# tarepan/DDSP-SVC-official

Hardware: AMD Instinct MI355X
Metric: audio samples/sec @44.1kHz CombSub synth (higher is better)
Workload: dtype f32 storage and accumulation; products of the GEMM / FIR contractions split-bf16x3 (hi*hi+hi*lo+lo*hi), of the attention split-bf16 from three pieces (6 products) for the feature projections and two (3 products) for the context sums; everything else f32; `value_fp32_mfma` is the leg with every produ; 1 GPU; CombSub 44.1 kHz, batch=64x2 s per GPU (Fr=172, T=88064), units/f0/volume/spk_id -> audio, seeded random weights, in-kernel noise

## Files before the change

### ddsp-svc-official_amd/csrc/fir_synth.hip

```cpp
#include "gemm_f32.h"
#include "tables.h"

#include <stdlib.h>

namespace {

__global__ void __launch_bounds__(256) fir_act_kernel(int mode, const float* __restrict__ ctrl, int64_t ld, int M,
                                                      int ldo, int64_t rows, float* __restrict__ out, int split) {
    const int lane = threadIdx.x & 63;
    const int64_t row = (int64_t)blockIdx.x * 4 + (threadIdx.x >> 6);
    if (row >= rows) return;
    const float* src = ctrl + row * ld;
    if (mode != DDSP_FIR_ALLPASS) {
        float* dst = out + row * ldo;
        const float scale = (mode == DDSP_FIR_STATIC) ? (1.0f / 128.0f) : 1.0f;
        if (split) {
            for (int f0 = 0; f0 < M; f0 += 64) {
                const int f = f0 + lane;
                const float v = f < M ? expf(src[f]) * scale : 0.f;
                const uint32_t w = ddsp_split1_group8(v, lane);
                if (f < M) ((uint32_t*)dst)[f] = w;
            }
            return;
        }
        for (int f = lane; f < M; f += 64) dst[f] = expf(src[f]) * scale;
        return;
    }
    float* dst = out + row * ldo;
    const float pi_f = 3.14159274101257324f;
    double carry = 0.0;
    for (int f0 = 0; f0 < M; f0 += 64) {
        const int f = f0 + lane;
        const float gd = (f < M) ? __fmul_rn(pi_f, tanhf(src[f])) : 0.f;
        double incl = (double)gd;
#pragma unroll
        for (int o = 1; o < 64; o <<= 1) {
            double nb = __shfl_up(incl, o, 64);
            if (lane >= o) incl += nb;
        }
        const float phi = (float)(carry + incl);
        carry += __shfl(incl, 63, 64);
        float s = 0.f, c = 0.f;
        if (f < M) sincosf(phi, &s, &c);
        if (split) {
            const uint32_t wc = ddsp_split1_group8(c, lane), ws = ddsp_split1_group8(s, lane);
            if (f < M) {
                ((uint32_t*)dst)[f] = wc;
                ((uint32_t*)dst)[M + f] = ws;
            }
        } else if (f < M) {
            dst[f] = c;
            dst[M + f] = s;
        }
    }
}

struct EpiDynWindow {
    float* ir;
    int n;
    const float* f0;
    float sr15;
    int fast;
    __device__ __forceinline__ float col(int) const { return 0.f; }
    __device__ __forceinline__ float window_fast(float inv_hw, int k) const {
        float w = (float)(k - n / 2) * inv_hw;
        if (w > 1.0f) w = 0.0f;
        return fmaf(0.5f, __builtin_amdgcn_cosf(0.5f * w), 0.5f);
    }
    __device__ __forceinline__ float window(float hw, int k) const {
        float w = __fdiv_rn((float)(k - n / 2), hw);
        if (w > 1.0f) w = 0.0f;
        return __fdiv_rn(__fadd_rn(1.0f, cosf(__fmul_rn(3.14159274101257324f, w))), 2.0f);
    }
    __device__ __forceinline__ void operator()(int, int m, int k, float v, float) const {
        float* row = ir + (int64_t)m * n;
        if (fast) {
            const float inv_hw = __fdiv_rn(__fadd_rn(f0[m], 1e-3f), sr15);
            row[k] = v * window_fast(inv_hw, k);
            if (k > 0 && k < n / 2) row[n - k] = v * window_fast(inv_hw, n - k);
            return;
        }
        const float hw = __fdiv_rn(sr15, __fadd_rn(f0[m], 1e-3f));
        row[k] = __fmul_rn(v, window(hw, k));
        if (k > 0 && k < n / 2) row[n - k] = __fmul_rn(v, window(hw, n - k));
    }
};

struct EpiMirrorStore {
    float* ir;
    int n;
    __device__ __forceinline__ float col(int) const { return 0.f; }
    __device__ __forceinline__ void operator()(int, int m, int k, float v, float) const {
        float* row = ir + (int64_t)m * n;
        row[k] = v;
        if (k > 0 && k < n / 2) row[n - k] = v;
    }
};


__global__ void __launch_bounds__(256) fir_act_exp8_kernel(float scale, const float* __restrict__ ctrl, int64_t ld, int M, int ldo,
                                                           int64_t rows, float* __restrict__ out, int split) {
    const int per_row = M / 8;
    const int64_t i = (int64_t)blockIdx.x * 256 + threadIdx.x;
    if (i >= rows * per_row) return;
    const int64_t row = i / per_row;
    const int gq = (int)(i % per_row);
    const float* src = ctrl + row * ld + 8 * gq;
    const f32x4 a = *(const f32x4*)src, b = *(const f32x4*)(src + 4);
    float v[8];
#pragma unroll
    for (int e = 0; e < 4; ++e) {
        v[e] = expf(a[e]) * scale;
        v[4 + e] = expf(b[e]) * scale;
    }
    float* dst = out + row * ldo + 8 * gq;
    if (split) {
        ddsp_u32x4 hi, lo;
        ddsp_split8(v, hi, lo);
        *(ddsp_u32x4*)dst = hi;
        *(ddsp_u32x4*)(dst + 4) = lo;
    } else {
        *(f32x4*)dst = f32x4{v[0], v[1], v[2], v[3]};
        *(f32x4*)(dst + 4) = f32x4{v[4], v[5], v[6], v[7]};
    }
}

template <int CTRL, int ROW_MASK>
__device__ __forceinline__ double act_dpp_d(double v) {
    const uint64_t u = __builtin_bit_cast(uint64_t, v);
    const int lo = __builtin_amdgcn_update_dpp(0, (int)(uint32_t)u, CTRL, ROW_MASK, 0xf, false);
    const int hi = __builtin_amdgcn_update_dpp(0, (int)(uint32_t)(u >> 32), CTRL, ROW_MASK, 0xf, false);
    return __builtin_bit_cast(double, ((uint64_t)(uint32_t)hi << 32) | (uint32_t)lo);
}
__global__ void __launch_bounds__(256) fir_act_allpass4_kernel(const float* __restrict__ ctrl, int64_t ld, int M, int ldo, int64_t rows,
                                                               float* __restrict__ out, int split) {
    const int lane = threadIdx.x & 63;
    const int64_t row = (int64_t)blockIdx.x * 4 + (threadIdx.x >> 6);
    if (row >= rows) return;
    const float* src = ctrl + row * ld;
    float* dst = out + row * ldo;
    const float pi_f = 3.14159274101257324f;
    double carry = 0.0;
    for (int f0 = 0; f0 < M; f0 += 256) {
        const int f = f0 + 4 * lane;
        const bool in = f < M;
        f32x4 x = {0.f, 0.f, 0.f, 0.f};
        if (in) x = *(const f32x4*)(src + f);
        double run = 0.0, loc[4];
#pragma unroll
        for (int e = 0; e < 4; ++e) {
            const float gd = in ? __fmul_rn(pi_f, tanhf(x[e])) : 0.f;
            run += (double)gd;
            loc[e] = run;
        }
        double incl = run;
        incl += act_dpp_d<0x111, 0xf>(incl);
        incl += act_dpp_d<0x112, 0xf>(incl);
        incl += act_dpp_d<0x114, 0xf>(incl);
        incl += act_dpp_d<0x118, 0xf>(incl);
        incl += act_dpp_d<0x142, 0xa>(incl);
        incl += act_dpp_d<0x143, 0xc>(incl);
        const double base = carry + (incl - run);
        f32x4 c, sn;
#pragma unroll
        for (int e = 0; e < 4; ++e) {
            const float phi = (float)(base + loc[e]);
            float s_ = 0.f, c_ = 0.f;
            if (in) sincosf(phi, &s_, &c_);
            c[e] = c_;
            sn[e] = s_;
        }
        {
            const uint64_t u = __builtin_bit_cast(uint64_t, incl);
            const uint32_t lo = __builtin_amdgcn_readlane((int)(uint32_t)u, 63), hi = __builtin_amdgcn_readlane((int)(uint32_t)(u >> 32), 63);
            carry += __builtin_bit_cast(double, ((uint64_t)hi << 32) | lo);
        }
        if (split) {
            const ddsp_u32x4 pc = ddsp_split4_pair(c, (lane & 1) != 0, 1), ps = ddsp_split4_pair(sn, (lane & 1) != 0, 1);
            if (in) {
                *(ddsp_u32x4*)(dst + f) = pc;
                *(ddsp_u32x4*)(dst + M + f) = ps;
            }
        } else if (in) {
            *(f32x4*)(dst + f) = c;
            *(f32x4*)(dst + M + f) = sn;
        }
    }
}

__global__ void __launch_bounds__(256) repack_rows_kernel(const float* __restrict__ src, int n, int64_t rows, int ld,
                                                          float* __restrict__ dst) {
    typedef float f32x2r __attribute__((ext_vector_type(2)));
    const int half = ld / 2;
    const int64_t total = rows * half;
    for (int64_t i = (int64_t)blockIdx.x * blockDim.x + threadIdx.x; i < total; i += (int64_t)gridDim.x * blockDim.x) {
        const int64_t m = i / half;
        const int k = 2 * (int)(i % half);
        f32x2r v = {0.f, 0.f};
        if (k < n) v = *(const f32x2r*)(src + m * n + k);
        *(f32x2r*)(dst + m * ld + k) = v;
    }
}

__global__ void __launch_bounds__(256) dyn_window_scale_kernel(float* __restrict__ d_ir, const float* __restrict__ f0,
                                                               int n, int64_t rows, float sr15) {
    const int64_t total = rows * n;
    for (int64_t i = (int64_t)blockIdx.x * blockDim.x + threadIdx.x; i < total; i += (int64_t)gridDim.x * blockDim.x) {
        const int64_t m = i / n;
        const int k = (int)(i % n);
        const float hw = __fdiv_rn(sr15, __fadd_rn(f0[m], 1e-3f));
        float w = __fdiv_rn((float)(k - n / 2), hw);
        if (w > 1.0f) w = 0.0f;
        d_ir[i] *= __fdiv_rn(__fadd_rn(1.0f, cosf(__fmul_rn(3.14159274101257324f, w))), 2.0f);
    }
}

__global__ void __launch_bounds__(256) fir_act_bwd_kernel(int mode, const float* __restrict__ ctrl, int64_t ld, int M,
                                                          const float* __restrict__ d_act, int lda, int64_t rows,
                                                          float* __restrict__ d_ctrl, int64_t ldo) {
    const int lane = threadIdx.x & 63;
    const int64_t row = (int64_t)blockIdx.x * 4 + (threadIdx.x >> 6);
    if (row >= rows) return;
    const float* src = ctrl + row * ld;
    const float* g = d_act + row * lda;
    float* dst = d_ctrl + row * ldo;
    if (mode != DDSP_FIR_ALLPASS) {
        const float scale = (mode == DDSP_FIR_STATIC) ? (1.0f / 128.0f) : 1.0f;
        for (int f = lane; f < M; f += 64) dst[f] = g[f] * (expf(src[f]) * scale);
        return;
    }
    const float pi_f = 3.14159274101257324f;
    float th[16], dphi[16];
    double carry = 0.0;
    const int nchunk = (M + 63) / 64;
#pragma unroll
    for (int c = 0; c < 16; ++c) {
        th[c] = 0.f;
        dphi[c] = 0.f;
        if (c < nchunk) {
            const int f = c * 64 + lane;
            const float t = (f < M) ? tanhf(src[f]) : 0.f;
            th[c] = t;
            double incl = (double)((f < M) ? __fmul_rn(pi_f, t) : 0.f);
#pragma unroll
            for (int o = 1; o < 64; o <<= 1) {
                double nb = __shfl_up(incl, o, 64);
                if (lane >= o) incl += nb;
            }
            const float phi = (float)(carry + incl);
            carry += __shfl(incl, 63, 64);
            if (f < M) {
                double sn, cs;
                sincos((double)phi, &sn, &cs);
                dphi[c] = (float)(-sn * (double)g[f] + cs * (double)g[M + f]);
            }
        }
    }
    float tail = 0.f;
#pragma unroll
    for (int c = 15; c >= 0; --c) {
        if (c < nchunk) {
            float incl = dphi[c];
#pragma unroll
            for (int o = 1; o < 64; o <<= 1) {
                float nb = __shfl_down(incl, o, 64);
                if (lane + o < 64) incl += nb;
            }
            const float G = incl + tail;
            tail += __shfl(incl, 0, 64);
            const int f = c * 64 + lane;
            if (f < M) dst[f] = G * pi_f * (1.0f - th[c] * th[c]);
        }
    }
}

}


extern "C" int ddsp_fir_from_ctrl(ddsp_ctx* ctx, void* stream, int mode, const float* ctrl, int64_t ctrl_ld,
                                  int n_mag, const float* f0_frames, int64_t rows, int sr, float* ir) {
    DDSP_REQUIRE(ctx, ctx && ctrl && ir, "ddsp_fir_from_ctrl: null argument");
    DDSP_REQUIRE(ctx, mode >= 0 && mode <= 2, "ddsp_fir_from_ctrl: unknown mode");
    DDSP_REQUIRE(ctx, n_mag >= 3 && n_mag <= 1024 && ctrl_ld >= n_mag && rows >= 0 && rows < (1 << 30),
                 "ddsp_fir_from_ctrl: bad shape");
    DDSP_REQUIRE(ctx, mode != DDSP_FIR_DYNAMIC || f0_frames, "ddsp_fir_from_ctrl: DYNAMIC needs f0_frames");
    if (rows == 0) return DDSP_OK;
    hipStream_t st = (hipStream_t)stream;
    DDSP_ENTER_DEVICE(ctx);
    const int M = n_mag, n = 2 * (n_mag - 1);
    const int K = (mode == DDSP_FIR_ALLPASS) ? 2 * M : M;
    const int lda = ddsp_pad4(K);
    int rc = ddsp_scratch_reserve_bytes(ctx, (size_t)rows * lda * sizeof(float) + 4096);
    if (rc) return rc;
    ddsp_scratch_reset(ctx);
    float* act = nullptr;
    rc = ddsp_scratch_get(ctx, (size_t)rows * lda * sizeof(float), (void**)&act);
    if (rc) return rc;
    float* tab = nullptr;
    const int kind = mode == DDSP_FIR_ALLPASS ? TAB_IRDFT_CPLX : (mode == DDSP_FIR_STATIC ? TAB_IRDFT_RE_HANN : TAB_IRDFT_RE);
    const bool tap_major = K % 32 == 0;
    rc = ddsp_get_table(ctx, st, kind, M, tap_major ? 1 : 0, &tab);
    if (rc) return rc;
    float* tab_split = nullptr;
    if (tap_major && ctx->math != DDSP_MATH_FP32 && (rc = ddsp_get_table(ctx, st, kind, M, 2, &tab_split))) return rc;

    const bool presplit = tap_major && tab_split && rows >= 8192 && M % 8 == 0 && ctx->math != 4;
    ddsp_prof_begin(ctx, st, PF_FIR_ACT);
    const bool wide = M % 8 == 0 && ctrl_ld % 4 == 0 && lda % 8 == 0 && ((uintptr_t)ctrl % 16) == 0;
    if (wide && mode != DDSP_FIR_ALLPASS)
        hipLaunchKernelGGL(fir_act_exp8_kernel, dim3((unsigned)ceil_div64(rows * (M / 8), 256)), dim3(256), 0, st,
                           mode == DDSP_FIR_STATIC ? 1.0f / 128.0f : 1.0f, ctrl, ctrl_ld, M, lda, rows, act, presplit ? 1 : 0);
    else if (wide)
        hipLaunchKernelGGL(fir_act_allpass4_kernel, dim3((unsigned)ceil_div64(rows, 4)), dim3(256), 0, st, ctrl, ctrl_ld, M, lda, rows,
                           act, presplit ? 1 : 0);
    else
        hipLaunchKernelGGL(fir_act_kernel, dim3((unsigned)ceil_div64(rows, 4)), dim3(256), 0, st, mode, ctrl, ctrl_ld, M,
                           lda, rows, act, presplit ? 1 : 0);
    ddsp_prof_end(ctx, st, 0.0, 4.0 * rows * (M + K));
    DDSP_LAUNCH_CHECK(ctx);
    ddsp_prof_begin(ctx, st, PF_FIR_DFT_GEMM);

    auto run = [&](gemm::Args g, const auto& epi) {
        g.math = tap_major ? (ctx->math == 4 ? DDSP_MATH_SPLIT_BF16 : ctx->math) : 0;
        g.B_split = tab_split;
        if (presplit) {
            g.A_split = 1;
            g.B = tab_split;
        }
        if (tap_major)
            gemm::launch<true, true, gemm::A_PLAIN>(st, g, 1, epi);
        else
            gemm::launch<true, false, gemm::A_PLAIN>(st, g, 1, epi);
    };
    const int64_t ldb = tap_major ? K : ddsp_pad4(n);
    if (mode == DDSP_FIR_ALLPASS) {
        gemm::Args g = gemm::make(act, lda, tab, ldb, (int)rows, n, K);
        run(g, gemm::EpiStore{ir, n, nullptr, 1, 0, 0});
    } else {
        gemm::Args g = gemm::make(act, lda, tab, ldb, (int)rows, n / 2 + 1, K);
        if (mode == DDSP_FIR_DYNAMIC)
            run(g, EpiDynWindow{ir, n, f0_frames, 1.5f * (float)sr, (tap_major && ctx->math != DDSP_MATH_FP32) ? 1 : 0});
        else
            run(g, EpiMirrorStore{ir, n});
    }
    ddsp_prof_end(ctx, st, 2.0 * rows * (double)n * K, 4.0 * rows * (K + n));
    DDSP_LAUNCH_CHECK(ctx);
    return DDSP_OK;
}

extern "C" int ddsp_fir_from_ctrl_bwd(ddsp_ctx* ctx, void* stream, int mode, const float* ctrl, int64_t ctrl_ld,
                                      int n_mag, const float* f0_frames, int64_t rows, int sr, float* d_ir,
                                      float* d_ctrl, int64_t d_ctrl_ld) {
    DDSP_REQUIRE(ctx, ctx && ctrl && d_ir && d_ctrl, "ddsp_fir_from_ctrl_bwd: null argument");
    DDSP_REQUIRE(ctx, mode >= 0 && mode <= 2, "ddsp_fir_from_ctrl_bwd: unknown mode");
    DDSP_REQUIRE(ctx, n_mag >= 3 && n_mag <= 1024 && ctrl_ld >= n_mag && d_ctrl_ld >= n_mag && rows >= 0 && rows < (1 << 30),
                 "ddsp_fir_from_ctrl_bwd: bad shape");
    DDSP_REQUIRE(ctx, mode != DDSP_FIR_DYNAMIC || f0_frames, "ddsp_fir_from_ctrl_bwd: DYNAMIC needs f0_frames");
    if (rows == 0) return DDSP_OK;
    hipStream_t st = (hipStream_t)stream;
    DDSP_ENTER_DEVICE(ctx);
    const int M = n_mag, n = 2 * (n_mag - 1);
    const int K = (mode == DDSP_FIR_ALLPASS) ? 2 * M : M;
    const int lda = ddsp_pad4(K);
    const int ldp = ddsp_pad4(n);
    const bool repack = ctx->math != DDSP_MATH_FP32 && ldp % 32 == 0 && rows >= 1024;
    int rc = ddsp_scratch_reserve_bytes(ctx, (size_t)rows * (lda + (repack ? ldp : 0)) * sizeof(float) + 8192);
    if (rc) return rc;
    ddsp_scratch_reset(ctx);
    float* d_act = nullptr;
    if ((rc = ddsp_scratch_get(ctx, (size_t)rows * lda * sizeof(float), (void**)&d_act))) return rc;
    float* d_pad = nullptr;
    if (repack && (rc = ddsp_scratch_get(ctx, (size_t)rows * ldp * sizeof(float), (void**)&d_pad))) return rc;
    float* tab = nullptr;
    const int kind = mode == DDSP_FIR_ALLPASS ? TAB_IRDFT_CPLX : (mode == DDSP_FIR_STATIC ? TAB_IRDFT_RE_HANN : TAB_IRDFT_RE);
    if ((rc = ddsp_get_table(ctx, st, kind, M, 0, &tab))) return rc;
    ddsp_prof_begin(ctx, st, PF_FIR_SYNTH_BWD);
    if (mode == DDSP_FIR_DYNAMIC) {
        int64_t blocks = ceil_div64(rows * n, 256);
        if (blocks > 8192) blocks = 8192;
        hipLaunchKernelGGL(dyn_window_scale_kernel, dim3((unsigned)blocks), dim3(256), 0, st, d_ir, f0_frames, n, rows,
                           1.5f * (float)sr);
    }
    gemm::EpiStore e{d_act, lda, nullptr, 1, 0, 0};
    if (repack) {
        int64_t blocks = ceil_div64(rows * (ldp / 2), 256);
        if (blocks > 8192) blocks = 8192;
        hipLaunchKernelGGL(repack_rows_kernel, dim3((unsigned)blocks), dim3(256), 0, st, d_ir, n, rows, ldp, d_pad);
        gemm::Args g = gemm::make(d_pad, ldp, tab, ldp, (int)rows, K, ldp);
        g.math = DDSP_MATH_SPLIT_BF16;
        gemm::launch<true, true, gemm::A_PLAIN>(st, g, 1, e);
    } else {
        gemm::Args g = gemm::make(d_ir, n, tab, ddsp_pad4(n), (int)rows, K, n);
        gemm::launch<true, true, gemm::A_PLAIN>(st, g, 1, e);
    }
    hipLaunchKernelGGL(fir_act_bwd_kernel, dim3((unsigned)ceil_div64(rows, 4)), dim3(256), 0, st, mode, ctrl, ctrl_ld, M,
                       d_act, lda, rows, d_ctrl, d_ctrl_ld);
    ddsp_prof_end(ctx, st, 2.0 * rows * (double)n * K, 4.0 * rows * (2.0 * K + n));
    DDSP_LAUNCH_CHECK(ctx);
    return DDSP_OK;
}
```

### ddsp-svc-official_amd/csrc/gemm_f32.h

```cpp
#pragma once
#include "common.h"

#include <stdlib.h>
#include <type_traits>

namespace gemm {

enum { A_PLAIN = 0, A_CONV3 = 1, A_FRAMES = 2, A_CONVK = 3 };

struct Args {
    const float* A;
    const float* B;
    int M, N, K;
    int64_t lda, ldb;
    int zdiv;
    int64_t sA_hi, sA_lo, sB_hi, sB_lo;
    int Fr, Cin;
    int tap_shift;
    int ktaps, dil;
    float in_slope;
    const float* zeros;
    int sub_from, parent_tn;
    int math;
    const float* B_split;
    int A_split;
    int xcd;
    int xcd_cut;
    int kz;
};

constexpr int BK = 32;
typedef float f32x4_u __attribute__((ext_vector_type(4), aligned(4)));

template <class E, class = void>
struct epi_wants_pair : std::false_type {};
template <class E>
struct epi_wants_pair<E, std::void_t<decltype(E::kPair)>> : std::true_type {};
template <class E, class = void>
struct epi_has_store4 : std::false_type {};
template <class E>
struct epi_has_store4<E, std::void_t<decltype(E::kStore4)>> : std::true_type {};

template <class E, class = void>
struct epi_is_gated : std::false_type {};
template <class E>
struct epi_is_gated<E, std::void_t<decltype(E::kGatedPair)>> : std::true_type {};

template <class E, class = void>
struct epi_is_rowpair : std::false_type {};
template <class E>
struct epi_is_rowpair<E, std::void_t<decltype(E::kRowPair)>> : std::true_type {};

__device__ __forceinline__ void quad_transpose(float (&x)[4], int q) {
    const bool odd = q & 1, hi = q & 2;
    auto swap1 = [](float v) { return __builtin_bit_cast(float, __builtin_amdgcn_mov_dpp(__builtin_bit_cast(int, v), 0xB1, 0xF, 0xF, true)); };
    auto swap2 = [](float v) { return __builtin_bit_cast(float, __builtin_amdgcn_mov_dpp(__builtin_bit_cast(int, v), 0x4E, 0xF, 0xF, true)); };
    const float r0 = swap1(odd ? x[0] : x[1]);
    const float r1 = swap1(odd ? x[2] : x[3]);
    const float a_lo = odd ? r0 : x[0], a_hi = odd ? x[1] : r0;
    const float b_lo = odd ? r1 : x[2], b_hi = odd ? x[3] : r1;
    const float s_lo = swap2(hi ? a_lo : b_lo);
    const float s_hi = swap2(hi ? a_hi : b_hi);
    x[0] = hi ? s_lo : a_lo;
    x[1] = hi ? s_hi : a_hi;
    x[2] = hi ? b_lo : s_lo;
    x[3] = hi ? b_hi : s_hi;
}

template <int BM, int BN, bool A_KC, bool B_KC, int A_MODE, class Epi, int NW = 4>
__global__ void __launch_bounds__(64 * NW) kernel(Args g, Epi epi) {
    constexpr int WGM = NW / 2, WGN = 2, NT = 64 * NW;
    constexpr int TM = BM / (32 * WGM), TN = BN / (32 * WGN);
    static_assert(TM >= 1 && TN >= 1, "tile too small for the wave grid");
    constexpr int LDM = BM + 1, LDN = BN + 1;
    __shared__ float lds[2 * BK * (LDM + LDN)];
    float* const As0 = lds;
    float* const Bs0 = lds + 2 * BK * LDM;

    const int tid = threadIdx.x;
    const int lane = tid & 63;
    const int wave = tid >> 6;
    const int wm = (wave >> 1) * (BM / WGM);
    const int wn = (wave & 1) * (BN / WGN);
    const int m0 = blockIdx.y * BM;
    const int n0 = blockIdx.x * BN;
    const int z = blockIdx.z;
    const float* __restrict__ A = g.A + (A_MODE == A_FRAMES ? 0 : (int64_t)(z / g.zdiv) * g.sA_hi + (int64_t)(z % g.zdiv) * g.sA_lo);
    const float* __restrict__ B = g.B + (int64_t)(z / g.zdiv) * g.sB_hi + (int64_t)(z % g.zdiv) * g.sB_lo;

    constexpr int NA = BM * BK / (4 * NT), NB = BN * BK / (4 * NT);
    static_assert(NA >= 1 && NB >= 1, "tile too small for the thread count");
    f32x4 ra[NA], rb[NB];

    auto arow = [&](int m) -> const float* {
        if (A_MODE == A_FRAMES) return A + (int64_t)(m / g.Fr) * g.sA_hi + (int64_t)(m % g.Fr) * g.lda;
        return A + (int64_t)m * g.lda;
    };
    auto load_tiles = [&](int k0) {
        const bool k_full = (k0 + BK <= g.K);
        const bool a_full = k_full && (m0 + BM <= g.M);
        const bool b_full = k_full && (n0 + BN <= g.N);
#pragma unroll
        for (int i = 0; i < NA; ++i) {
            const int q = tid + i * NT;
            f32x4 v = {0.f, 0.f, 0.f, 0.f};
            if (A_KC) {
                const int r = q / (BK / 4), kq = q % (BK / 4);
                const int m = m0 + r, k = k0 + kq * 4;
                if (A_MODE == A_CONV3) {
                    if (m < g.M && k < g.K) {
                        const int tap = k / g.Cin, c = k - tap * g.Cin;
                        const int off = tap - 1 + g.tap_shift;
                        const int f = m % g.Fr + off;
                        if (f >= 0 && f < g.Fr) v = *(const f32x4_u*)(A + (int64_t)(m + off) * g.lda + c);
                    }
                } else if (A_MODE == A_CONVK) {
                    if (m < g.M && k < g.K) {
                        const int tap = k / g.Cin, c = k - tap * g.Cin;
                        const int off = (tap - (g.ktaps - 1) / 2) * g.dil;
                        const int f = m % g.Fr + off;
                        if (f >= 0 && f < g.Fr) {
                            v = *(const f32x4_u*)(A + (int64_t)(m + off) * g.lda + c);
#pragma unroll
                            for (int j = 0; j < 4; ++j) v[j] = v[j] > 0.f ? v[j] : v[j] * g.in_slope;
                        }
                    }
                } else if (a_full) {
                    v = *(const f32x4_u*)(arow(m) + k);
                } else if (m < g.M) {
                    const float* p = arow(m) + k;
                    if (k + 3 < g.K) {
                        v = *(const f32x4_u*)p;
                    } else {
                        if (k < g.K) v[0] = p[0];
                        if (k + 1 < g.K) v[1] = p[1];
                        if (k + 2 < g.K) v[2] = p[2];
                    }
                }
            } else {
                const int kr = q / (BM / 4), mq = q % (BM / 4);
                const int k = k0 + kr, m = m0 + mq * 4;
                if (a_full) {
                    v = *(const f32x4_u*)(A + (int64_t)k * g.lda + m);
                } else if (k < g.K) {
                    const float* p = A + (int64_t)k * g.lda + m;
                    if (m + 3 < g.M) {
                        v = *(const f32x4_u*)p;
                    } else {
                        if (m < g.M) v[0] = p[0];
                        if (m + 1 < g.M) v[1] = p[1];
                        if (m + 2 < g.M) v[2] = p[2];
                    }
                }
            }
            ra[i] = v;
        }
#pragma unroll
        for (int i = 0; i < NB; ++i) {
            const int q = tid + i * NT;
            f32x4 v = {0.f, 0.f, 0.f, 0.f};
            if (B_KC) {
                const int r = q / (BK / 4), kq = q % (BK / 4);
                const int n = n0 + r, k = k0 + kq * 4;
                if (b_full) {
                    v = *(const f32x4_u*)(B + (int64_t)n * g.ldb + k);
                } else if (n < g.N) {
                    const float* p = B + (int64_t)n * g.ldb + k;
                    if (k + 3 < g.K) {
                        v = *(const f32x4_u*)p;
                    } else {
                        if (k < g.K) v[0] = p[0];
                        if (k + 1 < g.K) v[1] = p[1];
                        if (k + 2 < g.K) v[2] = p[2];
                    }
                }
            } else {
                const int kr = q / (BN / 4), nq = q % (BN / 4);
                const int k = k0 + kr, n = n0 + nq * 4;
                if (b_full) {
                    v = *(const f32x4_u*)(B + (int64_t)k * g.ldb + n);
                } else if (k < g.K) {
                    const float* p = B + (int64_t)k * g.ldb + n;
                    if (n + 3 < g.N) {
                        v = *(const f32x4_u*)p;
                    } else {
                        if (n < g.N) v[0] = p[0];
                        if (n + 1 < g.N) v[1] = p[1];
                        if (n + 2 < g.N) v[2] = p[2];
                    }
                }
            }
            rb[i] = v;
        }
    };

    auto store_tiles = [&](int buf) {
        float* as = As0 + buf * (BK * LDM);
        float* bs = Bs0 + buf * (BK * LDN);
#pragma unroll
        for (int i = 0; i < NA; ++i) {
            const int q = tid + i * NT;
            if (A_KC) {
                const int r = q / (BK / 4), kq = q % (BK / 4);
#pragma unroll
                for (int j = 0; j < 4; ++j) as[(kq * 4 + j) * LDM + r] = ra[i][j];
            } else {
                const int kr = q / (BM / 4), mq = q % (BM / 4);
#pragma unroll
                for (int j = 0; j < 4; ++j) as[kr * LDM + mq * 4 + j] = ra[i][j];
            }
        }
#pragma unroll
        for (int i = 0; i < NB; ++i) {
            const int q = tid + i * NT;
            if (B_KC) {
                const int r = q / (BK / 4), kq = q % (BK / 4);
#pragma unroll
                for (int j = 0; j < 4; ++j) bs[(kq * 4 + j) * LDN + r] = rb[i][j];
            } else {
                const int kr = q / (BN / 4), nq = q % (BN / 4);
#pragma unroll
                for (int j = 0; j < 4; ++j) bs[kr * LDN + nq * 4 + j] = rb[i][j];
            }
        }
    };

    f32x16 acc[TM][TN];
#pragma unroll
    for (int i = 0; i < TM; ++i)
#pragma unroll
        for (int j = 0; j < TN; ++j)
#pragma unroll
            for (int r = 0; r < 16; ++r) acc[i][j][r] = 0.f;

    const int nk = (g.K + BK - 1) / BK;
    load_tiles(0);
    store_tiles(0);
    __syncthreads();
    const int lr = lane & 31, lh = lane >> 5;
    for (int kt = 0; kt < nk; ++kt) {
        const int buf = kt & 1;
        if (kt + 1 < nk) load_tiles((kt + 1) * BK);
        const float* as = As0 + buf * (BK * LDM) + wm + lr + lh * LDM;
        const float* bs = Bs0 + buf * (BK * LDN) + wn + lr + lh * LDN;
        float a[TM], b[TN];
#pragma unroll
        for (int i = 0; i < TM; ++i) a[i] = as[32 * i];
#pragma unroll
        for (int j = 0; j < TN; ++j) b[j] = bs[32 * j];
#pragma unroll
        for (int kk = 0; kk < BK; kk += 2) {
            float an[TM], bn[TN];
            if (kk + 2 < BK) {
#pragma unroll
                for (int i = 0; i < TM; ++i) an[i] = as[(kk + 2) * LDM + 32 * i];
#pragma unroll
                for (int j = 0; j < TN; ++j) bn[j] = bs[(kk + 2) * LDN + 32 * j];
            }
#pragma unroll
            for (int i = 0; i < TM; ++i)
#pragma unroll
                for (int j = 0; j < TN; ++j)
                    acc[i][j] = __builtin_amdgcn_mfma_f32_32x32x2f32(a[i], b[j], acc[i][j], 0, 0, 0);
            if (kk + 2 < BK) {
#pragma unroll
                for (int i = 0; i < TM; ++i) a[i] = an[i];
#pragma unroll
                for (int j = 0; j < TN; ++j) b[j] = bn[j];
            }
        }
        if (kt + 1 < nk) store_tiles(buf ^ 1);
        __syncthreads();
    }

#pragma unroll
    for (int i = 0; i < TM; ++i)
#pragma unroll
        for (int j = 0; j < TN; ++j) {
            const int n = n0 + wn + 32 * j + lr;
            const bool n_ok = n < g.N;
            const float cb = n_ok ? epi.col(n) : 0.f;
#pragma unroll
            for (int r = 0; r < 16; ++r) {
                const int m = m0 + wm + 32 * i + (r & 3) + 8 * (r >> 2) + 4 * lh;
                if constexpr (epi_is_rowpair<Epi>::value) {
                    if ((r & 1) == 0 && n_ok && m < g.M) epi.pair(z, m, n, acc[i][j][r], acc[i][j][r + 1], cb);
                } else if constexpr (epi_wants_pair<Epi>::value) {
                    const float other = __shfl_xor(acc[i][j][r], 1, 64);
                    if (n_ok && m < g.M) epi(z, m, n, acc[i][j][r], other);
                } else {
                    if (n_ok && m < g.M) epi(z, m, n, acc[i][j][r], cb);
                }
            }
        }
}


template <int BM, int BN, class Epi, int NS = 3, int NW = 8, int A_MODE = A_PLAIN, int MATH = 0>
__global__ void __launch_bounds__(64 * NW, (NW == 4 ? 3 : BM * BN <= 128 * 128 ? 4 : 2)) kernel_dma(Args g, Epi epi, int tiles_m, int tiles_n, int total_tiles) {
    constexpr int WGM = NW / 2, WGN = 2;
    constexpr int TM = BM / (32 * WGM), TN = BN / (32 * WGN);
    constexpr int ROWS = BM + BN;
    constexpr int STAGE = ROWS * 32;
    constexpr int PIECES = ROWS / 8;
    constexpr int PPW = PIECES / NW;
    static_assert(PIECES % NW == 0, "stage must split evenly over the waves");
    __shared__ __attribute__((aligned(1024))) float lds[NS * STAGE];

    const int tid = threadIdx.x, lane = tid & 63, wave = __builtin_amdgcn_readfirstlane(tid >> 6);
    const int wm = (wave >> 1) * (BM / WGM), wn = (wave & 1) * (BN / WGN);
    const int lr = lane & 31, lh = lane >> 5;
    const int nk = g.K / 32;

    const bool xcd_order = g.xcd && (gridDim.x & 7) == 0 && g.sub_from == 0 && total_tiles == tiles_m * tiles_n - g.xcd_cut;
    const int xq0 = (int)blockIdx.x >> 3, xgs = (int)gridDim.x >> 3, xx = (int)blockIdx.x & 7;
    const int xown = (tiles_m / 8) * tiles_n, xleft = (tiles_m % 8) * tiles_n - g.xcd_cut;
    int my_tiles = (total_tiles - (int)blockIdx.x + (int)gridDim.x - 1) / (int)gridDim.x;
    if (xcd_order) {
        const int qx = xown + (xleft > xx ? (xleft - xx + 7) / 8 : 0);
        my_tiles = xq0 < qx ? (qx - xq0 + xgs - 1) / xgs : 0;
    }
    auto tile_of = [&](int i) -> int {
        if (!xcd_order) return (int)blockIdx.x + i * (int)gridDim.x;
        const int q = xq0 + i * xgs;
        if (q < xown) return (xx + 8 * (q / tiles_n)) * tiles_n + q % tiles_n;
        const int u = (q - xown) * 8 + xx;
        return ((tiles_m / 8) * 8 + u / tiles_n) * tiles_n + u % tiles_n;
    };
    const int steps = my_tiles * nk;

    constexpr int PA = (BM / 8) / NW;
    static_assert((BM / 8) % NW == 0, "A rows must split evenly over the waves");
    const float* src_m1[PA];
    const float* src_p1[PA];
    int conv_f[PA];
    int kbase_cur = 0;
    auto tile_src = [&](int tile, const float* (&src)[PPW]) {
        const int per_z = tiles_m * tiles_n;
        int z = tile / per_z, rem = tile - z * per_z;
        int m0 = (rem / tiles_n) * BM, n0 = (rem % tiles_n) * BN;
        if (g.sub_from > 0) {
            const int big = g.sub_from + (tile >> 2), q = tile & 3;
            z = 0;
            m0 = (2 * (big / g.parent_tn) + (q >> 1)) * BM;
            n0 = (2 * (big % g.parent_tn) + (q & 1)) * BN;
        }
        const float* A = g.A + (int64_t)(z / g.zdiv) * g.sA_hi + (int64_t)(z % g.zdiv) * g.sA_lo;
        const float* B = g.B + (int64_t)(z / g.zdiv) * g.sB_hi + (int64_t)(z % g.zdiv) * g.sB_lo;
        kbase_cur = z * g.kz;
#pragma unroll
        for (int i = 0; i < PPW; ++i) {
            const int piece = wave + NW * i;
            const int row = piece * 8 + (lane >> 3);
            const int slot = (lane & 7) ^ ((row >> 1) & 7);
            if (row < BM) {
                int m = m0 + row;
                m = m < g.M ? m : g.M - 1;
                src[i] = A + (int64_t)m * g.lda + slot * 4;
                if constexpr (A_MODE == A_CONVK) {
                    if (i < PA) conv_f[i < PA ? i : 0] = m % g.Fr;
                }
                if constexpr (A_MODE == A_CONV3) {
                    if (i < PA) {
                        const int f = m % g.Fr;
                        const int s = g.tap_shift;
                        const float* base = src[i];
                        const float* zp = g.zeros + slot * 4;
                        src_m1[i < PA ? i : 0] = (f - 1 + s >= 0 && f - 1 + s < g.Fr) ? base + (int64_t)(s - 1) * g.lda : zp;
                        src_p1[i < PA ? i : 0] = (f + 1 + s >= 0 && f + 1 + s < g.Fr) ? base + (int64_t)(s + 1) * g.lda : zp;
                        src[i] = (f + s >= 0 && f + s < g.Fr) ? base + (int64_t)s * g.lda : zp;
                    }
                }
            } else {
                int n = n0 + row - BM;
                n = n < g.N ? n : g.N - 1;
                src[i] = B + (int64_t)n * g.ldb + slot * 4;
            }
        }
    };
    auto issue = [&](const float* const (&src)[PPW], int kt, int stage) {
        int tap = 1, koff = kt * 32 + kbase_cur;
        if constexpr (A_MODE == A_CONV3 || A_MODE == A_CONVK) {
            tap = koff / g.Cin;
            koff -= tap * g.Cin;
        }
        const int conv_off = A_MODE == A_CONVK ? (tap - (g.ktaps - 1) / 2) * g.dil : 0;
#pragma unroll
        for (int i = 0; i < PPW; ++i) {
            const int piece = wave + NW * i;
            const float* p = src[i] + kt * 32 + kbase_cur;
            if constexpr (A_MODE == A_CONV3) {
                if (i < PA) p = (tap == 0 ? src_m1[i < PA ? i : 0] : tap == 1 ? src[i] : src_p1[i < PA ? i : 0]) + koff;
            }
            if constexpr (A_MODE == A_CONVK) {
                if (i < PA) {
                    const int f = conv_f[i < PA ? i : 0] + conv_off;
                    p = (f >= 0 && f < g.Fr) ? src[i] + (int64_t)conv_off * g.lda + koff : g.zeros + (lane & 7) * 4;
                }
            }
            __builtin_amdgcn_global_load_lds((const __attribute__((address_space(1))) void*)p,
                                             (__attribute__((address_space(3))) void*)(lds + stage * STAGE + piece * 256),
                                             16, 0, 0);
        }
    };

    const float* src_cur[PPW];
    int issued = 0;
    int issue_tile = 0, issue_kt = 0;
    if (steps > 0) tile_src(tile_of(0), src_cur);
    auto issue_next = [&]() {
        if (issued >= steps) return;
        issue(src_cur, issue_kt, issued % NS);
        ++issued;
        if (++issue_kt == nk) {
            issue_kt = 0;
            ++issue_tile;
            if (issue_tile < my_tiles) tile_src(tile_of(issue_tile), src_cur);
        }
    };
#pragma unroll
    for (int i = 0; i < NS - 1; ++i) issue_next();

    f32x16 acc[TM][TN];
#pragma unroll
    for (int i = 0; i < TM; ++i)
#pragma unroll
        for (int j = 0; j < TN; ++j)
#pragma unroll
            for (int r = 0; r < 16; ++r) acc[i][j][r] = 0.f;

    int kt = 0, tile_i = 0;
    for (int step = 0; step < steps; ++step) {
        static_assert((NS - 2) * PPW <= 63, "vmcnt is a 6-bit counter");
        if (NS > 2 && step + NS - 2 < steps)
            asm volatile("s_waitcnt vmcnt(%0)" ::"n"((NS - 2) * PPW) : "memory");
        else
            asm volatile("s_waitcnt vmcnt(0)" ::: "memory");
        __builtin_amdgcn_s_barrier();
        issue_next();
        const float* st = lds + (step % NS) * STAGE;
        f32x4 av[TM][4], bv[TN][4];
#pragma unroll
        for (int i = 0; i < TM; ++i) {
            const int row = wm + 32 * i + lr;
            const float* rp = st + row * 32;
#pragma unroll
            for (int c = 0; c < 4; ++c) av[i][c] = *(const f32x4*)(rp + 4 * ((4 * lh + c) ^ ((row >> 1) & 7)));
        }
#pragma unroll
        for (int j = 0; j < TN; ++j) {
            const int row = BM + wn + 32 * j + lr;
            const float* rp = st + row * 32;
#pragma unroll
            for (int c = 0; c < 4; ++c) bv[j][c] = *(const f32x4*)(rp + 4 * ((4 * lh + c) ^ ((row >> 1) & 7)));
        }
        if constexpr (MATH != 0) {
            typedef __bf16 bf16x8 __attribute__((ext_vector_type(8)));
            typedef float f32x2p __attribute__((ext_vector_type(2)));
            typedef __bf16 bf16x2p __attribute__((ext_vector_type(2)));
            typedef uint32_t u32x4p __attribute__((ext_vector_type(4)));
            auto split = [](const f32x4& x0, const f32x4& x1, bf16x8 (&p)[3]) {
                constexpr int NQ = 2;
                u32x4p w[3];
#pragma unroll
                for (int d = 0; d < 4; ++d) {
                    f32x2p r = d < 2 ? (f32x2p){x0[2 * d], x0[2 * d + 1]} : (f32x2p){x1[2 * d - 4], x1[2 * d - 3]};
#pragma unroll
                    for (int q = 0; q < NQ; ++q) {
                        const uint32_t h = __builtin_bit_cast(uint32_t, __builtin_convertvector(r, bf16x2p));
                        w[q][d] = h;
                        if (q + 1 < NQ)
                            r = r - (f32x2p){__builtin_bit_cast(float, h << 16), __builtin_bit_cast(float, h & 0xffff0000u)};
                    }
                }
#pragma unroll
                for (int q = 0; q < NQ; ++q) p[q] = __builtin_bit_cast(bf16x8, w[q]);
            };
#pragma unroll
            for (int half = 0; half < 2; ++half) {
                bf16x8 ap[TM][3], bp[TN][3];
#pragma unroll
                for (int i = 0; i < TM; ++i) {
                    if constexpr (MATH == 8) {
                        ap[i][0] = __builtin_bit_cast(bf16x8, av[i][2 * half]);
                        ap[i][1] = __builtin_bit_cast(bf16x8, av[i][2 * half + 1]);
                    } else {
                        split(av[i][2 * half], av[i][2 * half + 1], ap[i]);
                    }
                }
#pragma unroll
                for (int j = 0; j < TN; ++j) {
                    if constexpr (MATH == 7 || MATH == 8) {
                        bp[j][0] = __builtin_bit_cast(bf16x8, bv[j][2 * half]);
                        bp[j][1] = __builtin_bit_cast(bf16x8, bv[j][2 * half + 1]);
                    } else {
                        split(bv[j][2 * half], bv[j][2 * half + 1], bp[j]);
                    }
                }
#pragma unroll
                for (int i = 0; i < TM; ++i)
#pragma unroll
                    for (int j = 0; j < TN; ++j) {
                        auto mm = [&](int x, int y) {
                            acc[i][j] = __builtin_amdgcn_mfma_f32_32x32x16_bf16(ap[i][x], bp[j][y], acc[i][j], 0, 0, 0);
                        };
                        mm(1, 0);
                        mm(0, 1);
                        mm(0, 0);
                    }
            }
        } else {
#pragma unroll
            for (int s = 0; s < 16; ++s)
#pragma unroll
                for (int i = 0; i < TM; ++i)
#pragma unroll
                    for (int j = 0; j < TN; ++j)
                        acc[i][j] = __builtin_amdgcn_mfma_f32_32x32x2f32(av[i][s >> 2][s & 3], bv[j][s >> 2][s & 3],
                                                                         acc[i][j], 0, 0, 0);
        }
        if (++kt == nk) {
            const int tile = tile_of(tile_i);
            const int per_z = tiles_m * tiles_n;
            int z = tile / per_z, rem = tile - z * per_z;
            int m0 = (rem / tiles_n) * BM, n0 = (rem % tiles_n) * BN;
            if (g.sub_from > 0) {
                const int big = g.sub_from + (tile >> 2), q = tile & 3;
                z = 0;
                m0 = (2 * (big / g.parent_tn) + (q >> 1)) * BM;
                n0 = (2 * (big % g.parent_tn) + (q & 1)) * BN;
            }
            bool vec = false;
            if constexpr (epi_has_store4<Epi>::value) vec = epi.vec_ok() && n0 + BN <= g.N;
            if constexpr (epi_is_gated<Epi>::value) {
                static_assert(TN == 2, "gated-pair epilogue needs the wave's two column blocks");
                const int q = lane & 3;
                const int na = n0 + wn + lr;
                const float ba = epi.col(na), bg = epi.col(na + 32);
                const int oc = ((n0 + wn) >> 1) + (lr & ~3);
#pragma unroll
                for (int i = 0; i < TM; ++i)
#pragma unroll
                    for (int rg = 0; rg < 4; ++rg) {
                        float x[4];
#pragma unroll
                        for (int r = 0; r < 4; ++r) {
                            const float a = acc[i][0][4 * rg + r] + ba, gt = acc[i][1][4 * rg + r] + bg;
                            if constexpr (MATH != 0)
                                x[r] = a * __builtin_amdgcn_rcpf(1.0f + __builtin_amdgcn_exp2f(-1.44269504088896341f * gt));
                            else
                                x[r] = a * (1.0f / (1.0f + expf(-gt)));
                            acc[i][0][4 * rg + r] = 0.f;
                            acc[i][1][4 * rg + r] = 0.f;
                        }
                        quad_transpose(x, q);
                        const int m = m0 + wm + 32 * i + q + 8 * rg + 4 * lh;
                        if (m < g.M) epi.store4(z, m, oc, f32x4{x[0], x[1], x[2], x[3]});
                    }
            } else if (vec) {
                if constexpr (epi_has_store4<Epi>::value) {
                    const int q = lane & 3;
#pragma unroll
                    for (int i = 0; i < TM; ++i)
#pragma unroll
                        for (int j = 0; j < TN; ++j) {
                            const int n = n0 + wn + 32 * j + (lr & ~3);
#pragma unroll
                            for (int rg = 0; rg < 4; ++rg) {
                                float x[4] = {acc[i][j][4 * rg], acc[i][j][4 * rg + 1], acc[i][j][4 * rg + 2], acc[i][j][4 * rg + 3]};
                                quad_transpose(x, q);
                                const int m = m0 + wm + 32 * i + q + 8 * rg + 4 * lh;
                                if (m < g.M) epi.store4(z, m, n, f32x4{x[0], x[1], x[2], x[3]});
#pragma unroll
                                for (int r = 0; r < 4; ++r) acc[i][j][4 * rg + r] = 0.f;
                            }
                        }
                }
            } else
#pragma unroll
            for (int i = 0; i < TM; ++i)
#pragma unroll
                for (int j = 0; j < TN; ++j) {
                    const int n = n0 + wn + 32 * j + lr;
                    const bool n_ok = n < g.N;
                    const float cb = n_ok ? epi.col(n) : 0.f;
#pragma unroll
                    for (int r = 0; r < 16; ++r) {
                        const int m = m0 + wm + 32 * i + (r & 3) + 8 * (r >> 2) + 4 * lh;
                        if constexpr (epi_is_rowpair<Epi>::value) {
                            if ((r & 1) == 0 && n_ok && m < g.M) epi.pair(z, m, n, acc[i][j][r], acc[i][j][r + 1], cb);
                        } else if constexpr (epi_wants_pair<Epi>::value) {
                            const float other = __shfl_xor(acc[i][j][r], 1, 64);
                            if (n_ok && m < g.M) epi(z, m, n, acc[i][j][r], other);
                        } else {
                            if (n_ok && m < g.M) epi(z, m, n, acc[i][j][r], cb);
                        }
                        acc[i][j][r] = 0.f;
                    }
                }
            kt = 0;
            ++tile_i;
        }
    }
}

inline bool dma_ok(const Args& g) {
    return g.K % 32 == 0 && g.lda % 4 == 0 && g.ldb % 4 == 0 && ((uintptr_t)g.A % 16) == 0 && ((uintptr_t)g.B % 16) == 0 &&
           g.sA_hi % 4 == 0 && g.sA_lo % 4 == 0 && g.sB_hi % 4 == 0 && g.sB_lo % 4 == 0;
}

template <int BM, int BN, class Epi, int NS = 3, int NW = 8, int A_MODE = A_PLAIN, int MATH = 0>
inline void launch_dma(hipStream_t st, const Args& g, int batch, const Epi& epi, int total_override = -1) {
    const int tiles_m = (g.M + BM - 1) / BM, tiles_n = (g.N + BN - 1) / BN;
    const int total = total_override >= 0 ? total_override : tiles_m * tiles_n * batch;
    if (total == 0) return;
    constexpr int lds_bytes = NS * (BM + BN) * 128;
    constexpr int by_waves = 16 / NW;
    constexpr int by_lds = 160 * 1024 / lds_bytes;
    constexpr int per_cu = by_lds < by_waves ? by_lds : by_waves;
    int grid = 256 * per_cu;
    if (grid > total) grid = total;
    hipLaunchKernelGGL((kernel_dma<BM, BN, Epi, NS, NW, A_MODE, MATH>), dim3(grid), dim3(64 * NW), 0, st, g, epi, tiles_m, tiles_n, total);
}

inline int xcd_default(int math) { return math == 3 ? 1 : 0; }

template <int BM, int BN, class Epi, int NS = 3, int NW = 8, int A_MODE = A_PLAIN>
inline void dma_go(hipStream_t st, const Args& g0, int batch, const Epi& epi, int total_override = -1) {
    Args g = g0;
    if (g.xcd < 0) g.xcd = (batch == 1 && total_override < 0) ? xcd_default(g.math) : 0;
    if (g.math == 3 && g.B_split && g.A_split) {
        Args h = g;
        h.B = g.B_split;
        launch_dma<BM, BN, Epi, NS, NW, A_MODE, 8>(st, h, batch, epi, total_override);
    } else if (g.math == 3 && g.B_split) {
        Args h = g;
        h.B = g.B_split;
        launch_dma<BM, BN, Epi, NS, NW, A_MODE, 7>(st, h, batch, epi, total_override);
    } else if (g.math == 3)
        launch_dma<BM, BN, Epi, NS, NW, A_MODE, 3>(st, g, batch, epi, total_override);
    else
        launch_dma<BM, BN, Epi, NS, NW, A_MODE, 0>(st, g, batch, epi, total_override);
}

template <int BM, int BN, bool A_KC, bool B_KC, int A_MODE, class Epi, int NW = 4>
inline void launch_tile(hipStream_t st, const Args& g, int batch, const Epi& epi) {
    dim3 grid((g.N + BN - 1) / BN, (g.M + BM - 1) / BM, batch);
    hipLaunchKernelGGL((kernel<BM, BN, A_KC, B_KC, A_MODE, Epi, NW>), grid, dim3(64 * NW), 0, st, g, epi);
}

constexpr int64_t T128_MIN = 512;

constexpr int SMALL_NS = 4;


template <bool A_KC, bool B_KC, int A_MODE, class Epi>
inline void launch(hipStream_t st, const Args& g, int batch, const Epi& epi) {
    auto blocks = [&](int bm, int bn) {
        return (int64_t)((g.M + bm - 1) / bm) * ((g.N + bn - 1) / bn) * batch;
    };
    if constexpr (A_KC && B_KC && A_MODE == A_CONV3) {
        if (dma_ok(g) && g.zeros && g.Cin % 32 == 0 && g.Cin + 32 <= DDSP_ZERO_FLOATS && g.N <= 256) {
            if (blocks(64, 64) < 128 && blocks(64, 64) > 16)
                dma_go<32, 64, Epi, 4, 2, A_CONV3>(st, g, batch, epi);
            else
                dma_go<64, 64, Epi, 3, 4, A_CONV3>(st, g, batch, epi);
            return;
        }
    }
    if constexpr (A_KC && B_KC && A_MODE == A_PLAIN) {
        if (dma_ok(g) && blocks(64, 64) < 128 && blocks(64, 64) > 16 && g.K >= 256) {
            dma_go<32, 64, Epi, 4, 2>(st, g, batch, epi);
            return;
        }
        if (dma_ok(g) && blocks(64, 64) < 256 && g.K >= 256) {
            dma_go<64, 64, Epi, SMALL_NS, 4>(st, g, batch, epi);
            return;
        }
        if (dma_ok(g) && g.N <= 256 && blocks(64, 64) >= 256) {
            dma_go<64, 64, Epi, 3, 4>(st, g, batch, epi);
            return;
        }
        if (dma_ok(g) && blocks(128, 64) >= 256) {
            if (g.N <= 256)
                dma_go<64, 64, Epi, 3, 4>(st, g, batch, epi);
            else if (blocks(128, 128) >= T128_MIN) {
                const int total = (int)blocks(128, 128);
                const int rem = total % 512;
                bool split = false;
                if constexpr (!epi_is_gated<Epi>::value) {
                    const bool xcd_on = g.xcd > 0 || (g.xcd < 0 && xcd_default(g.math));
                    if (batch == 1 && rem > 0 && rem <= 64 && !xcd_on) {
                        split = true;
                        dma_go<128, 128, Epi, 2>(st, g, batch, epi, total - rem);
                        Args r = g;
                        r.xcd = 0;
                        r.sub_from = total - rem;
                        r.parent_tn = (g.N + 127) / 128;
                        dma_go<64, 64, Epi, 3, 4>(st, r, 1, epi, 4 * rem);
                    }
                }
                if (!split) dma_go<128, 128, Epi, 2>(st, g, batch, epi);
            }
            else
                dma_go<128, 64, Epi, 3>(st, g, batch, epi);
            return;
        }
        if (dma_ok(g) && blocks(64, 64) >= 256) {
            dma_go<64, 64, Epi, 3, 4>(st, g, batch, epi);
            return;
        }
    }
    if ((g.B_split && g.B_split == g.B) || g.A_split) {
        ddsp_launch_refusal() = "pre-split GEMM operands reached the register-staged path (size predicates disagree)";
        return;
    }
    if (blocks(128, 64) >= 512)
        launch_tile<128, 64, A_KC, B_KC, A_MODE, Epi, 8>(st, g, batch, epi);
    else
        launch_tile<64, 64, A_KC, B_KC, A_MODE, Epi, 4>(st, g, batch, epi);
}

inline Args make(const float* A, int64_t lda, const float* B, int64_t ldb, int M, int N, int K) {
    Args g;
    g.A = A;
    g.B = B;
    g.M = M;
    g.N = N;
    g.K = K;
    g.lda = lda;
    g.ldb = ldb;
    g.zdiv = 1;
    g.sA_hi = g.sA_lo = g.sB_hi = g.sB_lo = 0;
    g.Fr = 1;
    g.Cin = 4;
    g.tap_shift = 0;
    g.ktaps = 3;
    g.dil = 1;
    g.in_slope = 1.f;
    g.zeros = nullptr;
    g.sub_from = 0;
    g.parent_tn = 0;
    g.math = 0;
    g.B_split = nullptr;
    g.A_split = 0;
    g.xcd_cut = 0;
    g.xcd = -1;
    g.kz = 0;
    return g;
}

struct EpiStore {
    float* C;
    int64_t ldc;
    const float* bias;
    int zdiv;
    int64_t sC_hi, sC_lo;
    __device__ __forceinline__ float col(int n) const { return bias ? bias[n] : 0.f; }
    __device__ __forceinline__ void operator()(int z, int m, int n, float v, float cb) const {
        float* c = C + (int64_t)(z / zdiv) * sC_hi + (int64_t)(z % zdiv) * sC_lo;
        c[(int64_t)m * ldc + n] = v + cb;
    }
    static constexpr bool kStore4 = true;
    __device__ __forceinline__ bool vec_ok() const {
        return ((uintptr_t)C % 16) == 0 && ldc % 4 == 0 && sC_hi % 4 == 0 && sC_lo % 4 == 0;
    }
    __device__ __forceinline__ void store4(int z, int m, int n, f32x4 v) const {
        float* c = C + (int64_t)(z / zdiv) * sC_hi + (int64_t)(z % zdiv) * sC_lo;
        if (bias) v += *(const f32x4_u*)(bias + n);
        *(f32x4*)(c + (int64_t)m * ldc + n) = v;
    }
};

struct EpiResidual {
    float* C;
    const float* res;
    int64_t ldc;
    const float* bias;
    __device__ __forceinline__ float col(int n) const { return bias[n]; }
    __device__ __forceinline__ void operator()(int, int m, int n, float v, float cb) const {
        const int64_t o = (int64_t)m * ldc + n;
        C[o] = res[o] + (v + cb);
    }
    static constexpr bool kStore4 = true;
    __device__ __forceinline__ bool vec_ok() const { return (((uintptr_t)C | (uintptr_t)res) % 16) == 0 && ldc % 4 == 0; }
    __device__ __forceinline__ void store4(int, int m, int n, f32x4 v) const {
        const int64_t o = (int64_t)m * ldc + n;
        *(f32x4*)(C + o) = *(const f32x4*)(res + o) + (v + *(const f32x4_u*)(bias + n));
    }
};

}
```

### ddsp-svc-official_amd/csrc/tables.h

```cpp
#pragma once
#include "common.h"

enum {
    TAB_IRDFT_RE = 1,
    TAB_IRDFT_RE_HANN = 2,
    TAB_IRDFT_CPLX = 3,
    TAB_RDFT_FWD_W = 4,
    TAB_RDFT_INV_W = 5,
};

static inline int ddsp_pad4(int n) { return (n + 3) & ~3; }
```

### ddsp-svc-official_amd/csrc/tables.hip

```cpp
#include "tables.h"

namespace {

constexpr double kTwoPi = 6.283185307179586476925286766559;

__global__ void irdft_table_kernel(float* __restrict__ tab, int M, int n, int ld, int rows, int hann, int tap_major) {
    const int64_t total = tap_major ? (int64_t)n * rows : (int64_t)rows * ld;
    for (int64_t idx = (int64_t)blockIdx.x * blockDim.x + threadIdx.x; idx < total;
         idx += (int64_t)gridDim.x * blockDim.x) {
        const int row = tap_major ? (int)(idx % rows) : (int)(idx / ld);
        const int k = tap_major ? (int)(idx / rows) : (int)(idx % ld);
        if (k >= n) {
            tab[idx] = 0.f;
            continue;
        }
        const int f = row < M ? row : row - M;
        const double cf = (f == 0 || f == M - 1) ? 1.0 : 2.0;
        int64_t r = ((int64_t)f * (k - n / 2)) % n;
        if (r < 0) r += n;
        const double ang = kTwoPi * (double)r / (double)n;
        double v;
        if (row < M)
            v = cf / n * cos(ang);
        else
            v = (f == 0 || f == M - 1) ? 0.0 : -cf / n * sin(ang);
        if (hann) v *= 0.5 - 0.5 * cos(kTwoPi * (double)k / (double)n);
        tab[idx] = (float)v;
    }
}

__global__ void rdft_w_table_kernel(float* __restrict__ tab, int N, int ld, int inverse) {
    const int Mb = N / 2 + 1;
    const int64_t total = inverse ? (int64_t)N * 2 * Mb : (int64_t)N * ld;
    for (int64_t idx = (int64_t)blockIdx.x * blockDim.x + threadIdx.x; idx < total;
         idx += (int64_t)gridDim.x * blockDim.x) {
        int i, col;
        if (!inverse) {
            i = (int)(idx / ld);
            col = (int)(idx % ld);
            if (col >= 2 * Mb) {
                tab[idx] = 0.f;
                continue;
            }
        } else {
            col = (int)(idx / N);
            i = (int)(idx % N);
        }
        const int f = col < Mb ? col : col - Mb;
        const bool im = col >= Mb;
        const int64_t r = ((int64_t)f * i) % N;
        const double ang = kTwoPi * (double)r / (double)N;
        const double w = sqrt(0.5 - 0.5 * cos(kTwoPi * (double)i / (double)N));
        double v;
        if (!inverse) {
            v = im ? -sin(ang) : cos(ang);
        } else {
            const double cf = (f == 0 || f == N / 2) ? 1.0 : 2.0;
            v = im ? ((f == 0 || f == N / 2) ? 0.0 : -cf / N * sin(ang)) : cf / N * cos(ang);
        }
        tab[idx] = (float)(v * w);
    }
}

__global__ void presplit_kernel(const float* __restrict__ src, uint32_t* __restrict__ dst, int64_t groups) {
    typedef float f32x2v __attribute__((ext_vector_type(2)));
    typedef __bf16 bf16x2v __attribute__((ext_vector_type(2)));
    for (int64_t gidx = (int64_t)blockIdx.x * blockDim.x + threadIdx.x; gidx < groups; gidx += (int64_t)gridDim.x * blockDim.x) {
        const float* s = src + 8 * gidx;
        uint32_t hi[4], lo[4];
#pragma unroll
        for (int d = 0; d < 4; ++d) {
            const float a = s[2 * d], b = s[2 * d + 1];
            hi[d] = __builtin_bit_cast(uint32_t, __builtin_convertvector((f32x2v){a, b}, bf16x2v));
            const float ha = __builtin_bit_cast(float, hi[d] << 16), hb = __builtin_bit_cast(float, hi[d] & 0xffff0000u);
            lo[d] = __builtin_bit_cast(uint32_t, __builtin_convertvector((f32x2v){a - ha, b - hb}, bf16x2v));
        }
        uint32_t* o = dst + 8 * gidx;
#pragma unroll
        for (int d = 0; d < 4; ++d) {
            o[d] = hi[d];
            o[4 + d] = lo[d];
        }
    }
}

}

int ddsp_get_table(ddsp_ctx* ctx, hipStream_t st, int kind, int n0, int n1, float** out) {
    for (int i = 0; i < ctx->n_tables; ++i) {
        ddsp_table& t = ctx->tables[i];
        if (t.kind == kind && t.n0 == n0 && t.n1 == n1) {
            *out = t.dev;
            return DDSP_OK;
        }
    }
    if (ctx->n_tables >= 64) return ddsp_fail(ctx, DDSP_ERR_OOM, "table cache full", "");
    if (n1 == 2) {
        float* plain = nullptr;
        int rc = ddsp_get_table(ctx, st, kind, n0, 1, &plain);
        if (rc) return rc;
        if (ctx->n_tables >= 64) return ddsp_fail(ctx, DDSP_ERR_OOM, "table cache full", "");
        size_t bytes = 0;
        for (int i = 0; i < ctx->n_tables; ++i)
            if (ctx->tables[i].dev == plain) bytes = ctx->tables[i].bytes;
        if (bytes == 0 || bytes % 32 != 0) return ddsp_fail(ctx, DDSP_ERR_ARG, "table cannot be pre-split", "");
        float* dev = nullptr;
        hipError_t e = hipMalloc((void**)&dev, bytes);
        if (e != hipSuccess) return ddsp_fail(ctx, DDSP_ERR_OOM, "table hipMalloc", hipGetErrorString(e));
        const int64_t groups = (int64_t)(bytes / 32);
        hipLaunchKernelGGL(presplit_kernel, dim3((unsigned)((groups + 255) / 256 > 2048 ? 2048 : (groups + 255) / 256)), dim3(256), 0,
                           st, plain, (uint32_t*)dev, groups);
        DDSP_LAUNCH_CHECK(ctx);
        ddsp_table& t = ctx->tables[ctx->n_tables++];
        t.kind = kind;
        t.n0 = n0;
        t.n1 = n1;
        t.dev = dev;
        t.bytes = bytes;
        *out = dev;
        return DDSP_OK;
    }
    size_t elems = 0;
    switch (kind) {
        case TAB_IRDFT_RE:
        case TAB_IRDFT_RE_HANN:
            elems = n1 ? (size_t)n0 * 2 * (n0 - 1) : (size_t)n0 * ddsp_pad4(2 * (n0 - 1));
            break;
        case TAB_IRDFT_CPLX:
            elems = n1 ? (size_t)2 * n0 * 2 * (n0 - 1) : (size_t)2 * n0 * ddsp_pad4(2 * (n0 - 1));
            break;
        case TAB_RDFT_FWD_W:
            elems = (size_t)n0 * ddsp_pad4(2 * (n0 / 2 + 1));
            break;
        case TAB_RDFT_INV_W:
            elems = (size_t)n0 * 2 * (n0 / 2 + 1);
            break;
        default:
            return ddsp_fail(ctx, DDSP_ERR_ARG, "unknown table kind", "");
    }
    float* dev = nullptr;
    hipError_t e = hipMalloc((void**)&dev, elems * sizeof(float));
    if (e != hipSuccess) return ddsp_fail(ctx, DDSP_ERR_OOM, "table hipMalloc", hipGetErrorString(e));
    const unsigned blocks = (unsigned)((elems + 255) / 256 > 2048 ? 2048 : (elems + 255) / 256);
    if (kind == TAB_IRDFT_RE || kind == TAB_IRDFT_RE_HANN || kind == TAB_IRDFT_CPLX) {
        const int M = n0, n = 2 * (n0 - 1);
        const int rows = kind == TAB_IRDFT_CPLX ? 2 * M : M;
        hipLaunchKernelGGL(irdft_table_kernel, dim3(blocks), dim3(256), 0, st, dev, M, n, ddsp_pad4(n), rows,
                           kind == TAB_IRDFT_RE_HANN ? 1 : 0, n1 ? 1 : 0);
    } else {
        hipLaunchKernelGGL(rdft_w_table_kernel, dim3(blocks), dim3(256), 0, st, dev, n0,
                           ddsp_pad4(2 * (n0 / 2 + 1)), kind == TAB_RDFT_INV_W ? 1 : 0);
    }
    DDSP_LAUNCH_CHECK(ctx);
    ddsp_table& t = ctx->tables[ctx->n_tables++];
    t.kind = kind;
    t.n0 = n0;
    t.n1 = n1;
    t.dev = dev;
    t.bytes = elems * sizeof(float);
    *out = dev;
    return DDSP_OK;
}
```

### ddsp-svc-official_amd/ddsp/vocoder.py

```python
import os

import torch
import yaml

import hipddsp
from hipddsp import (COMB_SINC, COMB_SINC_GATED, COMB_NONE, EXC_AUDIO, EXC_GENERATE, EXC_UNIT_NOISE, FIR_ALLPASS,
                     FIR_DYNAMIC, FIR_STATIC, FIR_SPLIT_BF16)


from .hubert import RaggedCounts
from .unit2control import Unit2Control


class Volume_Extractor:

    def __init__(self, hop_size=512, device="cuda"):
        self.hop_size = hop_size
        self.device = device

    def extract(self, audio, n_samples=None):
        import numpy as np
        if n_samples is not None:
            if not isinstance(audio, torch.Tensor) or audio.dim() != 2:
                raise ValueError("Volume_Extractor.extract: a ragged batch is a (B, T) tensor")
            if not float(self.hop_size).is_integer():
                raise ValueError("Volume_Extractor.extract: a ragged batch needs an integral hop_size")
            vals = hipddsp.check_volume_n_samples(n_samples, audio.shape[0], audio.shape[1], int(self.hop_size))
            if not audio.is_cuda:
                raise RuntimeError("Volume_Extractor runs on a HIP device only (no CPU fallback)")
            return hipddsp.context_for(audio.device).volume_extract(audio, int(self.hop_size), vals)
        is_np = isinstance(audio, np.ndarray)
        x = torch.from_numpy(np.ascontiguousarray(audio, dtype=np.float32)).to(self.device) if is_np else audio
        if not x.is_cuda:
            raise RuntimeError("Volume_Extractor runs on a HIP device only (no CPU fallback)")
        flat = x.dim() == 1
        hop = int(self.hop_size) if float(self.hop_size).is_integer() else float(self.hop_size)
        vol = hipddsp.context_for(x.device).volume_extract(x.reshape(1, -1) if flat else x, hop)
        vol = vol[0] if flat else vol
        return vol.cpu().numpy() if is_np else vol


def _find_torchcrepe_checkpoint(model="full"):
    import importlib.util
    try:
        spec = importlib.util.find_spec("torchcrepe")
    except (ImportError, ValueError):
        spec = None
    for d in (list(spec.submodule_search_locations or []) if spec is not None else []):
        p = os.path.join(d, "assets", f"{model}.pth")
        if os.path.isfile(p):
            return p
    raise FileNotFoundError(
        f"F0_Extractor('crepe'): no CREPE checkpoint given and no installed torchcrepe with assets/{model}.pth was found; pass "
        "crepe_ckpt='/path/to/full.pth' (torchcrepe's state dict) or a ddsp.crepe.Crepe module")


class F0_Extractor:

    def __init__(self, f0_extractor, sample_rate=44100, hop_size=512, f0_min=65, f0_max=800, *, crepe_ckpt=None, device=None):
        if f0_extractor in ('parselmouth', 'dio', 'harvest'):
            raise NotImplementedError(
                f"f0 extractor '{f0_extractor}' has no device implementation (it is a CPU library): 'crepe' is the device "
                "extractor; keep the reference's F0_Extractor for the others")
        if f0_extractor != 'crepe':
            raise ValueError(f" [x] Unknown f0 extractor: {f0_extractor}")
        self.f0_extractor, self.sample_rate, self.hop_size, self.f0_min, self.f0_max = \
            f0_extractor, sample_rate, hop_size, f0_min, f0_max
        if device is None:
            if not torch.cuda.is_available():
                raise RuntimeError("F0_Extractor runs on a HIP device only (no CPU fallback)")
            device = "cuda"
        if torch.device(device).type != "cuda":
            raise RuntimeError("F0_Extractor runs on a HIP device only (no CPU fallback); got device=%r" % (device,))
        from .crepe import Crepe
        if isinstance(crepe_ckpt, Crepe):
            model = crepe_ckpt
        else:
            path = crepe_ckpt if crepe_ckpt is not None else _find_torchcrepe_checkpoint("full")
            sd = torch.load(path, map_location="cpu", weights_only=True)
            model = Crepe("tiny" if sd["conv1.weight"].shape[0] == 128 else "full")
            model.load_state_dict(sd)
        self.model = model.to(device).eval()
        self.device = device

    def extract(self, audio, uv_interp=False, device=None, silence_front=0, *, dither=True, seed=None, seed_dev=None,
                n_samples=None):
        import numpy as np
        from .crepe import HOP, SAMPLE_RATE
        if n_samples is not None:
            return self._extract_ragged(audio, uv_interp, silence_front, dither, seed, seed_dev, n_samples)
        is_np = isinstance(audio, np.ndarray)
        x = torch.from_numpy(np.ascontiguousarray(audio, dtype=np.float32)).to(self.device) if is_np else audio
        if not x.is_cuda:
            raise RuntimeError("F0_Extractor runs on a HIP device only (no CPU fallback)")
        flat = x.dim() == 1
        if x.dim() not in (1, 2):
            raise ValueError("F0_Extractor.extract: audio must be (T,) or (B, T)")
        x = x.reshape(1, -1) if flat else x
        sr, hop = self.sample_rate, self.hop_size
        n_frames = int(x.shape[-1] // hop) + 1
        start_frame = int(silence_front * sr / hop)
        real_silence_front = start_frame * hop / sr
        x = x[:, int(np.round(real_silence_front * sr)):].contiguous().float()
        ctx = hipddsp.context_for(x.device)
        x16 = x if int(sr) == SAMPLE_RATE else ctx.resample(x, int(sr), SAMPLE_RATE, lowpass_filter_width=128)
        fr = hipddsp.crepe_frames(x16.shape[-1], HOP)
        if fr < 3:
            raise ValueError(f"F0_Extractor('crepe'): {x16.shape[-1]} samples at 16 kHz give {fr} CREPE frames; the reference's "
                             "reflect-padded filters need at least 3 (audio of at least 160 samples at 16 kHz)")
        probs = self.model.activations(x16, HOP)
        if seed_dev is not None:
            f0, pd = ctx.crepe_decode(probs, self.f0_min, self.f0_max, segment=512, dither=dither, seed_dev=seed_dev)
        else:
            if dither and seed is None:
                seed = _seed_from_torch()
            f0, pd = ctx.crepe_decode(probs, self.f0_min, self.f0_max, segment=512, dither_seed=int(seed or 0), dither=dither)
        out = ctx.f0_postfilter(f0, pd, sr, hop, n_frames, start_frame, 0.05, uv_interp, self.f0_min)
        out = out[0] if flat else out
        return out.cpu().numpy() if is_np else out


    def _extract_ragged(self, audio, uv_interp, silence_front, dither, seed, seed_dev, n_samples):
        from .crepe import HOP, SAMPLE_RATE
        if silence_front != 0:
            raise ValueError("F0_Extractor.extract: silence_front is not available with n_samples (a ragged batch)")
        if seed_dev is not None:
            raise ValueError("F0_Extractor.extract: seed_dev is not available with n_samples (a ragged batch)")
        if not isinstance(audio, torch.Tensor) or audio.dim() != 2:
            raise ValueError("F0_Extractor.extract: a ragged batch is a (B, T) tensor")
        B, T = audio.shape
        sr, hop = self.sample_rate, self.hop_size
        vals = hipddsp.check_n_samples(n_samples, B, T)
        resampled = int(sr) != SAMPLE_RATE
        lib = hipddsp.load_library()
        n16 = [int(lib.ddsp_resample_length(v, int(sr), SAMPLE_RATE)) for v in vals] if resampled else vals
        T16 = int(lib.ddsp_resample_length(T, int(sr), SAMPLE_RATE)) if resampled else T
        n16 = hipddsp.check_crepe_n_samples(n16, B, T16, HOP)
        if not audio.is_cuda:
            raise RuntimeError("F0_Extractor runs on a HIP device only (no CPU fallback)")
        ctx = hipddsp.context_for(audio.device)
        n_crepe = [hipddsp.crepe_frames(v, HOP) for v in n16]
        n_out = [int(v // hop) + 1 for v in vals]
        table = hipddsp.crepe_ragged_table(n16, HOP)
        dev = ctx.ragged_counts(vals + table + n_crepe + n_out)
        n_dev, table_dev, nc_dev, no_dev = dev[:B], dev[B:3 * B + 1], dev[3 * B + 1:4 * B + 1], dev[4 * B + 1:]
        x = audio.contiguous().float()
        x16 = ctx.resample_ragged(x, n_dev, int(sr), SAMPLE_RATE, lowpass_filter_width=128) if resampled else x
        probs = self.model.activations(x16, HOP, n16, table_dev)
        if dither and seed is None:
            seed = _seed_from_torch()
        f0, pd = ctx.crepe_decode(probs, self.f0_min, self.f0_max, segment=512, dither_seed=int(seed or 0), dither=dither,
                                  n_frames=n_crepe, counts_dev=nc_dev)
        return ctx.f0_postfilter(f0, pd, sr, hop, max(n_out), 0, 0.05, uv_interp, self.f0_min, n_crepe=n_crepe, n_out=n_out,
                                 counts_dev=(nc_dev, no_dev))


def align_units(units, n_samples, sample_rate, hop_size, encoder_sample_rate=16000, encoder_hop_size=320):
    n_frames = int(int(n_samples) // hop_size) + 1
    ratio = (hop_size / sample_rate) / (encoder_hop_size / encoder_sample_rate)
    return hipddsp.context_for(units.device).align_units(units, n_frames, ratio)


class Audio2HubertSoft(torch.nn.Module):

    def __init__(self, path, h_sample_rate=16000, h_hop_size=320, device=None):
        super().__init__()
        from torch.nn.modules.utils import consume_prefix_in_state_dict_if_present
        from .hubert import HubertSoft
        print(' [Encoder Model] HuBERT Soft')
        self.hubert = HubertSoft()
        print(' [Loading] ' + path)
        checkpoint = torch.load(path, map_location="cpu")
        consume_prefix_in_state_dict_if_present(checkpoint, "module.")
        self.hubert.load_state_dict(checkpoint)
        self.hubert.eval()
        if device is not None:
            self.hubert.to(device)

    def forward(self, audio, n_samples=None):
        return self.hubert.units(audio.unsqueeze(1), n_samples)


class Units_Encoder:

    def __init__(self, encoder, encoder_ckpt, encoder_sample_rate=16000, encoder_hop_size=320, device=None):
        if encoder in ('hubertbase', 'hubertbase768', 'contentvec', 'contentvec768', 'xunit', 'yunit'):
            raise NotImplementedError(
                f"units encoder '{encoder}' has no device implementation: 'hubertsoft' is the device encoder; callers that "
                "keep the reference's encoders can align their units on the device with ddsp.vocoder.align_units")
        if encoder != 'hubertsoft':
            raise ValueError(f" [x] Unknown units encoder: {encoder}")
        if device is None:
            if not torch.cuda.is_available():
                raise RuntimeError("Units_Encoder runs on a HIP device only (no CPU fallback)")
            device = "cuda"
        if torch.device(device).type != "cuda":
            raise RuntimeError("Units_Encoder runs on a HIP device only (no CPU fallback); got device=%r" % (device,))
        self.device = device
        self.model = Audio2HubertSoft(encoder_ckpt, device=device)
        self.model = self.model.eval()
        self.encoder_sample_rate = encoder_sample_rate
        self.encoder_hop_size = encoder_hop_size

    def encode(self, audio, sample_rate, hop_size, n_samples=None):
        if n_samples is not None:
            return self._encode_ragged(audio, sample_rate, hop_size, n_samples)
        if not audio.is_cuda:
            raise RuntimeError("Units_Encoder runs on a HIP device only (no CPU fallback)")
        ctx = hipddsp.context_for(audio.device)
        audio_res = audio if sample_rate == self.encoder_sample_rate else \
            ctx.resample(audio, int(sample_rate), int(self.encoder_sample_rate), lowpass_filter_width=128)
        units = self.model(audio_res)
        return align_units(units, audio.size(-1), sample_rate, hop_size, self.encoder_sample_rate, self.encoder_hop_size)

    def _encode_ragged(self, audio, sample_rate, hop_size, n_samples):
        if audio.dim() != 2:
            raise ValueError("Units_Encoder.encode: a ragged batch is (B, T) audio")
        B, T = audio.shape
        vals = hipddsp.check_n_samples(n_samples, B, T)
        resampled = sample_rate != self.encoder_sample_rate
        lib = hipddsp.load_library()
        n16 = [int(lib.ddsp_resample_length(v, int(sample_rate), int(self.encoder_sample_rate))) for v in vals] \
            if resampled else vals
        T16 = int(lib.ddsp_resample_length(T, int(sample_rate), int(self.encoder_sample_rate))) if resampled else T
        n16 = hipddsp.check_hubert_n_samples(n16, B, T16)
        if not audio.is_cuda:
            raise RuntimeError("Units_Encoder runs on a HIP device only (no CPU fallback)")
        ctx = hipddsp.context_for(audio.device)
        n_units = [hipddsp.hubert_frames(v) for v in n16]
        n_out = [int(v // hop_size) + 1 for v in vals]
        dev = ctx.ragged_counts(vals + n16 + n_units + n_out).reshape(4, B)
        audio_res = ctx.resample_ragged(audio, dev[0], int(sample_rate), int(self.encoder_sample_rate),
                                        lowpass_filter_width=128) if resampled else audio
        units = self.model(audio_res, RaggedCounts(n16, T16, dev[1]))
        ratio = (hop_size / sample_rate) / (self.encoder_hop_size / self.encoder_sample_rate)
        return ctx.align_units_ragged(units, max(n_out), ratio, dev[2], dev[3])


class DotDict(dict):

    def __getattr__(self, key):
        val = self.get(key)
        return DotDict(val) if type(val) is dict else val

    __setattr__ = dict.__setitem__
    __delattr__ = dict.__delitem__


def load_model(model_path, device="cpu"):
    with open(os.path.join(os.path.split(model_path)[0], "config.yaml"), "r") as fh:
        args = DotDict(yaml.safe_load(fh))
    kind = args.model.type
    if kind == "Sins":
        model = Sins(sampling_rate=args.data.sampling_rate, block_size=args.data.block_size,
                     n_harmonics=args.model.n_harmonics, n_mag_allpass=args.model.n_mag_allpass,
                     n_mag_noise=args.model.n_mag_noise, n_unit=args.data.encoder_out_channels,
                     n_spk=args.model.n_spk, c=args.model.c)
    elif kind == "CombSub":
        model = CombSub(sampling_rate=args.data.sampling_rate, block_size=args.data.block_size,
                        n_mag_allpass=args.model.n_mag_allpass, n_mag_harmonic=args.model.n_mag_harmonic,
                        n_mag_noise=args.model.n_mag_noise, n_unit=args.data.encoder_out_channels,
                        n_spk=args.model.n_spk, c=args.model.c)
    elif kind == "CombSubFast":
        model = CombSubFast(sampling_rate=args.data.sampling_rate, block_size=args.data.block_size,
                            n_unit=args.data.encoder_out_channels, n_spk=args.model.n_spk, c=args.model.c)
    else:
        raise ValueError(f" [x] Unknown Model: {kind}")
    print(" [Loading] " + model_path)
    ckpt = torch.load(model_path, map_location=torch.device(device), weights_only=True)
    model.to(device)
    model.load_state_dict(ckpt["model"])
    model.eval()
    return model, args


def _seed_from_torch():
    return int(torch.randint(0, 2 ** 62, (1,), dtype=torch.int64).item())


class _SynthBase(torch.nn.Module):
    def __init__(self, sampling_rate, block_size):
        super().__init__()
        self.register_buffer("sampling_rate", torch.tensor(sampling_rate))
        self.register_buffer("block_size", torch.tensor(block_size))
        self._sr = int(sampling_rate)
        self._hop = int(block_size)

    def _front(self, f0_frames, initial_phase, infer, comb_mode, **want):
        if not f0_frames.is_cuda:
            raise RuntimeError("the synthesiser runs on a HIP device only (no CPU fallback): move the model and its "
                               "inputs to 'cuda'")
        ctx = hipddsp.context_for(f0_frames.device)
        return ctx, ctx.phase_scan(f0_frames, self._hop, self._sr, initial_phase, bool(infer), comb_mode, **want)

    def _ragged_front(self, units, f0_frames, volume, n_frames, initial_phase, infer, comb_mode, **want):
        B, Fr = units.shape[0], units.shape[1]
        vals = hipddsp.check_n_frames(n_frames, B, Fr)
        if self._training_graph():
            raise NotImplementedError("n_frames= (ragged batches) is inference only: there is no ragged backward pass; call the "
                                      "model under torch.no_grad() (training crops every clip to one length)")
        if not f0_frames.is_cuda:
            raise RuntimeError("the synthesiser runs on a HIP device only (no CPU fallback): move the model and its "
                               "inputs to 'cuda'")
        if self._hop % 4:
            raise ValueError("n_frames= needs a block_size that is a multiple of 4")
        ctx = hipddsp.context_for(f0_frames.device)
        n_dev = ctx.ragged_counts(vals)
        units = ctx.ragged_frames(units, n_dev, hold=False)
        f0 = ctx.ragged_frames(f0_frames.reshape(B, Fr), n_dev, hold=True).reshape(B, Fr, 1)
        volume = ctx.ragged_frames(volume.reshape(B, Fr), n_dev, hold=False)
        ps = ctx.phase_scan(f0, self._hop, self._sr, initial_phase, bool(infer), comb_mode, **want)
        return ctx, n_dev, units, f0, volume, ps

    def _ragged_noise(self, ctx, n_dev, B, Fr, noise, noise_seed):
        seed = 0 if noise is not None else (_seed_from_torch() if noise_seed is None else int(noise_seed))
        return ctx.ragged_noise(noise, seed, n_dev, B, Fr, self._hop), EXC_UNIT_NOISE, 0

    def _empty_result(self, f0_frames, sample_rate_phase=False, shared=False):
        Fr = f0_frames.shape[1]
        T = Fr * self._hop
        z = lambda *shape: torch.zeros(*shape, device=f0_frames.device)
        sig = z(0, T)
        ph = z(0, T, 1) if sample_rate_phase else z(0, Fr, 1)
        return sig, ph, ((sig, sig) if shared else (z(0, T), z(0, T)))

    def _training_graph(self):
        return torch.is_grad_enabled() and any(p.requires_grad for p in self.unit2ctrl.parameters())

    @staticmethod
    def _noise_args(noise, noise_seed):
        if noise is not None:
            return noise.contiguous().float(), EXC_UNIT_NOISE, 0
        return None, EXC_GENERATE, (_seed_from_torch() if noise_seed is None else int(noise_seed))


class _SynthTrainFn(torch.autograd.Function):

    @staticmethod
    def forward(fctx, model, units, f0_frames, volume, spk_id, spk_mix_dict, initial_phase, infer, noise, noise_seed,
                *params):
        ctx, ps = model._front(f0_frames, initial_phase, infer, model._comb_mode, **model._front_wants)
        keep_math = ctx.math
        ctx.set_math(hipddsp.MATH_FP32)
        try:
            ctrl, kept = model.unit2ctrl.forward_flat_keep(units, f0_frames, ps["phase_frames"], volume, spk_id,
                                                           spk_mix_dict, ctx=ctx)
            nargs = model._noise_args(noise, noise_seed)
            outs, saved = model._train_forward(ctx, ctrl, ps, f0_frames, nargs)
        finally:
            ctx.set_math(keep_math)
        fctx.model, fctx.dsp = model, ctx
        fctx.set_materialize_grads(False)
        fctx.args = (units, f0_frames, volume, spk_id, spk_mix_dict, nargs, ps["phase_frames"])
        fctx.saved = (ctrl, saved, kept)
        phase_out = ps["phase"] if model._front_wants.get("want_phase") else ps["phase_frames"]
        fctx.mark_non_differentiable(phase_out)
        return (phase_out,) + tuple(outs)

    @staticmethod
    def backward(fctx, d_phase, *d_outs):
        model, ctx = fctx.model, fctx.dsp
        units, f0_frames, volume, spk_id, spk_mix_dict, nargs, phase_frames = fctx.args
        if fctx.saved is None:
            raise RuntimeError("this synthesiser forward was already back-propagated (its kept activations are released)")
        ctrl, saved, kept = fctx.saved
        B, Fr = ctrl.shape[0], ctrl.shape[1]
        d_ctrl = model._train_backward(ctx, ctrl, saved, f0_frames, nargs, d_outs)
        grads = model.unit2ctrl.backward_flat(units, f0_frames, phase_frames, volume, spk_id, spk_mix_dict,
                                              d_ctrl.reshape(B, Fr, -1), ctx=ctx, kept=kept)
        fctx.saved = None
        return (None,) * 10 + tuple(grads.get(p) for p in model.unit2ctrl.parameters())


def _sum_grads(ref, *gs):
    acc = None
    for g in gs:
        if g is not None:
            acc = g.contiguous() if acc is None else acc + g
    return torch.zeros_like(ref) if acc is None else acc


class CombSub(_SynthBase):

    def __init__(self, sampling_rate, block_size, n_mag_allpass, n_mag_harmonic, n_mag_noise, n_unit=256, n_spk=1,
                 c=False):
        super().__init__(sampling_rate, block_size)
        print(" [DDSP Model] Combtooth Subtractive Synthesiser (Old Version)")
        self.n_mags = (int(n_mag_allpass), int(n_mag_harmonic), int(n_mag_noise))
        self.unit2ctrl = Unit2Control(n_unit, n_spk, {"group_delay": n_mag_allpass,
                                                      "harmonic_magnitude": n_mag_harmonic,
                                                      "noise_magnitude": n_mag_noise}, c)

    _comb_mode = COMB_SINC
    _front_wants = {}

    def _train_forward(self, ctx, ctrl, ps, f0_frames, nargs):
        B, Fr = ctrl.shape[0], ctrl.shape[1]
        rows, sr, hop = B * Fr, self._sr, self._hop
        na, nh, nn_ = self.n_mags
        c2 = ctrl.reshape(rows, -1)
        ir_ap = ctx.fir_from_ctrl(FIR_ALLPASS, c2, 0, na, rows, sr)
        h1, _ = ctx.ltv_fir(ps["comb"], ir_ap, B, Fr, hop, math=ctx.fir_math)
        ir_h = ctx.fir_from_ctrl(FIR_DYNAMIC, c2, na, nh, rows, sr, f0_frames)
        harmonic, _ = ctx.ltv_fir(h1, ir_h, B, Fr, hop, math=ctx.fir_math)
        ir_n = ctx.fir_from_ctrl(FIR_STATIC, c2, na + nh, nn_, rows, sr)
        nz, exc, seed = nargs
        noise_out, signal = ctx.ltv_fir(nz, ir_n, B, Fr, hop, excitation=exc, noise_seed=seed, add_in=harmonic,
                                        math=ctx.fir_math)
        return (signal, harmonic, noise_out), (ps["comb"], h1, ir_ap, ir_h, ir_n)

    def _train_backward(self, ctx, ctrl, saved, f0_frames, nargs, d_outs):
        comb, h1, ir_ap, ir_h, ir_n = saved
        d_signal, d_harm, d_noise = d_outs
        B, Fr = ctrl.shape[0], ctrl.shape[1]
        rows, sr, hop = B * Fr, self._sr, self._hop
        na, nh, nn_ = self.n_mags
        nz, exc, seed = nargs
        d_h = _sum_grads(comb, d_signal, d_harm)
        d_n = _sum_grads(comb, d_signal, d_noise)
        c2 = ctrl.reshape(rows, -1)
        d_ctrl = torch.empty_like(c2)
        _, d_ir = ctx.ltv_fir_bwd(nz, ir_n, d_n, B, Fr, hop, excitation=exc, noise_seed=seed, want_d_audio=False)
        ctx.fir_from_ctrl_bwd(FIR_STATIC, c2, na + nh, nn_, rows, sr, d_ir, d_ctrl)
        d_h1, d_ir = ctx.ltv_fir_bwd(h1, ir_h, d_h, B, Fr, hop)
        ctx.fir_from_ctrl_bwd(FIR_DYNAMIC, c2, na, nh, rows, sr, d_ir, d_ctrl, f0_frames)
        _, d_ir = ctx.ltv_fir_bwd(comb, ir_ap, d_h1, B, Fr, hop, want_d_audio=False)
        ctx.fir_from_ctrl_bwd(FIR_ALLPASS, c2, 0, na, rows, sr, d_ir, d_ctrl)
        return d_ctrl

    def synth_from_ctrl(self, ctx, ctrl, f0_frames, comb, noise=None, noise_seed=None, n_dev=None):
        B, Fr = ctrl.shape[0], ctrl.shape[1]
        rows, sr, hop = B * Fr, self._sr, self._hop
        na, nh, nn_ = self.n_mags
        c2 = ctrl.reshape(rows, -1)
        crop = (lambda *xs: ctx.ragged_crop_(n_dev, Fr, hop, *xs)) if n_dev is not None else (lambda *xs: None)
        crop(comb)
        ir = ctx.fir_from_ctrl(FIR_ALLPASS, c2, 0, na, rows, sr)
        h, _ = ctx.ltv_fir(comb, ir, B, Fr, hop, math=ctx.fir_math)
        crop(h)
        ir = ctx.fir_from_ctrl(FIR_DYNAMIC, c2, na, nh, rows, sr, f0_frames)
        harmonic, _ = ctx.ltv_fir(h, ir, B, Fr, hop, math=ctx.fir_math)
        crop(harmonic)
        ir = ctx.fir_from_ctrl(FIR_STATIC, c2, na + nh, nn_, rows, sr)
        nz, exc, seed = self._noise_args(noise, noise_seed) if n_dev is None else \
            self._ragged_noise(ctx, n_dev, B, Fr, noise, noise_seed)
        noise_out, signal = ctx.ltv_fir(nz, ir, B, Fr, hop, excitation=exc, noise_seed=seed, add_in=harmonic,
                                        math=ctx.fir_math)
        crop(noise_out, signal)
        return signal, harmonic, noise_out

    def forward(self, units_frames, f0_frames, volume_frames, spk_id, spk_mix_dict=None, initial_phase=None,
                infer=True, noise=None, noise_seed=None, n_frames=None, **kwargs):
        if units_frames.shape[0] == 0:
            return self._empty_result(f0_frames)
        if n_frames is not None:
            ctx, n_dev, units, f0, vol, ps = self._ragged_front(units_frames, f0_frames, volume_frames, n_frames,
                                                                initial_phase, infer, COMB_SINC)
            ctrl = self.unit2ctrl.forward_ragged(ctx, units, f0, ps["phase_frames"], vol, spk_id, spk_mix_dict, n_dev)
            signal, harmonic, noise_out = self.synth_from_ctrl(ctx, ctrl, f0, ps["comb"], noise, noise_seed, n_dev)
            pf = ctx.ragged_frames(ps["phase_frames"], n_dev, hold=False, out=ps["phase_frames"])
            return signal, pf.unsqueeze(-1), (harmonic, noise_out)
        if self._training_graph():
            pf, signal, harmonic, noise_out = _SynthTrainFn.apply(
                self, units_frames, f0_frames, volume_frames, spk_id, spk_mix_dict, initial_phase, infer, noise,
                noise_seed, *self.unit2ctrl.parameters())
            return signal, pf.unsqueeze(-1), (harmonic, noise_out)
        ctx, ps = self._front(f0_frames, initial_phase, infer, COMB_SINC)
        ctrl = self.unit2ctrl.forward_flat(units_frames, f0_frames, ps["phase_frames"], volume_frames, spk_id,
                                           spk_mix_dict)
        signal, harmonic, noise_out = self.synth_from_ctrl(ctx, ctrl, f0_frames, ps["comb"], noise, noise_seed)
        return signal, ps["phase_frames"].unsqueeze(-1), (harmonic, noise_out)


class Sins(_SynthBase):

    def __init__(self, sampling_rate, block_size, n_harmonics, n_mag_allpass, n_mag_noise, n_unit=256, n_spk=1,
                 c=False):
        super().__init__(sampling_rate, block_size)
        print(" [DDSP Model] Sinusoids Additive Synthesiser")
        self.n_mags = (int(n_harmonics), int(n_mag_allpass), int(n_mag_noise))
        self.unit2ctrl = Unit2Control(n_unit, n_spk, {"amplitudes": n_harmonics, "group_delay": n_mag_allpass,
                                                      "noise_magnitude": n_mag_noise}, c)

    _comb_mode = COMB_NONE
    _front_wants = {"want_phase": True}

    def _train_forward(self, ctx, ctrl, ps, f0_frames, nargs):
        B, Fr = ctrl.shape[0], ctrl.shape[1]
        rows, sr, hop = B * Fr, self._sr, self._hop
        nhm, na, nn_ = self.n_mags
        c2 = ctrl.reshape(rows, -1)
        sinusoids = ctx.sins_bank(c2, 0, nhm, f0_frames, ps["phase"], B, Fr, hop, sr)
        ir_ap = ctx.fir_from_ctrl(FIR_ALLPASS, c2, nhm, na, rows, sr)
        harmonic, _ = ctx.ltv_fir(sinusoids, ir_ap, B, Fr, hop, math=ctx.fir_math)
        ir_n = ctx.fir_from_ctrl(FIR_STATIC, c2, nhm + na, nn_, rows, sr)
        nz, exc, seed = nargs
        noise_out, signal = ctx.ltv_fir(nz, ir_n, B, Fr, hop, excitation=exc, noise_seed=seed, add_in=harmonic,
                                        math=ctx.fir_math)
        return (signal, harmonic, noise_out), (ps["phase"], sinusoids, ir_ap, ir_n)

    def _train_backward(self, ctx, ctrl, saved, f0_frames, nargs, d_outs):
        phase, sinusoids, ir_ap, ir_n = saved
        d_signal, d_harm, d_noise = d_outs
        B, Fr = ctrl.shape[0], ctrl.shape[1]
        rows, sr, hop = B * Fr, self._sr, self._hop
        nhm, na, nn_ = self.n_mags
        nz, exc, seed = nargs
        d_h = _sum_grads(sinusoids, d_signal, d_harm)
        d_n = _sum_grads(sinusoids, d_signal, d_noise)
        c2 = ctrl.reshape(rows, -1)
        d_ctrl = torch.empty_like(c2)
        _, d_ir = ctx.ltv_fir_bwd(nz, ir_n, d_n, B, Fr, hop, excitation=exc, noise_seed=seed, want_d_audio=False)
        ctx.fir_from_ctrl_bwd(FIR_STATIC, c2, nhm + na, nn_, rows, sr, d_ir, d_ctrl)
        d_sin, d_ir = ctx.ltv_fir_bwd(sinusoids, ir_ap, d_h, B, Fr, hop)
        ctx.fir_from_ctrl_bwd(FIR_ALLPASS, c2, nhm, na, rows, sr, d_ir, d_ctrl)
        ctx.sins_bank_bwd(c2, 0, nhm, f0_frames, phase, d_sin, B, Fr, hop, sr, d_ctrl)
        return d_ctrl

    def synth_from_ctrl(self, ctx, ctrl, f0_frames, phase, noise=None, noise_seed=None, n_dev=None):
        B, Fr = ctrl.shape[0], ctrl.shape[1]
        rows, sr, hop = B * Fr, self._sr, self._hop
        nhm, na, nn_ = self.n_mags
        c2 = ctrl.reshape(rows, -1)
        crop = (lambda *xs: ctx.ragged_crop_(n_dev, Fr, hop, *xs)) if n_dev is not None else (lambda *xs: None)
        sinusoids = ctx.sins_bank(c2, 0, nhm, f0_frames, phase, B, Fr, hop, sr)
        crop(sinusoids)
        ir = ctx.fir_from_ctrl(FIR_ALLPASS, c2, nhm, na, rows, sr)
        harmonic, _ = ctx.ltv_fir(sinusoids, ir, B, Fr, hop, math=ctx.fir_math)
        crop(harmonic)
        ir = ctx.fir_from_ctrl(FIR_STATIC, c2, nhm + na, nn_, rows, sr)
        nz, exc, seed = self._noise_args(noise, noise_seed) if n_dev is None else \
            self._ragged_noise(ctx, n_dev, B, Fr, noise, noise_seed)
        noise_out, signal = ctx.ltv_fir(nz, ir, B, Fr, hop, excitation=exc, noise_seed=seed, add_in=harmonic,
                                        math=ctx.fir_math)
        crop(noise_out, signal)
        return signal, harmonic, noise_out

    def forward(self, units_frames, f0_frames, volume_frames, spk_id, spk_mix_dict=None, initial_phase=None,
                infer=True, max_upsample_dim=32, noise=None, noise_seed=None, n_frames=None):
        if units_frames.shape[0] == 0:
            return self._empty_result(f0_frames, sample_rate_phase=True)
        if n_frames is not None:
            ctx, n_dev, units, f0, vol, ps = self._ragged_front(units_frames, f0_frames, volume_frames, n_frames,
                                                                initial_phase, infer, COMB_NONE, want_phase=True)
            ctrl = self.unit2ctrl.forward_ragged(ctx, units, f0, ps["phase_frames"], vol, spk_id, spk_mix_dict, n_dev)
            signal, harmonic, noise_out = self.synth_from_ctrl(ctx, ctrl, f0, ps["phase"], noise, noise_seed, n_dev)
            ctx.ragged_crop_(n_dev, f0.shape[1], self._hop, ps["phase"])
            return signal, ps["phase"].unsqueeze(-1), (harmonic, noise_out)
        if self._training_graph():
            ph, signal, harmonic, noise_out = _SynthTrainFn.apply(
                self, units_frames, f0_frames, volume_frames, spk_id, spk_mix_dict, initial_phase, infer, noise,
                noise_seed, *self.unit2ctrl.parameters())
            return signal, ph.unsqueeze(-1), (harmonic, noise_out)
        ctx, ps = self._front(f0_frames, initial_phase, infer, COMB_NONE, want_phase=True)
        ctrl = self.unit2ctrl.forward_flat(units_frames, f0_frames, ps["phase_frames"], volume_frames, spk_id,
                                           spk_mix_dict)
        signal, harmonic, noise_out = self.synth_from_ctrl(ctx, ctrl, f0_frames, ps["phase"], noise, noise_seed)
        return signal, ps["phase"].unsqueeze(-1), (harmonic, noise_out)


class CombSubFast(_SynthBase):

    def __init__(self, sampling_rate, block_size, n_unit=256, n_spk=1, c=False):
        super().__init__(sampling_rate, block_size)
        print(" [DDSP Model] Combtooth Subtractive Synthesiser")
        self.register_buffer("window", torch.sqrt(torch.hann_window(2 * block_size)))
        nb = int(block_size) + 1
        self.unit2ctrl = Unit2Control(n_unit, n_spk, {"harmonic_magnitude": nb, "harmonic_phase": nb,
                                                      "noise_magnitude": nb}, c)

    _comb_mode = COMB_SINC_GATED
    _front_wants = {}

    def _train_forward(self, ctx, ctrl, ps, f0_frames, nargs):
        B, Fr = ctrl.shape[0], ctrl.shape[1]
        nz, exc, seed = nargs
        signal = ctx.spectral_ola(ctrl.reshape(B * Fr, -1), ps["comb"], nz, exc, seed, B, Fr, self._hop)
        return (signal,), (ps["comb"],)

    def _train_backward(self, ctx, ctrl, saved, f0_frames, nargs, d_outs):
        (comb,) = saved
        B, Fr = ctrl.shape[0], ctrl.shape[1]
        nz, exc, seed = nargs
        return ctx.spectral_ola_bwd(ctrl.reshape(B * Fr, -1), comb, nz, exc, seed, _sum_grads(comb, *d_outs), B, Fr,
                                    self._hop)

    def synth_from_ctrl(self, ctx, ctrl, comb, noise=None, noise_seed=None, n_dev=None):
        B, Fr = ctrl.shape[0], ctrl.shape[1]
        if n_dev is None:
            nz, exc, seed = self._noise_args(noise, noise_seed)
            return ctx.spectral_ola(ctrl.reshape(B * Fr, -1), comb, nz, exc, seed, B, Fr, self._hop)
        ctx.ragged_crop_(n_dev, Fr, self._hop, comb)
        nz, exc, seed = self._ragged_noise(ctx, n_dev, B, Fr, noise, noise_seed)
        signal = ctx.spectral_ola(ctrl.reshape(B * Fr, -1), comb, nz, exc, seed, B, Fr, self._hop)
        ctx.ragged_crop_(n_dev, Fr, self._hop, signal)
        return signal

    def forward(self, units_frames, f0_frames, volume_frames, spk_id, spk_mix_dict=None, initial_phase=None,
                infer=True, noise=None, noise_seed=None, n_frames=None, **kwargs):
        if units_frames.shape[0] == 0:
            return self._empty_result(f0_frames, shared=True)
        if n_frames is not None:
            ctx, n_dev, units, f0, vol, ps = self._ragged_front(units_frames, f0_frames, volume_frames, n_frames,
                                                                initial_phase, infer, COMB_SINC_GATED)
            ctrl = self.unit2ctrl.forward_ragged(ctx, units, f0, ps["phase_frames"], vol, spk_id, spk_mix_dict, n_dev)
            signal = self.synth_from_ctrl(ctx, ctrl, ps["comb"], noise, noise_seed, n_dev)
            pf = ctx.ragged_frames(ps["phase_frames"], n_dev, hold=False, out=ps["phase_frames"])
            return signal, pf.unsqueeze(-1), (signal, signal)
        if self._training_graph():
            pf, signal = _SynthTrainFn.apply(self, units_frames, f0_frames, volume_frames, spk_id, spk_mix_dict,
                                             initial_phase, infer, noise, noise_seed, *self.unit2ctrl.parameters())
            return signal, pf.unsqueeze(-1), (signal, signal)
        ctx, ps = self._front(f0_frames, initial_phase, infer, COMB_SINC_GATED)
        ctrl = self.unit2ctrl.forward_flat(units_frames, f0_frames, ps["phase_frames"], volume_frames, spk_id,
                                           spk_mix_dict)
        signal = self.synth_from_ctrl(ctx, ctrl, ps["comb"], noise, noise_seed)
        return signal, ps["phase_frames"].unsqueeze(-1), (signal, signal)
```

### ddsp-svc-official_amd/hipddsp/__init__.py

```python
import ctypes
import numbers
import os
import threading

import torch

_HERE = os.path.dirname(os.path.abspath(__file__))
LIB_PATH = os.path.join(_HERE, "libddsp_amd.so")

DDSP_OK, DDSP_ERR_ARG, DDSP_ERR_HIP, DDSP_ERR_OOM = 0, -1, -2, -3

COMB_NONE, COMB_SINC, COMB_SINC_GATED = 0, 1, 2
FIR_ALLPASS, FIR_DYNAMIC, FIR_STATIC = 0, 1, 2
EXC_AUDIO, EXC_UNIT_NOISE, EXC_GENERATE = 0, 1, 2
FIR_FP32, FIR_SPLIT_BF16 = 0, 3
ABI_VERSION = 7
MATH_FP32, MATH_SPLIT_BF16 = 0, 3
ATTENTION_CAUSAL = 200
ATTENTION_PAIR = 100

_c = ctypes
_vp, _i64, _u64, _int, _f32, _f64 = _c.c_void_p, _c.c_int64, _c.c_uint64, _c.c_int, _c.c_float, _c.c_double


class U2CWeights(_c.Structure):
    _fields_ = (
        [(n, _vp) for n in ("prenet_conv1_w", "prenet_conv1_b", "prenet_gn_w", "prenet_gn_b",
                            "prenet_conv2_w", "prenet_conv2_b",
                            "f0_w", "f0_b", "phase_w", "phase_b", "volume_w", "volume_b", "spk_table")]
        + [("n_spk", _int), ("n_unit", _int), ("n_out", _int), ("causal", _int)]
        + [(f"l{i}_{n}", _vp) for i in range(3) for n in (
            "norm_w", "norm_b", "q_w", "q_b", "k_w", "k_b", "v_w", "v_b", "proj", "out_w", "out_b",
            "cm_ln_w", "cm_ln_b", "cm_pw1_w", "cm_pw1_b", "cm_dw_w", "cm_dw_b", "cm_pw2_w", "cm_pw2_b")]
        + [(n, _vp) for n in ("final_ln_w", "final_ln_b", "head_g", "head_v", "head_b")]
        + [("version", _c.c_uint64)]
    )


HUBERT_LAYER_FIELDS = ("in_proj_w", "in_proj_b", "out_proj_w", "out_proj_b", "linear1_w", "linear1_b", "linear2_w",
                       "linear2_b", "norm1_w", "norm1_b", "norm2_w", "norm2_b")


class HubertWeights(_c.Structure):
    _fields_ = (
        [(n, _vp) for n in ("conv0_w", "norm0_w", "norm0_b")]
        + [(f"conv{i + 1}_w", _vp) for i in range(6)]
        + [(n, _vp) for n in ("fp_norm_w", "fp_norm_b", "fp_proj_w", "fp_proj_b", "pos_b", "pos_g", "pos_v", "norm_w", "norm_b")]
        + [(f"l{i}_{n}", _vp) for i in range(12) for n in HUBERT_LAYER_FIELDS]
        + [(n, _vp) for n in ("proj_w", "proj_b")]
        + [("version", _c.c_uint64)]
    )


class CrepeWeights(_c.Structure):
    _fields_ = (
        [(f"{n}{i + 1}_{s}", _vp) for n, s in (("conv", "w"), ("conv", "b"), ("bn", "w"), ("bn", "b"), ("bn", "mean"),
                                                 ("bn", "var")) for i in range(6)]
        + [("cls_w", _vp), ("cls_b", _vp)]
        + [("width", _int * 6)]
        + [("version", _c.c_uint64)]
    )


class WeightTable:

    def __init__(self, struct_cls, named_tensors, owner, copy=False, grad_uncached=False, **ints):
        self.struct_cls, self.named_tensors, self.owner = struct_cls, named_tensors, owner
        self.copy, self.grad_uncached, self.ints = copy, grad_uncached, ints
        self.invalidate()

    def invalidate(self):
        self._slots = self._ws = None
        self._nonce = int.from_bytes(os.urandom(6), "little") << 16

    def struct(self, module):
        if self._slots is None:
            by_id = {id(t): (d, k) for mod in module.modules() for d in (mod._parameters, mod._buffers)
                     for k, t in d.items() if t is not None}
            self._slots = [(name,) + by_id[id(t)] for name, t in self.named_tensors(module)]
        tensors = [d[k] for _, d, k in self._slots]
        uncached = self.grad_uncached and torch.is_grad_enabled()
        key = (uncached,) + tuple([(t.data_ptr(), t._version) for t in tensors])
        if self._ws is not None and self._ws[0] == key:
            return self._ws[1], self._ws[2]
        w = self.struct_cls(**self.ints)
        keep = []
        for (name, _, _), t in zip(self._slots, tensors):
            if not t.is_cuda:
                raise RuntimeError(f"{self.owner} parameters must live on a HIP device (no CPU fallback)")
            t = t.detach()
            if not t.is_contiguous() or t.dtype != torch.float32:
                if not self.copy:
                    raise ValueError(f"{self.owner} parameters must be contiguous fp32")
                t = t.contiguous().float()
            keep.append(t)
            setattr(w, name, t.data_ptr())
        w.version = 0 if uncached else (self._nonce + 1 + sum(int(t._version) for t in tensors)) & ((1 << 64) - 1)
        if all(a.data_ptr() == b.data_ptr() for a, b in zip(keep, tensors)):
            self._ws = (key, w, keep)
        return w, keep


class ProfEntry(_c.Structure):
    _fields_ = [("family", _int), ("name", _c.c_char * 36), ("launches", _i64), ("ms_total", _c.c_double),
                ("flops_total", _c.c_double), ("bytes_total", _c.c_double)]


CONV_X_SPLIT, CONV_ACT_SPLIT = 1, 2


def presplit(w):
    if w.dtype != torch.float32 or w.shape[-1] % 8:
        raise ValueError("presplit: fp32 with a multiple of 8 columns")
    g = w.contiguous().reshape(*w.shape[:-1], w.shape[-1] // 8, 8)
    hi = g.to(torch.bfloat16)
    lo = (g - hi.float()).to(torch.bfloat16)
    return torch.cat([hi, lo], dim=-1).contiguous().view(torch.float32).reshape(w.shape)


FAMILIES = ["phase_scan", "fir_act", "fir_dft_gemm", "ltv_fir", "u2c_prep", "u2c_gemm_conv3", "u2c_gemm_linear",
            "u2c_gemm_feat", "u2c_gemm_ctx", "u2c_gemm_attnout", "u2c_rowwise", "sins_bank", "spectral_ola", "rss_loss",
            "sola", "upsample", "other", "ltv_fir_bwd", "fir_synth_bwd", "u2c_bwd", "optim"]

SIGNATURES = {
    "ddsp_abi_version": (_int, []),
    "ddsp_ctx_create": (_int, [_c.POINTER(_vp), _int]),
    "ddsp_ctx_destroy": (_int, [_vp]),
    "ddsp_last_error": (_c.c_char_p, [_vp]),
    "ddsp_ctx_reserve": (_int, [_vp, _u64]),
    "ddsp_ctx_poll_error": (_int, [_vp]),
    "ddsp_ctx_set_math": (_int, [_vp, _int]),
    "ddsp_ctx_get_math": (_int, [_vp]),
    "ddsp_upsample": (_int, [_vp, _vp, _vp, _i64, _i64, _i64, _int, _vp]),
    "ddsp_phase_scan": (_int, [_vp, _vp, _vp, _vp, _i64, _i64, _int, _int, _int, _int, _vp, _vp, _vp, _vp, _vp]),
    "ddsp_fir_from_ctrl": (_int, [_vp, _vp, _int, _vp, _i64, _int, _vp, _i64, _int, _vp]),
    "ddsp_ltv_fir_bwd": (_int, [_vp, _vp, _vp, _int, _u64, _vp, _vp, _i64, _i64, _int, _int, _vp, _vp]),
    "ddsp_fir_from_ctrl_bwd": (_int, [_vp, _vp, _int, _vp, _i64, _int, _vp, _i64, _int, _vp, _vp, _i64]),
    "ddsp_sins_bank": (_int, [_vp, _vp, _vp, _i64, _int, _vp, _vp, _i64, _i64, _int, _int, _vp]),
    "ddsp_spectral_ola": (_int, [_vp, _vp, _vp, _i64, _vp, _vp, _int, _u64, _i64, _i64, _int, _vp]),
    "ddsp_sins_bank_bwd": (_int, [_vp, _vp, _vp, _i64, _int, _vp, _vp, _vp, _i64, _i64, _int, _int, _vp, _i64]),
    "ddsp_spectral_ola_bwd": (_int, [_vp, _vp, _vp, _i64, _vp, _vp, _int, _u64, _vp, _i64, _i64, _int, _vp, _i64]),
    "ddsp_rss_loss": (_int, [_vp, _vp, _vp, _vp, _i64, _i64, _c.POINTER(_int), _c.POINTER(_int), _int, _f32, _f32, _vp, _vp]),
    "ddsp_sola": (_int, [_vp, _vp, _vp, _i64, _int, _int, _int, _int, _vp, _vp, _vp]),
    "ddsp_volume_gate": (_int, [_vp, _vp, _vp, _vp, _f32, _i64, _i64, _int]),
    "ddsp_phase_vocoder": (_int, [_vp, _vp, _vp, _vp, _vp, _vp, _int, _vp]),
    "ddsp_volume_extract": (_int, [_vp, _vp, _vp, _i64, _i64, _int, _vp]),
    "ddsp_volume_extract_frac": (_int, [_vp, _vp, _vp, _i64, _i64, _f64, _vp]),
    "ddsp_align_units": (_int, [_vp, _vp, _vp, _i64, _i64, _i64, _i64, _f32, _vp]),
    "ddsp_gemm_res_ln": (_int, [_vp, _vp, _vp, _vp, _vp, _vp, _vp, _vp, _int, _int, _vp, _vp, _int]),
    "ddsp_conv1d_pair_supported": (_int, [_vp, _int, _int, _int]),
    "ddsp_conv1d_pair": (_int, [_vp, _vp, _vp, _vp, _vp, _vp, _vp, _i64, _int, _int, _int, _f32, _vp, _vp]),
    "ddsp_retime_f0": (_int, [_vp, _vp, _vp, _i64, _f64, _f64, _f32, _f64, _i64, _vp]),
    "ddsp_resample_length": (_i64, [_i64, _int, _int]),
    "ddsp_resample": (_int, [_vp, _vp, _vp, _i64, _i64, _int, _int, _int, _vp]),
    "ddsp_conv1d": (_int, [_vp, _vp, _vp, _vp, _vp, _i64, _int, _int, _int, _int, _f32, _vp, _vp, _vp, _f32, _vp, _int]),
    "ddsp_nsf_source": (_int, [_vp, _vp, _vp, _vp, _vp, _vp, _i64, _int, _int, _f32, _vp]),
    "ddsp_nsf_noise_conv": (_int, [_vp, _vp, _vp, _i64, _vp, _vp, _int, _int, _int, _int, _i64, _vp]),
    "ddsp_nsf_post": (_int, [_vp, _vp, _vp, _vp, _vp, _i64, _int, _int, _f32, _vp]),
    "ddsp_nsf_mean": (_int, [_vp, _vp, _vp, _vp, _vp, _int, _i64, _vp, _vp, _f32, _int]),
    "ddsp_log_mel": (_int, [_vp, _vp, _vp, _vp, _vp, _i64, _int, _int, _f32, _vp]),
    "ddsp_adamw_step": (_int, [_vp, _vp, _vp, _vp, _vp, _vp, _i64, _f32, _f32, _f32, _f32, _f32, _i64]),
    "ddsp_adamw_step_multi": (_int, [_vp, _vp, _int, _vp, _vp, _vp, _vp, _vp, _f32, _f32, _f32, _f32, _f32, _i64]),
    "ddsp_gemm_f32": (_int, [_vp, _vp, _vp, _i64, _int, _vp, _i64, _int, _vp, _vp, _i64, _int, _int, _int, _int, _int]),
    "ddsp_performer_attention": (_int, [_vp, _vp, _vp, _vp, _vp, _vp, _i64, _i64, _vp, _int]),
    "ddsp_hubert_frames": (_i64, [_i64]),
    "ddsp_hubert_soft_units": (_int, [_vp, _vp, _c.POINTER(HubertWeights), _vp, _i64, _i64, _vp]),
    "ddsp_hubert_encode": (_int, [_vp, _vp, _c.POINTER(HubertWeights), _vp, _i64, _i64, _int, _vp]),
    "ddsp_softmax_attention": (_int, [_vp, _vp, _vp, _vp, _vp, _i64, _i64, _int, _vp, _int]),
    "ddsp_hubert_soft_units_ragged": (_int, [_vp, _vp, _c.POINTER(HubertWeights), _vp, _i64, _i64, _vp, _vp]),
    "ddsp_hubert_encode_ragged": (_int, [_vp, _vp, _c.POINTER(HubertWeights), _vp, _i64, _i64, _vp, _int, _vp]),
    "ddsp_softmax_attention_ragged": (_int, [_vp, _vp, _vp, _vp, _vp, _i64, _i64, _int, _vp, _int, _vp]),
    "ddsp_resample_ragged": (_int, [_vp, _vp, _vp, _i64, _i64, _vp, _int, _int, _int, _vp]),
    "ddsp_align_units_ragged": (_int, [_vp, _vp, _vp, _i64, _i64, _i64, _i64, _f32, _vp, _vp, _vp]),
    "ddsp_conv1d_ragged": (_int, [_vp, _vp, _vp, _vp, _vp, _i64, _i64, _int, _int, _int, _int, _f32, _vp, _vp, _vp, _f32, _vp, _int,
                                  _vp, _int]),
    "ddsp_conv1d_pair_ragged": (_int, [_vp, _vp, _vp, _vp, _vp, _vp, _vp, _i64, _i64, _int, _int, _int, _f32, _vp, _vp, _vp, _int]),
    "ddsp_nsf_source_ragged": (_int, [_vp, _vp, _vp, _vp, _vp, _vp, _i64, _i64, _int, _int, _f32, _vp, _vp]),
    "ddsp_nsf_noise_conv_ragged": (_int, [_vp, _vp, _vp, _i64, _i64, _vp, _vp, _int, _int, _int, _int, _i64, _vp]),
    "ddsp_nsf_post_ragged": (_int, [_vp, _vp, _vp, _vp, _vp, _i64, _i64, _int, _int, _f32, _vp, _vp, _int]),
    "ddsp_stft_frames_ragged": (_int, [_vp, _vp, _vp, _i64, _i64, _vp, _int, _int, _i64, _vp]),
    "ddsp_retime_f0_ragged": (_int, [_vp, _vp, _vp, _i64, _i64, _vp, _f64, _f64, _f32, _f64, _i64, _vp, _vp]),
    "ddsp_volume_extract_ragged": (_int, [_vp, _vp, _vp, _i64, _i64, _vp, _int, _vp]),
    "ddsp_crepe_activations_ragged": (_int, [_vp, _vp, _c.POINTER(CrepeWeights), _vp, _i64, _i64, _vp, _vp, _i64, _int, _vp]),
    "ddsp_crepe_decode_ragged": (_int, [_vp, _vp, _vp, _i64, _i64, _vp, _f32, _f32, _i64, _u64, _int, _vp, _vp, _vp]),
    "ddsp_f0_postfilter_ragged": (_int, [_vp, _vp, _vp, _vp, _i64, _i64, _vp, _int, _f64, _i64, _vp, _f32, _int, _f32, _vp]),
    "ddsp_crepe_frames": (_i64, [_i64, _int]),
    "ddsp_crepe_activations": (_int, [_vp, _vp, _c.POINTER(CrepeWeights), _vp, _i64, _i64, _int, _vp]),
    "ddsp_crepe_decode": (_int, [_vp, _vp, _vp, _i64, _i64, _f32, _f32, _i64, _u64, _int, _vp, _vp, _vp]),
    "ddsp_crepe_decode_dseed": (_int, [_vp, _vp, _vp, _i64, _i64, _f32, _f32, _i64, _vp, _int, _vp, _vp, _vp]),
    "ddsp_stream_push": (_int, [_vp, _vp, _vp, _i64, _vp, _i64]),
    "ddsp_f0_postfilter": (_int, [_vp, _vp, _vp, _vp, _i64, _i64, _int, _f64, _i64, _i64, _f32, _int, _f32, _vp]),
    "ddsp_profile_begin": (_int, [_vp, _u64]),
    "ddsp_profile_mask": (_int, [_vp, _u64]),
    "ddsp_profile_end": (_int, [_vp, _c.POINTER(ProfEntry), _int, _c.POINTER(_int)]),
    "ddsp_unit2ctrl_fwd": (_int, [_vp, _vp, _c.POINTER(U2CWeights), _vp, _vp, _vp, _vp, _vp, _i64,
                                  _c.POINTER(_i64), _c.POINTER(_f32), _int, _i64, _i64, _vp]),
    "ddsp_unit2ctrl_bwd": (_int, [_vp, _vp, _c.POINTER(U2CWeights), _vp, _vp, _vp, _vp, _vp, _i64,
                                  _c.POINTER(_i64), _c.POINTER(_f32), _int, _i64, _i64, _vp, _c.POINTER(U2CWeights), _vp]),
    "ddsp_unit2ctrl_fwd_ragged": (_int, [_vp, _vp, _c.POINTER(U2CWeights), _vp, _vp, _vp, _vp, _vp, _i64,
                                         _c.POINTER(_i64), _c.POINTER(_f32), _int, _i64, _i64, _vp, _vp]),
    "ddsp_ragged_frames": (_int, [_vp, _vp, _vp, _vp, _i64, _i64, _i64, _int, _vp]),
    "ddsp_ragged_crop": (_int, [_vp, _vp, _vp, _vp, _vp, _vp, _i64, _i64, _int]),
    "ddsp_ragged_noise": (_int, [_vp, _vp, _vp, _u64, _vp, _i64, _i64, _int, _vp]),
    "ddsp_ltv_fir": (_int, [_vp, _vp, _vp, _int, _u64, _vp, _i64, _i64, _int, _int, _vp, _vp, _vp, _int]),
    "ddsp_unit2ctrl_keep_bytes": (_i64, [_c.POINTER(U2CWeights), _i64, _i64]),
    "ddsp_unit2ctrl_fwd_keep": (_int, [_vp, _vp, _c.POINTER(U2CWeights), _vp, _vp, _vp, _vp, _vp, _i64,
                                       _c.POINTER(_i64), _c.POINTER(_f32), _int, _i64, _i64, _vp, _i64, _vp]),
    "ddsp_unit2ctrl_bwd_kept": (_int, [_vp, _vp, _c.POINTER(U2CWeights), _vp, _vp, _vp, _vp, _vp, _i64,
                                       _c.POINTER(_i64), _c.POINTER(_f32), _int, _i64, _i64, _vp, _i64, _vp,
                                       _c.POINTER(U2CWeights)]),
}

_lib = None
_lib_lock = threading.Lock()


def load_library():
    global _lib
    with _lib_lock:
        if _lib is None:
            if not os.path.exists(LIB_PATH):
                raise RuntimeError(
                    f"{LIB_PATH} is missing: build it with `python ddsp-svc-official_amd/hipddsp/build.py` "
                    "(there is no CPU fallback for the synthesis path)")
            lib = ctypes.CDLL(LIB_PATH)
            for name, (res, args) in SIGNATURES.items():
                fn = getattr(lib, name)
                fn.restype = res
                fn.argtypes = args
            if lib.ddsp_abi_version() != ABI_VERSION:
                raise RuntimeError(f"{LIB_PATH} has ABI version {lib.ddsp_abi_version()}, this binding needs {ABI_VERSION}: "
                                   "rebuild it (`python ddsp-svc-official_amd/hipddsp/build.py`)")
            _lib = lib
    return _lib


def _check_counts(name, counts, B):
    if isinstance(counts, torch.Tensor):
        if counts.is_cuda:
            raise ValueError(f"{name} must be a CPU tensor or a sequence of ints (it is checked on the host)")
        if counts.dtype not in (torch.int8, torch.int16, torch.int32, torch.int64, torch.uint8) or counts.dim() != 1:
            raise ValueError(f"{name} must be an integer tensor of shape (B,), got {counts.dtype} {tuple(counts.shape)}")
        vals = counts.tolist()
    else:
        try:
            vals = list(counts)
        except TypeError:
            raise ValueError(f"{name} must be a sequence of B ints or a CPU integer tensor of shape (B,)") from None
        for v in vals:
            if isinstance(v, bool) or not isinstance(v, numbers.Integral):
                raise ValueError(f"{name} must hold ints, got {type(v).__name__} {v!r}")
        vals = [int(v) for v in vals]
    if len(vals) != int(B):
        raise ValueError(f"{name} must hold B={int(B)} counts, got {len(vals)}")
    return vals


def check_n_frames(n_frames, B, Fr):
    vals = _check_counts("n_frames", n_frames, B)
    for b, v in enumerate(vals):
        if not 1 <= v <= int(Fr):
            raise ValueError(f"n_frames[{b}] = {v} is outside 1..Fr={int(Fr)}")
    return vals


def check_n_samples(n_samples, B, T):
    vals = _check_counts("n_samples", n_samples, B)
    for b, v in enumerate(vals):
        if not 1 <= v <= int(T):
            raise ValueError(f"n_samples[{b}] = {v} is outside 1..T={int(T)}")
    return vals


def check_hubert_n_samples(n_samples, B, T):
    vals = check_n_samples(n_samples, B, T)
    for b, v in enumerate(vals):
        if hubert_frames(v) < 1:
            raise ValueError(f"n_samples[{b}] = {v} samples are too short for the conv stack")
    return vals


def check_crepe_n_samples(n_samples, B, T, hop=80):
    vals = check_n_samples(n_samples, B, T)
    for b, v in enumerate(vals):
        if crepe_frames(v, hop) < 3:
            raise ValueError(f"n_samples[{b}] = {v} samples at 16 kHz give {crepe_frames(v, hop)} CREPE frames; the "
                             "reflect-padded filters need at least 3")
    return vals


def check_volume_n_samples(n_samples, B, T, hop):
    vals = check_n_samples(n_samples, B, T)
    for b, v in enumerate(vals):
        if v <= (int(hop) + 1) // 2:
            raise ValueError(f"n_samples[{b}] = {v} samples are not longer than the reflect padding {(int(hop) + 1) // 2}")
    return vals


def _ptr(t):
    if t is None:
        return None
    if not t.is_cuda:
        raise RuntimeError("libddsp_amd needs device tensors (no CPU fallback)")
    if not t.is_contiguous():
        raise ValueError("libddsp_amd needs contiguous tensors")
    return t.data_ptr()


class Context:

    def __init__(self, device):
        self.lib = load_library()
        dev = torch.device(device)
        if dev.type != "cuda":
            raise RuntimeError("libddsp_amd runs on a HIP device only (no CPU fallback); got device=%r" % (device,))
        if not torch.cuda.is_available():
            raise RuntimeError("no HIP device visible: libddsp_amd cannot run (no CPU fallback)")
        self.device = torch.device("cuda", dev.index if dev.index is not None else torch.cuda.current_device())
        h = _vp()
        rc = self.lib.ddsp_ctx_create(ctypes.byref(h), self.device.index)
        if rc != DDSP_OK:
            raise RuntimeError(f"ddsp_ctx_create failed with {rc}")
        self.handle = h

    def __del__(self):
        try:
            if getattr(self, "handle", None):
                self.lib.ddsp_ctx_destroy(self.handle)
                self.handle = None
        except Exception:
            pass

    def _stream(self):
        s = torch.cuda.current_stream(self.device)
        last = getattr(self, "_last_stream", None)
        if last is not None and last != s and not torch.cuda.is_current_stream_capturing():
            s.wait_stream(last)
        self._last_stream = s
        return s.cuda_stream

    def _check(self, rc, what):
        if rc == DDSP_OK:
            return
        msg = self.lib.ddsp_last_error(self.handle)
        msg = msg.decode() if msg else ""
        if rc == DDSP_ERR_ARG:
            raise ValueError(f"{what}: {msg}")
        raise RuntimeError(f"{what} failed ({rc}): {msg}")

    def call(self, name, *args):
        if getattr(self, "_frozen", False):
            raise RuntimeError("this ddsp context belongs to a captured HIP graph (its scratch arena and tables are "
                               "referenced by the graph's kernels); use another context for eager calls")
        rc = getattr(self.lib, name)(self.handle, self._stream(), *args)
        self._check(rc, name)

    def freeze(self):
        self._frozen = True

    def poll_error(self):
        self._check(self.lib.ddsp_ctx_poll_error(self.handle), "ddsp_ctx_poll_error")

    @property
    def math(self):
        return self.lib.ddsp_ctx_get_math(self.handle)

    @property
    def fir_math(self):
        return FIR_FP32 if self.math == MATH_FP32 else FIR_SPLIT_BF16

    def set_math(self, math):
        self._check(self.lib.ddsp_ctx_set_math(self.handle, int(math)), "ddsp_ctx_set_math")

    def profile_begin(self, families=None):
        mask = 0
        for f in (families if families is not None else FAMILIES):
            mask |= 1 << FAMILIES.index(f)
        self._check(self.lib.ddsp_profile_begin(self.handle, mask), "ddsp_profile_begin")

    def profile_mask(self, families):
        mask = 0
        for f in families:
            mask |= 1 << FAMILIES.index(f)
        self._check(self.lib.ddsp_profile_mask(self.handle, mask), "ddsp_profile_mask")

    def profile_end(self):
        buf = (ProfEntry * 32)()
        n = _int(0)
        self._check(self.lib.ddsp_profile_end(self.handle, buf, 32, ctypes.byref(n)), "ddsp_profile_end")
        return {buf[i].name.decode(): {"launches": buf[i].launches, "ms_total": buf[i].ms_total,
                                       "flops_total": buf[i].flops_total, "bytes_total": buf[i].bytes_total}
                for i in range(n.value)}

    def upsample(self, x, hop):
        B, Fr, C = x.shape
        x = x.contiguous().float()
        out = torch.empty(B, Fr * hop, C, device=x.device, dtype=torch.float32)
        self.call("ddsp_upsample", _ptr(x), B, Fr, C, int(hop), _ptr(out))
        return out

    def phase_scan(self, f0_frames, hop, sr, initial_phase=None, precise=True, comb_mode=COMB_NONE,
                   want_rot=False, want_phase=False, want_f0=False):
        f0 = f0_frames.reshape(f0_frames.shape[0], -1).contiguous().float()
        B, Fr = f0.shape
        T = Fr * hop
        dev = f0.device
        mk = lambda: torch.empty(B, T, device=dev, dtype=torch.float32)
        rot = mk() if want_rot else None
        phase = mk() if want_phase else None
        comb = mk() if comb_mode != COMB_NONE else None
        f0_up = mk() if want_f0 else None
        pf = torch.empty(B, Fr, device=dev, dtype=torch.float32)
        ip = None if initial_phase is None else initial_phase.reshape(-1).contiguous().float()
        self.call("ddsp_phase_scan", _ptr(f0), _ptr(ip), B, Fr, int(hop), int(sr), 1 if precise else 0,
                  int(comb_mode), _ptr(rot), _ptr(phase), _ptr(comb), _ptr(f0_up), _ptr(pf))
        return {"rot": rot, "phase": phase, "comb": comb, "f0_up": f0_up, "phase_frames": pf}

    def unit2ctrl(self, weights, units, f0_frames, phase_frames, volume, spk_id, spk_mix_dict, n_out, n_frames=None):
        B, Fr, _ = units.shape
        dev = units.device
        units = units.contiguous().float()
        f0 = f0_frames.reshape(B, Fr).contiguous().float()
        ph = phase_frames.reshape(B, Fr).contiguous().float()
        vol = volume.reshape(B, Fr).contiguous().float()
        ctrl = torch.empty(B, Fr, n_out, device=dev, dtype=torch.float32)
        if spk_mix_dict is not None:
            n_mix = len(spk_mix_dict)
            ids = (_i64 * max(n_mix, 1))(*[int(k) for k in spk_mix_dict.keys()])
            ws = (_f32 * max(n_mix, 1))(*[float(v) for v in spk_mix_dict.values()])
            sid, n_sid = None, 0
        else:
            n_mix, ids, ws = 0, None, None
            sid = spk_id.reshape(-1).to(device=dev, dtype=torch.int64).contiguous()
            n_sid = sid.numel()
            if n_sid not in (1, B):
                raise ValueError(f"spk_id must hold 1 or B={B} ids, got {n_sid}")
        if n_frames is not None:
            self.call("ddsp_unit2ctrl_fwd_ragged", ctypes.byref(weights), _ptr(units), _ptr(f0), _ptr(ph), _ptr(vol), _ptr(sid),
                      n_sid, ids, ws, n_mix, B, Fr, _ptr(n_frames), _ptr(ctrl))
            return ctrl
        self.call("ddsp_unit2ctrl_fwd", ctypes.byref(weights), _ptr(units), _ptr(f0), _ptr(ph), _ptr(vol), _ptr(sid),
                  n_sid, ids, ws, n_mix, B, Fr, _ptr(ctrl))
        return ctrl

    def ragged_counts(self, counts):
        return torch.tensor(counts, dtype=torch.int32).to(self.device)

    @staticmethod
    def _counts_dev(t, B):
        if not (isinstance(t, torch.Tensor) and t.is_cuda and t.dtype == torch.int32 and t.numel() == B and t.is_contiguous()):
            raise ValueError("counts_dev must be a contiguous (B,) int32 device tensor (`ragged_counts`)")
        return t

    def ragged_frames(self, x, n_dev, hold, out=None):
        B, Fr = x.shape[0], x.shape[1]
        C = x.numel() // max(B * Fr, 1)
        if out is None:
            x = x.contiguous().float()
            out = torch.empty_like(x)
        elif x.dtype != torch.float32 or not x.is_contiguous() or out.data_ptr() != x.data_ptr():
            raise ValueError("ragged_frames: `out` is for the in-place call, out=x, on a contiguous fp32 tensor")
        self.call("ddsp_ragged_frames", _ptr(x), _ptr(n_dev), B, Fr, C, 1 if hold else 0, _ptr(out))
        return out

    def ragged_crop_(self, n_dev, Fr, hop, *signals):
        xs = [s for s in signals if s is not None]
        for s in xs:
            if s.dtype != torch.float32 or not s.is_contiguous() or s.dim() != 2 or s.shape[1] != int(Fr) * int(hop):
                raise ValueError("ragged_crop_: contiguous fp32 (B, Fr*hop) signals")
        for i in range(0, len(xs), 3):
            grp = xs[i:i + 3] + [None] * (3 - len(xs[i:i + 3]))
            self.call("ddsp_ragged_crop", _ptr(grp[0]), _ptr(grp[1]), _ptr(grp[2]), _ptr(n_dev), grp[0].shape[0], int(Fr), int(hop))

    def ragged_noise(self, noise, noise_seed, n_dev, B, Fr, hop):
        out = torch.empty(B, Fr * hop, device=self.device, dtype=torch.float32)
        if noise is not None:
            noise = noise.contiguous().float()
            if tuple(noise.shape) != (B, Fr * hop):
                raise ValueError(f"noise must be (B, Fr*hop) = {(B, Fr * hop)}, got {tuple(noise.shape)}")
        self.call("ddsp_ragged_noise", _ptr(noise), int(noise_seed) & ((1 << 64) - 1), _ptr(n_dev), B, Fr, int(hop), _ptr(out))
        return out

    def unit2ctrl_bwd(self, weights, grads, units, f0_frames, phase_frames, volume, spk_id, spk_mix_dict, n_out,
                      d_ctrl, want_ctrl=False):
        B, Fr, _ = units.shape
        dev = units.device
        units = units.contiguous().float()
        f0 = f0_frames.reshape(B, Fr).contiguous().float()
        ph = phase_frames.reshape(B, Fr).contiguous().float()
        vol = volume.reshape(B, Fr).contiguous().float()
        d_ctrl = d_ctrl.contiguous().float()
        ctrl = torch.empty(B, Fr, n_out, device=dev, dtype=torch.float32) if want_ctrl else None
        if spk_mix_dict is not None:
            n_mix = len(spk_mix_dict)
            ids = (_i64 * max(n_mix, 1))(*[int(k) for k in spk_mix_dict.keys()])
            ws = (_f32 * max(n_mix, 1))(*[float(v) for v in spk_mix_dict.values()])
            sid, n_sid = None, 0
        else:
            n_mix, ids, ws = 0, None, None
            sid = spk_id.reshape(-1).to(device=dev, dtype=torch.int64).contiguous()
            n_sid = sid.numel()
        self.call("ddsp_unit2ctrl_bwd", ctypes.byref(weights), _ptr(units), _ptr(f0), _ptr(ph), _ptr(vol), _ptr(sid),
                  n_sid, ids, ws, n_mix, B, Fr, _ptr(d_ctrl), ctypes.byref(grads), _ptr(ctrl))
        return ctrl

    def _u2c_inputs(self, units, f0_frames, phase_frames, volume, spk_id, spk_mix_dict):
        B, Fr, _ = units.shape
        dev = units.device
        units = units.contiguous().float()
        f0 = f0_frames.reshape(B, Fr).contiguous().float()
        ph = phase_frames.reshape(B, Fr).contiguous().float()
        vol = volume.reshape(B, Fr).contiguous().float()
        if spk_mix_dict is not None:
            n_mix = len(spk_mix_dict)
            ids = (_i64 * max(n_mix, 1))(*[int(k) for k in spk_mix_dict.keys()])
            ws = (_f32 * max(n_mix, 1))(*[float(v) for v in spk_mix_dict.values()])
            sid, n_sid = None, 0
        else:
            n_mix, ids, ws = 0, None, None
            sid = spk_id.reshape(-1).to(device=dev, dtype=torch.int64).contiguous()
            n_sid = sid.numel()
            if n_sid not in (1, B):
                raise ValueError(f"spk_id must hold 1 or B={B} ids, got {n_sid}")
        return (units, f0, ph, vol, sid), (_ptr(units), _ptr(f0), _ptr(ph), _ptr(vol), _ptr(sid), n_sid, ids, ws, n_mix, B, Fr)

    def unit2ctrl_keep(self, weights, units, f0_frames, phase_frames, volume, spk_id, spk_mix_dict, n_out):
        B, Fr, _ = units.shape
        nbytes = int(self.lib.ddsp_unit2ctrl_keep_bytes(ctypes.byref(weights), B, Fr))
        if nbytes < 0:
            raise ValueError("ddsp_unit2ctrl_keep_bytes: bad shape")
        keep = torch.empty(nbytes, device=units.device, dtype=torch.uint8)
        ctrl = torch.empty(B, Fr, n_out, device=units.device, dtype=torch.float32)
        hold, args = self._u2c_inputs(units, f0_frames, phase_frames, volume, spk_id, spk_mix_dict)
        self.call("ddsp_unit2ctrl_fwd_keep", ctypes.byref(weights), *args, _ptr(keep), nbytes, _ptr(ctrl))
        return ctrl, keep

    def unit2ctrl_bwd_kept(self, weights, grads, units, f0_frames, phase_frames, volume, spk_id, spk_mix_dict, keep, d_ctrl):
        d_ctrl = d_ctrl.contiguous().float()
        hold, args = self._u2c_inputs(units, f0_frames, phase_frames, volume, spk_id, spk_mix_dict)
        self.call("ddsp_unit2ctrl_bwd_kept", ctypes.byref(weights), *args, _ptr(keep), keep.numel(), _ptr(d_ctrl),
                  ctypes.byref(grads))

    def fir_from_ctrl(self, mode, ctrl2d, col0, n_mag, rows, sr, f0_frames=None):
        ld = ctrl2d.shape[-1]
        n = 2 * (n_mag - 1)
        ir = torch.empty(rows, n, device=ctrl2d.device, dtype=torch.float32)
        base = _ptr(ctrl2d) + 4 * col0
        f0 = None if f0_frames is None else f0_frames.reshape(-1).contiguous().float()
        self.call("ddsp_fir_from_ctrl", int(mode), base, ld, int(n_mag), _ptr(f0), rows, int(sr), _ptr(ir))
        return ir

    def ltv_fir(self, audio, ir, B, Fr, hop, excitation=EXC_AUDIO, noise_seed=0, add_in=None, want_out=True,
                math=FIR_FP32):
        n = ir.shape[-1]
        mk = lambda: torch.empty(B, Fr * hop, device=ir.device, dtype=torch.float32)
        out = mk() if want_out else None
        out_sum = mk() if add_in is not None else None
        self.call("ddsp_ltv_fir", _ptr(audio), int(excitation), int(noise_seed), _ptr(ir), B, Fr, int(hop), int(n),
                  _ptr(add_in), _ptr(out), _ptr(out_sum), int(math))
        return out, out_sum


    def ltv_fir_bwd(self, audio, ir, d_out, B, Fr, hop, excitation=EXC_AUDIO, noise_seed=0, want_d_audio=True,
                    want_d_ir=True):
        n = ir.shape[-1]
        d_out = d_out.contiguous().float()
        d_audio = torch.empty(B, Fr * hop, device=ir.device, dtype=torch.float32) if want_d_audio else None
        d_ir = torch.empty(B * Fr, n, device=ir.device, dtype=torch.float32) if want_d_ir else None
        self.call("ddsp_ltv_fir_bwd", _ptr(audio), int(excitation), int(noise_seed), _ptr(ir), _ptr(d_out), B, Fr,
                  int(hop), int(n), _ptr(d_audio), _ptr(d_ir))
        return d_audio, d_ir

    def fir_from_ctrl_bwd(self, mode, ctrl2d, col0, n_mag, rows, sr, d_ir, d_ctrl2d, f0_frames=None):
        f0 = None if f0_frames is None else f0_frames.reshape(-1).contiguous().float()
        self.call("ddsp_fir_from_ctrl_bwd", int(mode), _ptr(ctrl2d) + 4 * col0, ctrl2d.shape[-1], int(n_mag), _ptr(f0),
                  rows, int(sr), _ptr(d_ir), _ptr(d_ctrl2d) + 4 * col0, d_ctrl2d.shape[-1])

    def volume_extract(self, audio, hop, n_samples=None):
        audio = audio.contiguous().float()
        B, T = audio.shape
        if n_samples is not None:
            if not float(hop).is_integer():
                raise ValueError("volume_extract: a ragged batch needs an integral hop")
            vals = check_volume_n_samples(n_samples, B, T, int(hop))
            out = torch.empty(B, T // int(hop) + 1, device=audio.device, dtype=torch.float32)
            if B:
                n_dev = self.ragged_counts(vals)
                self.call("ddsp_volume_extract_ragged", _ptr(audio), B, T, _ptr(n_dev), int(hop), _ptr(out))
            return out
        if float(hop).is_integer():
            out = torch.empty(B, T // int(hop) + 1, device=audio.device, dtype=torch.float32)
            if B == 0:
                return out
            self.call("ddsp_volume_extract", _ptr(audio), B, T, int(hop), _ptr(out))
            return out
        hop = float(hop)
        out = torch.empty(B, int(T // hop) + 1, device=audio.device, dtype=torch.float32)
        self.call("ddsp_volume_extract_frac", _ptr(audio), B, T, hop, _ptr(out))
        return out

    def align_units(self, units, n_frames, ratio):
        units = units.contiguous().float()
        B, Lu, C = units.shape
        out = torch.empty(B, int(n_frames), C, device=units.device, dtype=torch.float32)
        if B == 0 or int(n_frames) == 0:
            return out
        self.call("ddsp_align_units", _ptr(units), B, Lu, C, int(n_frames), float(ratio), _ptr(out))
        return out

    def align_units_ragged(self, units, n_frames, ratio, n_units_dev, n_out_dev):
        units = units.contiguous().float()
        B, Lu, C = units.shape
        out = torch.empty(B, int(n_frames), C, device=units.device, dtype=torch.float32)
        if B == 0 or int(n_frames) == 0:
            return out
        self.call("ddsp_align_units_ragged", _ptr(units), B, Lu, C, int(n_frames), float(ratio), _ptr(n_units_dev),
                  _ptr(n_out_dev), _ptr(out))
        return out

    def retime_f0_ragged(self, f0, n_src_dev, step_num, div, scale, step_dst, n_dst, n_dst_dev):
        f0 = f0.contiguous().float()
        B, n_src = f0.shape
        out = torch.empty(B, int(n_dst), device=f0.device, dtype=torch.float32)
        self.call("ddsp_retime_f0_ragged", _ptr(f0), B, n_src, _ptr(n_src_dev), float(step_num), float(div), float(scale),
                  float(step_dst), int(n_dst), _ptr(n_dst_dev), _ptr(out))
        return out

    def retime_f0(self, f0, step_num, div, scale, step_dst, n_dst):
        f0 = f0.reshape(-1).contiguous().float()
        out = torch.empty(int(n_dst), device=f0.device, dtype=torch.float32)
        self.call("ddsp_retime_f0", _ptr(f0), f0.numel(), float(step_num), float(div), float(scale), float(step_dst), int(n_dst),
                  _ptr(out))
        return out

    def resample(self, audio, orig_freq, new_freq, lowpass_filter_width=6):
        flat = audio.dim() == 1
        x = (audio.reshape(1, -1) if flat else audio).contiguous().float()
        B, T = x.shape
        T_out = self.lib.ddsp_resample_length(T, int(orig_freq), int(new_freq))
        if T_out < 0:
            raise ValueError("resample: bad rates")
        out = torch.empty(B, T_out, device=x.device, dtype=torch.float32)
        if B and T:
            self.call("ddsp_resample", _ptr(x), B, T, int(orig_freq), int(new_freq), int(lowpass_filter_width), _ptr(out))
        return out[0] if flat else out

    def resample_ragged(self, audio, n_dev, orig_freq, new_freq, lowpass_filter_width=6):
        x = audio.contiguous().float()
        B, T = x.shape
        T_out = self.lib.ddsp_resample_length(T, int(orig_freq), int(new_freq))
        if T_out < 0:
            raise ValueError("resample: bad rates")
        out = torch.empty(B, T_out, device=x.device, dtype=torch.float32)
        if B and T:
            self.call("ddsp_resample_ragged", _ptr(x), B, T, _ptr(n_dev), int(orig_freq), int(new_freq),
                      int(lowpass_filter_width), _ptr(out))
        return out

    def conv1d(self, x, w_packed, bias, ktaps, dil, in_slope, residual=None, want_out=True, act_slope=None, w_split=None,
               x_split=False, act_split=False, rows=None):
        T, Cin = x.shape
        Cout = w_packed.shape[0]
        if w_packed.shape[1] != ktaps * Cin:
            raise ValueError("conv1d: packed weight does not match (ktaps, Cin)")
        out = torch.empty(T, Cout, device=x.device, dtype=torch.float32) if want_out else None
        act = torch.empty(T, Cout, device=x.device, dtype=torch.float32) if act_slope is not None else None
        if out is None and act is None:
            raise ValueError("conv1d: nothing to return")
        flags = (CONV_X_SPLIT if x_split else 0) | (CONV_ACT_SPLIT if act_split else 0)
        if rows is not None:
            B, n_dev, scale = rows
            if T % int(B):
                raise ValueError("conv1d: x must hold B rows of equal padded length")
            self.call("ddsp_conv1d_ragged", _ptr(x), _ptr(w_packed), _ptr(bias), int(B), T // int(B), Cin, Cout, int(ktaps), int(dil),
                      float(in_slope), _ptr(residual), _ptr(out), _ptr(act), float(act_slope if act_slope is not None else 1.0),
                      _ptr(w_split), flags, _ptr(n_dev), int(scale))
            return out if act_slope is None else (out, act)
        self.call("ddsp_conv1d", _ptr(x), _ptr(w_packed), _ptr(bias), T, Cin, Cout, int(ktaps), int(dil), float(in_slope),
                  _ptr(residual), _ptr(out), _ptr(act), float(act_slope if act_slope is not None else 1.0), _ptr(w_split), flags)
        return out if act_slope is None else (out, act)

    def gemm_res_ln(self, A_split, W_split, bias, res, gamma, beta, y_split=True, a_fp32=False):
        M, K = A_split.shape
        X = torch.empty(M, 256, device=A_split.device, dtype=torch.float32)
        Y = torch.empty(M, 256, device=A_split.device, dtype=torch.float32)
        self.call("ddsp_gemm_res_ln", _ptr(A_split), _ptr(W_split), _ptr(bias), _ptr(res), _ptr(gamma), _ptr(beta), int(M), int(K),
                  _ptr(X), _ptr(Y), (1 if y_split else 0) | (2 if a_fp32 else 0))
        return X, Y

    def conv1d_pair_supported(self, C, ktaps, dil):
        return bool(self.lib.ddsp_conv1d_pair_supported(self.handle, int(C), int(ktaps), int(dil)))

    def conv1d_pair(self, x, w1, b1, w2, b2, ktaps, dil, slope, want_out=True, want_act=False, rows=None):
        T, C = x.shape
        out = torch.empty(T, C, device=x.device, dtype=torch.float32) if want_out else None
        act = torch.empty(T, C, device=x.device, dtype=torch.float32) if want_act else None
        if rows is not None:
            B, n_dev, scale = rows
            if T % int(B):
                raise ValueError("conv1d_pair: x must hold B rows of equal padded length")
            self.call("ddsp_conv1d_pair_ragged", _ptr(x), _ptr(w1), _ptr(b1), _ptr(w2), _ptr(b2), int(B), T // int(B), C, int(ktaps),
                      int(dil), float(slope), _ptr(out), _ptr(act), _ptr(n_dev), int(scale))
            return out, act
        self.call("ddsp_conv1d_pair", _ptr(x), _ptr(w1), _ptr(b1), _ptr(w2), _ptr(b2), T, C, int(ktaps), int(dil), float(slope),
                  _ptr(out), _ptr(act))
        return out, act

    def nsf_source(self, f0, rand_ini, lin_w, lin_b, upp, sr, sine_amp=0.1):
        L = f0.numel()
        out = torch.empty(L * int(upp), device=f0.device, dtype=torch.float32)
        self.call("ddsp_nsf_source", _ptr(f0), _ptr(rand_ini.contiguous().float()), _ptr(lin_w), _ptr(lin_b), L, int(upp),
                  int(sr), float(sine_amp), _ptr(out))
        return out

    def nsf_source_ragged(self, f0, rand_ini, lin_w, lin_b, upp, sr, sine_amp=0.1, n_dev=None):
        B, L = f0.shape
        if tuple(rand_ini.shape) != (B, 9):
            raise ValueError(f"nsf_source_ragged: rand_ini must be (B, 9) = ({B}, 9), got {tuple(rand_ini.shape)}")
        out = torch.empty(B, L * int(upp), device=f0.device, dtype=torch.float32)
        self.call("ddsp_nsf_source_ragged", _ptr(f0), _ptr(rand_ini.contiguous().float()), _ptr(lin_w), _ptr(lin_b), B, L, int(upp),
                  int(sr), float(sine_amp), _ptr(n_dev), _ptr(out))
        return out

    def nsf_noise_conv_ragged(self, src, w, b, K, stride, pad, T_out):
        B, T_src = src.shape
        C = w.shape[0]
        out = torch.empty(B * int(T_out), C, device=src.device, dtype=torch.float32)
        self.call("ddsp_nsf_noise_conv_ragged", _ptr(src), B, T_src, _ptr(w), _ptr(b), C, int(K), int(stride), int(pad), int(T_out),
                  _ptr(out))
        return out

    def nsf_post_ragged(self, x, w, b, K, slope, rows):
        B, n_dev, scale = rows
        T, C = x.shape[0] // int(B), x.shape[1]
        out = torch.empty(int(B), T, device=x.device, dtype=torch.float32)
        self.call("ddsp_nsf_post_ragged", _ptr(x), _ptr(w), _ptr(b), int(B), T, C, int(K), float(slope), _ptr(out), _ptr(n_dev),
                  int(scale))
        return out

    def stft_frames_ragged(self, audio, n_dev, n_fft, hop, L):
        audio = audio.contiguous().float()
        B, T = audio.shape
        out = torch.empty(B, int(L), int(n_fft), device=audio.device, dtype=torch.float32)
        self.call("ddsp_stft_frames_ragged", _ptr(audio), B, T, _ptr(n_dev), int(n_fft), int(hop), int(L), _ptr(out))
        return out

    def nsf_noise_conv(self, src, w, b, K, stride, pad, T_out):
        C = w.shape[0]
        out = torch.empty(int(T_out), C, device=src.device, dtype=torch.float32)
        self.call("ddsp_nsf_noise_conv", _ptr(src), src.numel(), _ptr(w), _ptr(b), C, int(K), int(stride), int(pad),
                  int(T_out), _ptr(out))
        return out

    def nsf_post(self, x, w, b, K, slope):
        T, C = x.shape
        out = torch.empty(T, device=x.device, dtype=torch.float32)
        self.call("ddsp_nsf_post", _ptr(x), _ptr(w), _ptr(b), T, C, int(K), float(slope), _ptr(out))
        return out

    def nsf_mean(self, terms, want_out=True, act_slope=None, act_split=False):
        a = terms[0]
        out = torch.empty_like(a) if want_out else None
        act = torch.empty_like(a) if act_slope is not None else None
        b = terms[1] if len(terms) > 1 else None
        c = terms[2] if len(terms) > 2 else None
        self.call("ddsp_nsf_mean", _ptr(a), _ptr(b), _ptr(c), len(terms), a.numel(), _ptr(out), _ptr(act),
                  float(act_slope if act_slope is not None else 1.0), CONV_ACT_SPLIT if act_split else 0)
        return out if act_slope is None else (out, act)

    def log_mel(self, frames, dft_table, mel_basis, clip):
        n_frames, n_fft = frames.shape
        n_mels = mel_basis.shape[0]
        out = torch.empty(n_frames, n_mels, device=frames.device, dtype=torch.float32)
        self.call("ddsp_log_mel", _ptr(frames), _ptr(dft_table), _ptr(mel_basis), n_frames, n_fft, n_mels, float(clip), _ptr(out))
        return out

    def adamw_step(self, param, grad, exp_avg, exp_avg_sq, lr, beta1, beta2, eps, weight_decay, step):
        self.call("ddsp_adamw_step", _ptr(param), _ptr(grad), _ptr(exp_avg), _ptr(exp_avg_sq), param.numel(), float(lr),
                  float(beta1), float(beta2), float(eps), float(weight_decay), int(step))

    def adamw_step_multi(self, params, grads, exp_avgs, exp_avg_sqs, lr, beta1, beta2, eps, weight_decay, step):
        n = len(params)
        if not (len(grads) == len(exp_avgs) == len(exp_avg_sqs) == n):
            raise ValueError("adamw_step_multi: lists of different length")
        for t in (*params, *grads, *exp_avgs, *exp_avg_sqs):
            if t.dtype != torch.float32:
                raise ValueError("adamw_step_multi: fp32 tensors only")
        for p, g, m, v in zip(params, grads, exp_avgs, exp_avg_sqs):
            if not (g.numel() == m.numel() == v.numel() == p.numel()):
                raise ValueError("adamw_step_multi: a tensor and its state differ in size")
        arr = lambda ts: (_vp * n)(*[_ptr(t) for t in ts])
        numel = (_i64 * n)(*[p.numel() for p in params])
        self.call("ddsp_adamw_step_multi", n, arr(params), arr(grads), arr(exp_avgs), arr(exp_avg_sqs), numel, float(lr),
                  float(beta1), float(beta2), float(eps), float(weight_decay), int(step))

    def gemm(self, A, B, bias=None, a_k_contig=True, b_k_contig=True, tile=0, variant=0, out=None):
        M, K = (A.shape if a_k_contig else A.shape[::-1])
        N = B.shape[0] if b_k_contig else B.shape[1]
        C = torch.empty(M, N, device=A.device, dtype=torch.float32) if out is None else out
        if C.shape != (M, N) or C.dtype != torch.float32 or not C.is_contiguous():
            raise ValueError("gemm: `out` must be a contiguous fp32 (M, N) matrix")
        for t in (A, B):
            if not t.is_cuda or t.stride(1) != 1 or t.dtype != torch.float32:
                raise ValueError("gemm operands must be fp32 device matrices with unit inner stride")
        self.call("ddsp_gemm_f32", A.data_ptr(), A.stride(0), int(a_k_contig), B.data_ptr(), B.stride(0), int(b_k_contig),
                  _ptr(bias), _ptr(C), N, M, N, K, int(tile), int(variant))
        return C

    def performer_attention(self, q, k, v, proj, B, Fr, math=MATH_SPLIT_BF16):
        out = torch.empty(B * Fr, 512, device=q.device, dtype=torch.float32)
        self.call("ddsp_performer_attention", _ptr(q), _ptr(k), _ptr(v), _ptr(proj), int(B), int(Fr), _ptr(out), int(math))
        return out

    def softmax_attention(self, q, k, v, B, L, heads, math=MATH_SPLIT_BF16):
        out = torch.empty(B * L, heads * 64, device=q.device, dtype=torch.float32)
        self.call("ddsp_softmax_attention", _ptr(q), _ptr(k), _ptr(v), int(B), int(L), int(heads), _ptr(out), int(math))
        return out

    def softmax_attention_ragged(self, q, k, v, B, L, heads, n_keys_dev, math=MATH_SPLIT_BF16, out=None):
        if out is None:
            out = torch.empty(B * L, heads * 64, device=q.device, dtype=torch.float32)
        elif out.dtype != torch.float32 or tuple(out.shape) != (B * L, heads * 64):
            raise ValueError("softmax_attention_ragged: `out` must be fp32 (B*L, heads*64)")
        self.call("ddsp_softmax_attention_ragged", _ptr(q), _ptr(k), _ptr(v), int(B), int(L), int(heads), _ptr(out), int(math),
                  _ptr(n_keys_dev))
        return out

    def hubert_units(self, weights, wav, n_dev=None):
        B, T = wav.shape
        Fr = hubert_frames(T)
        if Fr <= 0:
            raise ValueError(f"hubert: {T} samples are too short for the conv stack")
        wav = wav.contiguous().float()
        out = torch.empty(B, Fr, 256, device=wav.device, dtype=torch.float32)
        if B and n_dev is not None:
            self.call("ddsp_hubert_soft_units_ragged", ctypes.byref(weights), _ptr(wav), int(B), int(T), _ptr(n_dev), _ptr(out))
        elif B:
            self.call("ddsp_hubert_soft_units", ctypes.byref(weights), _ptr(wav), int(B), int(T), _ptr(out))
        return out

    def hubert_encode(self, weights, wav, layer, n_dev=None):
        B, T = wav.shape
        Fr = hubert_frames(T)
        if Fr <= 0:
            raise ValueError(f"hubert: {T} samples are too short for the conv stack")
        wav = wav.contiguous().float()
        out = torch.empty(B, Fr, 512 if layer == -1 else 768, device=wav.device, dtype=torch.float32)
        if B and n_dev is not None:
            self.call("ddsp_hubert_encode_ragged", ctypes.byref(weights), _ptr(wav), int(B), int(T), _ptr(n_dev), int(layer),
                      _ptr(out))
        elif B:
            self.call("ddsp_hubert_encode", ctypes.byref(weights), _ptr(wav), int(B), int(T), int(layer), _ptr(out))
        return out

    def crepe_activations(self, weights, audio16, hop=80, n_samples=None, counts_dev=None):
        B, T = audio16.shape
        Fr = crepe_frames(T, hop)
        x = audio16.contiguous().float()
        if n_samples is not None:
            vals = check_crepe_n_samples(n_samples, B, T, hop)
            table = crepe_ragged_table(vals, hop)
            if counts_dev is None:
                counts_dev = self.ragged_counts(table)
            elif counts_dev.dtype != torch.int32 or counts_dev.numel() != 2 * B + 1 or not counts_dev.is_contiguous():
                raise ValueError("crepe_activations: counts_dev must be the (2B + 1,) int32 upload of crepe_ragged_table")
            out = torch.empty(B, Fr, 360, device=x.device, dtype=torch.float32)
            if B:
                self.call("ddsp_crepe_activations_ragged", ctypes.byref(weights), _ptr(x), int(B), int(T), _ptr(counts_dev),
                          _ptr(counts_dev) + 4 * B, int(table[-1]), int(hop), _ptr(out))
            return out
        out = torch.empty(B, Fr, 360, device=x.device, dtype=torch.float32)
        if B:
            self.call("ddsp_crepe_activations", ctypes.byref(weights), _ptr(x), int(B), int(T), int(hop), _ptr(out))
        return out

    def crepe_decode(self, probs, fmin, fmax, segment=512, dither_seed=0, dither=False, want_bins=False, seed_dev=None,
                     n_frames=None, counts_dev=None):
        p = probs.contiguous().float()
        B, Fr, _ = p.shape
        if n_frames is not None:
            if seed_dev is not None:
                raise ValueError("crepe_decode: seed_dev is not available with n_frames (a ragged batch)")
            vals = check_n_frames(n_frames, B, Fr)
            n_dev = self._counts_dev(counts_dev, B) if counts_dev is not None else self.ragged_counts(vals)
            f0 = torch.empty(B, Fr, device=p.device, dtype=torch.float32)
            pd = torch.empty_like(f0)
            bins = torch.empty(B, Fr, device=p.device, dtype=torch.int32) if want_bins else None
            if B and Fr:
                self.call("ddsp_crepe_decode_ragged", _ptr(p), int(B), int(Fr), _ptr(n_dev), float(fmin), float(fmax),
                          int(segment), int(dither_seed) & ((1 << 64) - 1), 1 if dither else 0, _ptr(f0), _ptr(pd), _ptr(bins))
            return (f0, pd, bins) if want_bins else (f0, pd)
        f0 = torch.empty(B, Fr, device=p.device, dtype=torch.float32)
        pd = torch.empty_like(f0)
        bins = torch.empty(B, Fr, device=p.device, dtype=torch.int32) if want_bins else None
        if seed_dev is not None and (seed_dev.dtype != torch.int64 or seed_dev.numel() != 1 or seed_dev.device != p.device):
            raise ValueError("crepe_decode: seed_dev must be a (1,) int64 tensor on the device of probs")
        if B and Fr and seed_dev is not None:
            self.call("ddsp_crepe_decode_dseed", _ptr(p), int(B), int(Fr), float(fmin), float(fmax), int(segment),
                      _ptr(seed_dev), 1 if dither else 0, _ptr(f0), _ptr(pd), _ptr(bins))
        elif B and Fr:
            self.call("ddsp_crepe_decode", _ptr(p), int(B), int(Fr), float(fmin), float(fmax), int(segment),
                      int(dither_seed) & ((1 << 64) - 1), 1 if dither else 0, _ptr(f0), _ptr(pd), _ptr(bins))
        return (f0, pd, bins) if want_bins else (f0, pd)

    def f0_postfilter(self, f0, pd, sr, hop, n_frames, start_frame=0, threshold=0.05, uv_interp=False, f0_min=65.0,
                      n_crepe=None, n_out=None, counts_dev=None):
        f0 = f0.contiguous().float()
        pd = pd.contiguous().float()
        B, Fr = f0.shape
        if pd.shape != f0.shape:
            raise ValueError("f0_postfilter: f0 and pd must have the same shape")
        if (n_crepe is None) != (n_out is None):
            raise ValueError("f0_postfilter: a ragged batch needs both n_crepe and n_out")
        if n_crepe is not None:
            if int(start_frame) != 0:
                raise ValueError("f0_postfilter: start_frame must be 0 with n_crepe / n_out (a ragged batch)")
            vals = []
            for name, c, lo, hi in (("n_crepe", n_crepe, 3, Fr), ("n_out", n_out, 1, int(n_frames))):
                vals.append(_check_counts(name, c, B))
                for b, v in enumerate(vals[-1]):
                    if not lo <= v <= hi:
                        raise ValueError(f"{name}[{b}] = {v} is outside {lo}..{hi}")
            if counts_dev is not None:
                nc, no = (self._counts_dev(c, B) for c in counts_dev)
            else:
                nc, no = self.ragged_counts(vals[0] + vals[1]).reshape(2, B)
            out = torch.empty(B, int(n_frames), device=f0.device, dtype=torch.float32)
            if B:
                self.call("ddsp_f0_postfilter_ragged", _ptr(f0), _ptr(pd), int(B), int(Fr), _ptr(nc), int(sr), float(hop),
                          int(n_frames), _ptr(no), float(threshold), 1 if uv_interp else 0, float(f0_min), _ptr(out))
            return out
        out = torch.empty(B, int(n_frames), device=f0.device, dtype=torch.float32)
        if B:
            self.call("ddsp_f0_postfilter", _ptr(f0), _ptr(pd), int(B), int(Fr), int(sr), float(hop), int(n_frames),
                      int(start_frame), float(threshold), 1 if uv_interp else 0, float(f0_min), _ptr(out))
        return out

    def sins_bank(self, ctrl2d, col0, n_harmonics, f0_frames, phase, B, Fr, hop, sr):
        out = torch.empty(B, Fr * hop, device=ctrl2d.device, dtype=torch.float32)
        f0 = f0_frames.reshape(-1).contiguous().float()
        self.call("ddsp_sins_bank", _ptr(ctrl2d) + 4 * col0, ctrl2d.shape[-1], int(n_harmonics), _ptr(f0), _ptr(phase),
                  B, Fr, int(hop), int(sr), _ptr(out))
        return out

    def spectral_ola(self, ctrl2d, comb, noise, excitation, noise_seed, B, Fr, hop):
        out = torch.empty(B, Fr * hop, device=ctrl2d.device, dtype=torch.float32)
        self.call("ddsp_spectral_ola", _ptr(ctrl2d), ctrl2d.shape[-1], _ptr(comb), _ptr(noise), int(excitation),
                  int(noise_seed), B, Fr, int(hop), _ptr(out))
        return out

    def sins_bank_bwd(self, ctrl2d, col0, n_harmonics, f0_frames, phase, d_out, B, Fr, hop, sr, d_ctrl2d):
        f0 = f0_frames.reshape(-1).contiguous().float()
        self.call("ddsp_sins_bank_bwd", _ptr(ctrl2d) + 4 * col0, ctrl2d.shape[-1], int(n_harmonics), _ptr(f0),
                  _ptr(phase), _ptr(d_out.contiguous()), B, Fr, int(hop), int(sr), _ptr(d_ctrl2d) + 4 * col0,
                  d_ctrl2d.shape[-1])

    def spectral_ola_bwd(self, ctrl2d, comb, noise, excitation, noise_seed, d_out, B, Fr, hop):
        d_ctrl = torch.empty_like(ctrl2d)
        self.call("ddsp_spectral_ola_bwd", _ptr(ctrl2d), ctrl2d.shape[-1], _ptr(comb), _ptr(noise), int(excitation),
                  int(noise_seed), _ptr(d_out.contiguous()), B, Fr, int(hop), _ptr(d_ctrl), d_ctrl.shape[-1])
        return d_ctrl

    def rss_loss(self, x_pred, x_true, n_ffts, alpha=1.0, eps=1e-7, want_grad=False, hops=None):
        xp = x_pred.detach().contiguous().float()
        xt = x_true.detach().contiguous().float()
        B, T = xp.shape
        if xt.shape != xp.shape:
            raise ValueError(f"x_pred {tuple(xp.shape)} and x_true {tuple(xt.shape)} must have the same shape")
        if T % 4:
            raise ValueError("signal length must be a multiple of 4")
        arr = (_int * len(n_ffts))(*[int(n) for n in n_ffts])
        if hops is not None and len(hops) != len(n_ffts):
            raise ValueError("one hop per scale")
        harr = (_int * len(n_ffts))(*[int(h) for h in hops]) if hops is not None else None
        loss = torch.empty(1, device=xp.device, dtype=torch.float32)
        grad = torch.empty_like(xp) if want_grad else None
        self.call("ddsp_rss_loss", _ptr(xp), _ptr(xt), B, T, arr, harr, len(n_ffts), float(alpha), float(eps), _ptr(loss),
                  _ptr(grad))
        return loss, grad

    def sola(self, audio, sola_buffer, block, xfade, search, delay):
        audio = audio.contiguous().float()
        emitted = torch.empty(block, device=audio.device, dtype=torch.float32)
        shift = torch.empty(1, device=audio.device, dtype=torch.int32)
        self.call("ddsp_sola", _ptr(audio), audio.numel(), int(block), int(xfade), int(search), int(delay),
                  _ptr(sola_buffer), _ptr(emitted), _ptr(shift))
        return emitted, shift

    def stream_push_(self, window, block_in):
        if window.dtype != torch.float32 or block_in.dtype != torch.float32 or window.dim() != 1 or block_in.dim() != 1:
            raise ValueError("stream_push_: window and block_in must be 1-D fp32 tensors")
        self.call("ddsp_stream_push", _ptr(window), window.numel(), _ptr(block_in), block_in.numel())
        return window

    def phase_vocoder(self, a, b, fade_out, fade_in):
        a, b = a.contiguous().float(), b.contiguous().float()
        fo, fi = fade_out.contiguous().float(), fade_in.contiguous().float()
        n = a.numel()
        if not (b.numel() == fo.numel() == fi.numel() == n):
            raise ValueError("phase_vocoder: a, b and the fade windows must have the same length")
        out = torch.empty(n, device=a.device, dtype=torch.float32)
        self.call("ddsp_phase_vocoder", _ptr(a), _ptr(b), _ptr(fo), _ptr(fi), n, _ptr(out))
        return out

    def volume_gate_(self, signal, volume, threshold_db, hop):
        B, T = signal.shape
        vol = volume.reshape(B, -1).contiguous().float()
        self.call("ddsp_volume_gate", _ptr(signal), _ptr(vol), float(10 ** (float(threshold_db) / 20)), B,
                  vol.shape[1], int(hop))
        return signal


_contexts = {}
_ctx_lock = threading.Lock()


_override = threading.local()


def next_dither_seed(seed):
    return (int(seed) * 6364136223846793005 + 1442695040888963407) & ((1 << 64) - 1)


def hubert_frames(T):
    return int(load_library().ddsp_hubert_frames(int(T)))


def crepe_frames(T16, hop=80):
    n = int(load_library().ddsp_crepe_frames(int(T16), int(hop)))
    if n < 0:
        raise ValueError(f"crepe_frames: bad length {T16} or hop {hop}")
    return n


def crepe_ragged_table(n16, hop=80):
    prefix = [0]
    for v in n16:
        prefix.append(prefix[-1] + crepe_frames(v, hop))
    return list(n16) + prefix


class use_context:

    def __init__(self, ctx):
        self.ctx = ctx

    def __enter__(self):
        self.prev = getattr(_override, "ctx", None)
        _override.ctx = self.ctx
        return self.ctx

    def __exit__(self, *exc):
        _override.ctx = self.prev
        return False


def context_for(device):
    dev = torch.device(device)
    idx = dev.index if dev.index is not None else (torch.cuda.current_device() if torch.cuda.is_available() else 0)
    forced = getattr(_override, "ctx", None)
    if forced is not None and dev.type == "cuda" and forced.device.index == idx:
        return forced
    key = (dev.type, idx, threading.get_ident())
    with _ctx_lock:
        ctx = _contexts.get(key)
        if ctx is None:
            ctx = Context(torch.device(dev.type, idx) if dev.type == "cuda" else dev)
            _contexts[key] = ctx
    return ctx
```

### include/ddsp_amd.h

```cpp
#ifndef DDSP_AMD_H
#define DDSP_AMD_H

#include <stdint.h>

#ifdef __cplusplus
extern "C" {
#endif

#define DDSP_OK 0
#define DDSP_ERR_ARG (-1)
#define DDSP_ERR_HIP (-2)
#define DDSP_ERR_OOM (-3)

typedef struct ddsp_ctx ddsp_ctx;

int ddsp_ctx_create(ddsp_ctx** out, int device);
int ddsp_ctx_destroy(ddsp_ctx* ctx);
const char* ddsp_last_error(const ddsp_ctx* ctx);
int ddsp_ctx_reserve(ddsp_ctx* ctx, uint64_t bytes);
int ddsp_abi_version(void);
int ddsp_ctx_poll_error(ddsp_ctx* ctx);
#define DDSP_MATH_FP32 0
#define DDSP_MATH_SPLIT_BF16 3
int ddsp_ctx_set_math(ddsp_ctx* ctx, int math);
int ddsp_ctx_get_math(const ddsp_ctx* ctx);

int ddsp_upsample(ddsp_ctx* ctx, void* stream, const float* x, int64_t B, int64_t Fr, int64_t C, int hop,
                  float* out);

#define DDSP_COMB_NONE 0
#define DDSP_COMB_SINC 1
#define DDSP_COMB_SINC_GATED 2
int ddsp_phase_scan(ddsp_ctx* ctx, void* stream, const float* f0_frames, const float* initial_phase, int64_t B,
                    int64_t Fr, int hop, int sr, int precise, int comb_mode, float* rot, float* phase, float* comb,
                    float* f0_up, float* phase_frames);

#define DDSP_FIR_ALLPASS 0
#define DDSP_FIR_DYNAMIC 1
#define DDSP_FIR_STATIC 2
int ddsp_fir_from_ctrl(ddsp_ctx* ctx, void* stream, int mode, const float* ctrl, int64_t ctrl_ld, int n_mag,
                       const float* f0_frames, int64_t rows, int sr, float* ir);

#define DDSP_FIR_FP32 0
#define DDSP_FIR_SPLIT_BF16 3
#define DDSP_EXC_AUDIO 0
#define DDSP_EXC_UNIT_NOISE 1
#define DDSP_EXC_GENERATE 2
int ddsp_ltv_fir(ddsp_ctx* ctx, void* stream, const float* audio, int excitation, uint64_t noise_seed,
                 const float* ir, int64_t B, int64_t Fr, int hop, int n, const float* add_in, float* out,
                 float* out_sum, int math);


typedef struct ddsp_u2c_layer {
    const float *norm_w, *norm_b, *q_w, *q_b, *k_w, *k_b, *v_w, *v_b, *proj, *out_w, *out_b;
    const float *cm_ln_w, *cm_ln_b, *cm_pw1_w, *cm_pw1_b, *cm_dw_w, *cm_dw_b, *cm_pw2_w, *cm_pw2_b;
} ddsp_u2c_layer;

typedef struct ddsp_u2c_weights {
    const float *prenet_conv1_w, *prenet_conv1_b, *prenet_gn_w, *prenet_gn_b, *prenet_conv2_w, *prenet_conv2_b;
    const float *f0_w, *f0_b, *phase_w, *phase_b, *volume_w, *volume_b, *spk_table;
    int n_spk, n_unit, n_out;
    int causal;
    ddsp_u2c_layer layer[3];
    const float *final_ln_w, *final_ln_b, *head_g, *head_v, *head_b;
    uint64_t version;
} ddsp_u2c_weights;

int ddsp_unit2ctrl_fwd(ddsp_ctx* ctx, void* stream, const ddsp_u2c_weights* weights_host, const float* units,
                       const float* f0_frames, const float* phase_frames, const float* volume,
                       const int64_t* spk_id, int64_t n_spk_id, const int64_t* mix_ids_host,
                       const float* mix_w_host, int n_mix, int64_t B, int64_t Fr, float* ctrl);

int ddsp_unit2ctrl_fwd_ragged(ddsp_ctx* ctx, void* stream, const ddsp_u2c_weights* weights_host, const float* units,
                              const float* f0_frames, const float* phase_frames, const float* volume,
                              const int64_t* spk_id, int64_t n_spk_id, const int64_t* mix_ids_host,
                              const float* mix_w_host, int n_mix, int64_t B, int64_t Fr, const int32_t* n_frames,
                              float* ctrl);
int ddsp_ragged_frames(ddsp_ctx* ctx, void* stream, const float* src, const int32_t* n_frames, int64_t B, int64_t Fr,
                       int64_t C, int hold, float* dst);
int ddsp_ragged_crop(ddsp_ctx* ctx, void* stream, float* x0, float* x1, float* x2, const int32_t* n_frames, int64_t B,
                     int64_t Fr, int hop);
int ddsp_ragged_noise(ddsp_ctx* ctx, void* stream, const float* noise, uint64_t noise_seed, const int32_t* n_frames,
                      int64_t B, int64_t Fr, int hop, float* out);

int ddsp_unit2ctrl_bwd(ddsp_ctx* ctx, void* stream, const ddsp_u2c_weights* weights_host, const float* units,
                       const float* f0_frames, const float* phase_frames, const float* volume,
                       const int64_t* spk_id, int64_t n_spk_id, const int64_t* mix_ids_host,
                       const float* mix_w_host, int n_mix, int64_t B, int64_t Fr, const float* d_ctrl,
                       const ddsp_u2c_weights* grads_host, float* ctrl_out);

int64_t ddsp_unit2ctrl_keep_bytes(const ddsp_u2c_weights* w, int64_t B, int64_t Fr);
int ddsp_unit2ctrl_fwd_keep(ddsp_ctx* ctx, void* stream, const ddsp_u2c_weights* w, const float* units,
                            const float* f0_frames, const float* phase_frames, const float* volume,
                            const int64_t* spk_id, int64_t n_spk_id, const int64_t* mix_ids_host,
                            const float* mix_w_host, int n_mix, int64_t B, int64_t Fr, void* keep, int64_t keep_bytes,
                            float* ctrl);
int ddsp_unit2ctrl_bwd_kept(ddsp_ctx* ctx, void* stream, const ddsp_u2c_weights* w, const float* units,
                            const float* f0_frames, const float* phase_frames, const float* volume,
                            const int64_t* spk_id, int64_t n_spk_id, const int64_t* mix_ids_host,
                            const float* mix_w_host, int n_mix, int64_t B, int64_t Fr, void* keep, int64_t keep_bytes,
                            const float* d_ctrl, const ddsp_u2c_weights* grads_host);

int ddsp_ltv_fir_bwd(ddsp_ctx* ctx, void* stream, const float* audio, int excitation, uint64_t noise_seed,
                     const float* ir, const float* d_out, int64_t B, int64_t Fr, int hop, int n, float* d_audio,
                     float* d_ir);
int ddsp_fir_from_ctrl_bwd(ddsp_ctx* ctx, void* stream, int mode, const float* ctrl, int64_t ctrl_ld, int n_mag,
                           const float* f0_frames, int64_t rows, int sr, float* d_ir, float* d_ctrl,
                           int64_t d_ctrl_ld);

int ddsp_sins_bank(ddsp_ctx* ctx, void* stream, const float* ctrl, int64_t ctrl_ld, int n_harmonics,
                   const float* f0_frames, const float* phase, int64_t B, int64_t Fr, int hop, int sr, float* out);

int ddsp_spectral_ola(ddsp_ctx* ctx, void* stream, const float* ctrl, int64_t ctrl_ld, const float* comb,
                      const float* noise, int excitation, uint64_t noise_seed, int64_t B, int64_t Fr, int hop,
                      float* out);

int ddsp_sins_bank_bwd(ddsp_ctx* ctx, void* stream, const float* ctrl, int64_t ctrl_ld, int n_harmonics,
                       const float* f0_frames, const float* phase, const float* d_out, int64_t B, int64_t Fr, int hop,
                       int sr, float* d_ctrl, int64_t d_ctrl_ld);
int ddsp_spectral_ola_bwd(ddsp_ctx* ctx, void* stream, const float* ctrl, int64_t ctrl_ld, const float* comb,
                          const float* noise, int excitation, uint64_t noise_seed, const float* d_out, int64_t B,
                          int64_t Fr, int hop, float* d_ctrl, int64_t d_ctrl_ld);

int ddsp_rss_loss(ddsp_ctx* ctx, void* stream, const float* x_pred, const float* x_true, int64_t B, int64_t T,
                  const int* n_ffts_host, const int* hops_host, int n_scale, float alpha, float eps, float* loss,
                  float* grad_pred);

int ddsp_sola(ddsp_ctx* ctx, void* stream, const float* audio, int64_t n_audio, int block, int xfade, int search,
              int delay, float* sola_buffer, float* emitted, int* shift);

int ddsp_stream_push(ddsp_ctx* ctx, void* stream, float* window, int64_t n_in, const float* block_in, int64_t block);

int ddsp_phase_vocoder(ddsp_ctx* ctx, void* stream, const float* a, const float* b, const float* fade_out,
                       const float* fade_in, int n, float* out);

int ddsp_volume_gate(ddsp_ctx* ctx, void* stream, float* signal, const float* volume, float threshold, int64_t B,
                     int64_t Fr, int hop);

int ddsp_volume_extract(ddsp_ctx* ctx, void* stream, const float* audio, int64_t B, int64_t T, int hop,
                        float* volume);
int ddsp_volume_extract_ragged(ddsp_ctx* ctx, void* stream, const float* audio, int64_t B, int64_t T,
                               const int32_t* n_samples, int hop, float* volume);
int ddsp_volume_extract_frac(ddsp_ctx* ctx, void* stream, const float* audio, int64_t B, int64_t T, double hop_size,
                             float* volume);
int ddsp_align_units(ddsp_ctx* ctx, void* stream, const float* units, int64_t B, int64_t Lu, int64_t C,
                     int64_t n_frames, float ratio, float* out);
int ddsp_align_units_ragged(ddsp_ctx* ctx, void* stream, const float* units, int64_t B, int64_t Lu, int64_t C,
                            int64_t n_frames, float ratio, const int32_t* n_units, const int32_t* n_out, float* out);

int ddsp_retime_f0(ddsp_ctx* ctx, void* stream, const float* f0, int64_t n_src, double step_num, double div, float scale,
                   double step_dst, int64_t n_dst, float* out);
int ddsp_retime_f0_ragged(ddsp_ctx* ctx, void* stream, const float* f0, int64_t B, int64_t n_src, const int32_t* n_src_rows,
                          double step_num, double div, float scale, double step_dst, int64_t n_dst, const int32_t* n_dst_rows,
                          float* out);

int64_t ddsp_resample_length(int64_t T, int orig_freq, int new_freq);
int ddsp_resample(ddsp_ctx* ctx, void* stream, const float* x, int64_t B, int64_t T, int orig_freq, int new_freq,
                  int lowpass_filter_width, float* out);
int ddsp_resample_ragged(ddsp_ctx* ctx, void* stream, const float* x, int64_t B, int64_t T, const int32_t* n_samples,
                         int orig_freq, int new_freq, int lowpass_filter_width, float* out);

#define DDSP_CONV_X_SPLIT 1
#define DDSP_CONV_ACT_SPLIT 2
int ddsp_conv1d(ddsp_ctx* ctx, void* stream, const float* x, const float* w_packed, const float* bias, int64_t T, int Cin,
                int Cout, int ktaps, int dil, float in_slope, const float* residual, float* out, float* out_act,
                float act_slope, const float* w_split, int flags);
int ddsp_conv1d_pair_supported(ddsp_ctx* ctx, int C, int ktaps, int dil);
int ddsp_conv1d_pair(ddsp_ctx* ctx, void* stream, const float* x, const float* w1, const float* b1, const float* w2,
                     const float* b2, int64_t T, int C, int ktaps, int dil, float slope, float* out, float* out_act);

int ddsp_nsf_source(ddsp_ctx* ctx, void* stream, const float* f0, const float* rand_ini, const float* lin_w,
                    const float* lin_b, int64_t L, int upp, int sr, float sine_amp, float* out);
int ddsp_nsf_noise_conv(ddsp_ctx* ctx, void* stream, const float* src, int64_t T_src, const float* w, const float* b, int C,
                        int K, int stride, int pad, int64_t T_out, float* out);
int ddsp_nsf_post(ddsp_ctx* ctx, void* stream, const float* x, const float* w, const float* b, int64_t T, int C, int K,
                  float slope, float* out);
int ddsp_nsf_mean(ddsp_ctx* ctx, void* stream, const float* a, const float* b, const float* c, int n_terms, int64_t n,
                  float* out, float* out_act, float act_slope, int flags);
int ddsp_log_mel(ddsp_ctx* ctx, void* stream, const float* frames, const float* dft_table, const float* mel_basis,
                 int64_t n_frames, int n_fft, int n_mels, float clip, float* out);
int ddsp_conv1d_ragged(ddsp_ctx* ctx, void* stream, const float* x, const float* w_packed, const float* bias, int64_t B, int64_t T,
                       int Cin, int Cout, int ktaps, int dil, float in_slope, const float* residual, float* out, float* out_act,
                       float act_slope, const float* w_split, int flags, const int32_t* n_frames, int frame_scale);
int ddsp_conv1d_pair_ragged(ddsp_ctx* ctx, void* stream, const float* x, const float* w1, const float* b1, const float* w2,
                            const float* b2, int64_t B, int64_t T, int C, int ktaps, int dil, float slope, float* out,
                            float* out_act, const int32_t* n_frames, int frame_scale);
int ddsp_nsf_source_ragged(ddsp_ctx* ctx, void* stream, const float* f0, const float* rand_ini, const float* lin_w,
                           const float* lin_b, int64_t B, int64_t L, int upp, int sr, float sine_amp, const int32_t* n_frames,
                           float* out);
int ddsp_nsf_noise_conv_ragged(ddsp_ctx* ctx, void* stream, const float* src, int64_t B, int64_t T_src, const float* w,
                               const float* b, int C, int K, int stride, int pad, int64_t T_out, float* out);
int ddsp_nsf_post_ragged(ddsp_ctx* ctx, void* stream, const float* x, const float* w, const float* b, int64_t B, int64_t T, int C,
                         int K, float slope, float* out, const int32_t* n_frames, int frame_scale);
int ddsp_stft_frames_ragged(ddsp_ctx* ctx, void* stream, const float* audio, int64_t B, int64_t T, const int32_t* n_samples,
                            int n_fft, int hop, int64_t L, float* out);

int ddsp_adamw_step(ddsp_ctx* ctx, void* stream, float* param, const float* grad, float* exp_avg, float* exp_avg_sq,
                    int64_t n, float lr, float beta1, float beta2, float eps, float weight_decay, int64_t step);
int ddsp_adamw_step_multi(ddsp_ctx* ctx, void* stream, int n_tensors, float* const* params, const float* const* grads,
                          float* const* exp_avg, float* const* exp_avg_sq, const int64_t* numel, float lr,
                          float beta1, float beta2, float eps, float weight_decay, int64_t step);

int ddsp_gemm_f32(ddsp_ctx* ctx, void* stream, const float* A, int64_t lda, int a_k_contig, const float* B,
                  int64_t ldb, int b_k_contig, const float* bias, float* C, int64_t ldc, int M, int N, int K, int tile,
                  int variant);

int ddsp_gemm_res_ln(ddsp_ctx* ctx, void* stream, const float* A_split, const float* W_split, const float* bias,
                     const float* res, const float* gamma, const float* beta, int M, int K, float* X, float* Y, int y_split);

#define DDSP_ATTENTION_CAUSAL 200
#define DDSP_ATTENTION_PAIR 100
int ddsp_performer_attention(ddsp_ctx* ctx, void* stream, const float* q, const float* k, const float* v,
                             const float* proj, int64_t B, int64_t Fr, float* out, int math);

typedef struct ddsp_hubert_layer {
    const float *in_proj_w, *in_proj_b, *out_proj_w, *out_proj_b, *linear1_w, *linear1_b, *linear2_w, *linear2_b;
    const float *norm1_w, *norm1_b, *norm2_w, *norm2_b;
} ddsp_hubert_layer;

typedef struct ddsp_hubert_weights {
    const float *conv0_w, *norm0_w, *norm0_b;
    const float* conv_w[6];
    const float *fp_norm_w, *fp_norm_b, *fp_proj_w, *fp_proj_b;
    const float *pos_b, *pos_g, *pos_v;
    const float *norm_w, *norm_b;
    ddsp_hubert_layer layer[12];
    const float *proj_w, *proj_b;
    uint64_t version;
} ddsp_hubert_weights;

int64_t ddsp_hubert_frames(int64_t T);
int ddsp_hubert_soft_units(ddsp_ctx* ctx, void* stream, const ddsp_hubert_weights* w, const float* wav, int64_t B, int64_t T,
                           float* units);
int ddsp_hubert_encode(ddsp_ctx* ctx, void* stream, const ddsp_hubert_weights* w, const float* wav, int64_t B, int64_t T,
                       int layer, float* out);
int ddsp_softmax_attention(ddsp_ctx* ctx, void* stream, const float* q, const float* k, const float* v, int64_t B, int64_t L,
                           int heads, float* out, int math);

int ddsp_hubert_soft_units_ragged(ddsp_ctx* ctx, void* stream, const ddsp_hubert_weights* w, const float* wav, int64_t B,
                                  int64_t T, const int32_t* n_samples, float* units);
int ddsp_hubert_encode_ragged(ddsp_ctx* ctx, void* stream, const ddsp_hubert_weights* w, const float* wav, int64_t B, int64_t T,
                              const int32_t* n_samples, int layer, float* out);
int ddsp_softmax_attention_ragged(ddsp_ctx* ctx, void* stream, const float* q, const float* k, const float* v, int64_t B,
                                  int64_t L, int heads, float* out, int math, const int32_t* n_keys);

typedef struct ddsp_crepe_weights {
    const float* conv_w[6];
    const float* conv_b[6];
    const float* bn_w[6];
    const float* bn_b[6];
    const float* bn_mean[6];
    const float* bn_var[6];
    const float *cls_w, *cls_b;
    int width[6];
    uint64_t version;
} ddsp_crepe_weights;

int64_t ddsp_crepe_frames(int64_t T16, int hop);
int ddsp_crepe_activations(ddsp_ctx* ctx, void* stream, const ddsp_crepe_weights* w, const float* audio16, int64_t B, int64_t T,
                           int hop, float* probs);
int ddsp_crepe_decode(ddsp_ctx* ctx, void* stream, const float* probs, int64_t B, int64_t Fr, float fmin, float fmax,
                      int64_t segment, uint64_t dither_seed, int use_dither, float* f0, float* periodicity, int32_t* bins);
int ddsp_crepe_decode_dseed(ddsp_ctx* ctx, void* stream, const float* probs, int64_t B, int64_t Fr, float fmin, float fmax,
                            int64_t segment, uint64_t* seed_dev, int use_dither, float* f0, float* periodicity, int32_t* bins);
int ddsp_f0_postfilter(ddsp_ctx* ctx, void* stream, const float* f0, const float* pd, int64_t B, int64_t Fr, int sr, double hop,
                       int64_t n_frames, int64_t start_frame, float threshold, int uv_interp, float f0_min, float* out);

int ddsp_crepe_activations_ragged(ddsp_ctx* ctx, void* stream, const ddsp_crepe_weights* w, const float* audio16, int64_t B,
                                  int64_t T, const int32_t* n_samples, const int32_t* frame_prefix, int64_t n_packed, int hop,
                                  float* probs);
int ddsp_crepe_decode_ragged(ddsp_ctx* ctx, void* stream, const float* probs, int64_t B, int64_t Fr, const int32_t* n_frames,
                             float fmin, float fmax, int64_t segment, uint64_t dither_seed, int use_dither, float* f0,
                             float* periodicity, int32_t* bins);
int ddsp_f0_postfilter_ragged(ddsp_ctx* ctx, void* stream, const float* f0, const float* pd, int64_t B, int64_t Fr,
                              const int32_t* n_crepe, int sr, double hop, int64_t n_frames, const int32_t* n_out,
                              float threshold, int uv_interp, float f0_min, float* out);

typedef struct ddsp_prof_entry {
    int family;
    char name[36];
    int64_t launches;
    double ms_total;
    double flops_total;
    double bytes_total;
} ddsp_prof_entry;
int ddsp_profile_begin(ddsp_ctx* ctx, uint64_t family_mask);
int ddsp_profile_mask(ddsp_ctx* ctx, uint64_t family_mask);
int ddsp_profile_end(ddsp_ctx* ctx, ddsp_prof_entry* out, int max_entries, int* n_entries);

#ifdef __cplusplus
}
#endif
#endif
```

Measured before the change: 5.287 billion samples/s.

## Batch three FIR activation launches and use even/odd half-table all-pass DFT

Adds a combined entry point that computes the activations for all three FIR filters (all-pass, dynamic, static) in one segmented kernel launch instead of three. For the all-pass filter it uses a half-size inverse-DFT table whose two halves of K accumulate separately in a split-K MFMA kernel, and the epilogue forms the mirrored taps as e+o and e-o. This roughly halves the all-pass GEMM output width and removes launch overhead. The cost is more code paths, a new table kind, and an extra accumulator set that raises register pressure in the split-K kernel. It also adds a fallback that routes pre-split operands to the DMA kernel.

Result: faster. 5.429 billion samples/s (median of 6 runs) (+2.7%).

```diff
diff --git a/ddsp-svc-official_amd/csrc/fir_synth.hip b/ddsp-svc-official_amd/csrc/fir_synth.hip
--- a/ddsp-svc-official_amd/csrc/fir_synth.hip
+++ b/ddsp-svc-official_amd/csrc/fir_synth.hip
@@ -97,11 +97,22 @@
     }
 };
 
-
-__global__ void __launch_bounds__(256) fir_act_exp8_kernel(float scale, const float* __restrict__ ctrl, int64_t ld, int M, int ldo,
-                                                           int64_t rows, float* __restrict__ out, int split) {
+struct EpiEvenOdd {
+    float* ir;
+    int n;
+    __device__ __forceinline__ float col(int) const { return 0.f; }
+    __device__ __forceinline__ void operator()(int, int m, int t, float e, float o) const {
+        float* row = ir + (int64_t)m * n;
+        row[t] = e + o;
+        if (t > 0 && t < n / 2) row[n - t] = e - o;
+    }
+};
+
+
+__device__ __forceinline__ void fir_act_exp8_block(unsigned block, float scale, const float* __restrict__ ctrl, int64_t ld, int M, int ldo,
+                                                   int64_t rows, float* __restrict__ out, int split) {
     const int per_row = M / 8;
-    const int64_t i = (int64_t)blockIdx.x * 256 + threadIdx.x;
+    const int64_t i = (int64_t)block * 256 + threadIdx.x;
     if (i >= rows * per_row) return;
     const int64_t row = i / per_row;
     const int gq = (int)(i % per_row);
@@ -124,6 +135,10 @@
         *(f32x4*)(dst + 4) = f32x4{v[4], v[5], v[6], v[7]};
     }
 }
+__global__ void __launch_bounds__(256) fir_act_exp8_kernel(float scale, const float* __restrict__ ctrl, int64_t ld, int M, int ldo,
+                                                           int64_t rows, float* __restrict__ out, int split) {
+    fir_act_exp8_block(blockIdx.x, scale, ctrl, ld, M, ldo, rows, out, split);
+}
 
 template <int CTRL, int ROW_MASK>
 __device__ __forceinline__ double act_dpp_d(double v) {
@@ -132,10 +147,10 @@
     const int hi = __builtin_amdgcn_update_dpp(0, (int)(uint32_t)(u >> 32), CTRL, ROW_MASK, 0xf, false);
     return __builtin_bit_cast(double, ((uint64_t)(uint32_t)hi << 32) | (uint32_t)lo);
 }
-__global__ void __launch_bounds__(256) fir_act_allpass4_kernel(const float* __restrict__ ctrl, int64_t ld, int M, int ldo, int64_t rows,
-                                                               float* __restrict__ out, int split) {
+__device__ __forceinline__ void fir_act_allpass4_block(unsigned block, const float* __restrict__ ctrl, int64_t ld, int M, int ldo,
+                                                       int64_t rows, float* __restrict__ out, int split) {
     const int lane = threadIdx.x & 63;
-    const int64_t row = (int64_t)blockIdx.x * 4 + (threadIdx.x >> 6);
+    const int64_t row = (int64_t)block * 4 + (threadIdx.x >> 6);
     if (row >= rows) return;
     const float* src = ctrl + row * ld;
     float* dst = out + row * ldo;
@@ -186,6 +201,33 @@
             *(f32x4*)(dst + M + f) = sn;
         }
     }
+}
+__global__ void __launch_bounds__(256) fir_act_allpass4_kernel(const float* __restrict__ ctrl, int64_t ld, int M, int ldo, int64_t rows,
+                                                               float* __restrict__ out, int split) {
+    fir_act_allpass4_block(blockIdx.x, ctrl, ld, M, ldo, rows, out, split);
+}
+
+struct FirActSeg {
+    const float* ctrl;
+    float* out;
+    int M, ldo, mode, split;
+    unsigned blocks;
+};
+__global__ void __launch_bounds__(256) fir_act3_kernel(FirActSeg s0, FirActSeg s1, FirActSeg s2, int64_t ld, int64_t rows) {
+    unsigned b = blockIdx.x;
+    FirActSeg s = s0;
+    if (b >= s0.blocks) {
+        b -= s0.blocks;
+        s = s1;
+        if (b >= s1.blocks) {
+            b -= s1.blocks;
+            s = s2;
+        }
+    }
+    if (s.mode == DDSP_FIR_ALLPASS)
+        fir_act_allpass4_block(b, s.ctrl, ld, s.M, s.ldo, rows, s.out, s.split);
+    else
+        fir_act_exp8_block(b, s.mode == DDSP_FIR_STATIC ? 1.0f / 128.0f : 1.0f, s.ctrl, ld, s.M, s.ldo, rows, s.out, s.split);
 }
 
 __global__ void __launch_bounds__(256) repack_rows_kernel(const float* __restrict__ src, int n, int64_t rows, int ld,
@@ -277,6 +319,96 @@
 }
 
 
+namespace {
+
+struct FirPlan {
+    int mode, M, n, K, lda;
+    const float* ctrl;
+    float* ir;
+    bool tap_major, even_odd, presplit, wide;
+    float *tab, *tab_split;
+    float* act;
+};
+
+int fir_plan(ddsp_ctx* ctx, hipStream_t st, int mode, const float* ctrl, int64_t ctrl_ld, int n_mag, int64_t rows, float* ir,
+             FirPlan& p) {
+    p.mode = mode;
+    p.M = n_mag;
+    p.n = 2 * (n_mag - 1);
+    p.K = (mode == DDSP_FIR_ALLPASS) ? 2 * p.M : p.M;
+    p.lda = ddsp_pad4(p.K);
+    p.ctrl = ctrl;
+    p.ir = ir;
+    p.act = nullptr;
+    p.tap_major = p.K % 32 == 0;
+    p.even_odd = mode == DDSP_FIR_ALLPASS && p.tap_major && p.M % 32 == 0;
+    const int kind = mode == DDSP_FIR_ALLPASS ? (p.even_odd ? TAB_IRDFT_CPLX_HALF : TAB_IRDFT_CPLX)
+                                              : (mode == DDSP_FIR_STATIC ? TAB_IRDFT_RE_HANN : TAB_IRDFT_RE);
+    int rc = ddsp_get_table(ctx, st, kind, p.M, p.tap_major ? 1 : 0, &p.tab);
+    if (rc) return rc;
+    p.tab_split = nullptr;
+    if (p.tap_major && ctx->math != DDSP_MATH_FP32 && (rc = ddsp_get_table(ctx, st, kind, p.M, 2, &p.tab_split))) return rc;
+    p.presplit = p.tap_major && p.tab_split && rows >= 8192 && p.M % 8 == 0 && ctx->math != 4;
+    p.wide = p.M % 8 == 0 && ctrl_ld % 4 == 0 && p.lda % 8 == 0 && ((uintptr_t)ctrl % 16) == 0;
+    return DDSP_OK;
+}
+
+void fir_act_launch(hipStream_t st, const FirPlan& p, int64_t ctrl_ld, int64_t rows) {
+    if (p.wide && p.mode != DDSP_FIR_ALLPASS)
+        hipLaunchKernelGGL(fir_act_exp8_kernel, dim3((unsigned)ceil_div64(rows * (p.M / 8), 256)), dim3(256), 0, st,
+                           p.mode == DDSP_FIR_STATIC ? 1.0f / 128.0f : 1.0f, p.ctrl, ctrl_ld, p.M, p.lda, rows, p.act, p.presplit ? 1 : 0);
+    else if (p.wide)
+        hipLaunchKernelGGL(fir_act_allpass4_kernel, dim3((unsigned)ceil_div64(rows, 4)), dim3(256), 0, st, p.ctrl, ctrl_ld, p.M, p.lda,
+                           rows, p.act, p.presplit ? 1 : 0);
+    else
+        hipLaunchKernelGGL(fir_act_kernel, dim3((unsigned)ceil_div64(rows, 4)), dim3(256), 0, st, p.mode, p.ctrl, ctrl_ld, p.M,
+                           p.lda, rows, p.act, p.presplit ? 1 : 0);
+}
+
+void launch_even_odd(hipStream_t st, const gemm::Args& g, const EpiEvenOdd& epi) {
+    if (!gemm::dma_ok(g) || g.K % 64 != 0) {
+        ddsp_launch_refusal() = "even/odd all-pass operands do not qualify for the split-K LDS-DMA kernel";
+        return;
+    }
+    gemm::dma_go<64, 64, EpiEvenOdd, 3, 4, gemm::A_PLAIN, true>(st, g, 1, epi);
+}
+
+void fir_dft_launch(ddsp_ctx* ctx, hipStream_t st, const FirPlan& p, const float* f0_frames, int64_t rows, int sr) {
+    const int n = p.n, K = p.K;
+    auto prep = [&](gemm::Args& g) {
+        g.math = p.tap_major ? (ctx->math == 4 ? DDSP_MATH_SPLIT_BF16 : ctx->math) : 0;
+        g.B_split = p.tab_split;
+        if (p.presplit) {
+            g.A_split = 1;
+            g.B = p.tab_split;
+        }
+    };
+    auto run = [&](gemm::Args g, const auto& epi) {
+        prep(g);
+        if (p.tap_major)
+            gemm::launch<true, true, gemm::A_PLAIN>(st, g, 1, epi);
+        else
+            gemm::launch<true, false, gemm::A_PLAIN>(st, g, 1, epi);
+    };
+    const int64_t ldb = p.tap_major ? K : ddsp_pad4(n);
+    if (p.even_odd) {
+        gemm::Args g = gemm::make(p.act, p.lda, p.tab, ldb, (int)rows, n / 2 + 1, K);
+        prep(g);
+        launch_even_odd(st, g, EpiEvenOdd{p.ir, n});
+    } else if (p.mode == DDSP_FIR_ALLPASS) {
+        gemm::Args g = gemm::make(p.act, p.lda, p.tab, ldb, (int)rows, n, K);
+        run(g, gemm::EpiStore{p.ir, n, nullptr, 1, 0, 0});
+    } else {
+        gemm::Args g = gemm::make(p.act, p.lda, p.tab, ldb, (int)rows, n / 2 + 1, K);
+        if (p.mode == DDSP_FIR_DYNAMIC)
+            run(g, EpiDynWindow{p.ir, n, f0_frames, 1.5f * (float)sr, (p.tap_major && ctx->math != DDSP_MATH_FP32) ? 1 : 0});
+        else
+            run(g, EpiMirrorStore{p.ir, n});
+    }
+}
+
+}
+
 extern "C" int ddsp_fir_from_ctrl(ddsp_ctx* ctx, void* stream, int mode, const float* ctrl, int64_t ctrl_ld,
                                   int n_mag, const float* f0_frames, int64_t rows, int sr, float* ir) {
     DDSP_REQUIRE(ctx, ctx && ctrl && ir, "ddsp_fir_from_ctrl: null argument");
@@ -287,64 +419,80 @@
     if (rows == 0) return DDSP_OK;
     hipStream_t st = (hipStream_t)stream;
     DDSP_ENTER_DEVICE(ctx);
-    const int M = n_mag, n = 2 * (n_mag - 1);
-    const int K = (mode == DDSP_FIR_ALLPASS) ? 2 * M : M;
-    const int lda = ddsp_pad4(K);
-    int rc = ddsp_scratch_reserve_bytes(ctx, (size_t)rows * lda * sizeof(float) + 4096);
+    FirPlan p;
+    int rc = fir_plan(ctx, st, mode, ctrl, ctrl_ld, n_mag, rows, ir, p);
+    if (rc) return rc;
+    rc = ddsp_scratch_reserve_bytes(ctx, (size_t)rows * p.lda * sizeof(float) + 4096);
     if (rc) return rc;
     ddsp_scratch_reset(ctx);
-    float* act = nullptr;
-    rc = ddsp_scratch_get(ctx, (size_t)rows * lda * sizeof(float), (void**)&act);
+    rc = ddsp_scratch_get(ctx, (size_t)rows * p.lda * sizeof(float), (void**)&p.act);
     if (rc) return rc;
-    float* tab = nullptr;
-    const int kind = mode == DDSP_FIR_ALLPASS ? TAB_IRDFT_CPLX : (mode == DDSP_FIR_STATIC ? TAB_IRDFT_RE_HANN : TAB_IRDFT_RE);
-    const bool tap_major = K % 32 == 0;
-    rc = ddsp_get_table(ctx, st, kind, M, tap_major ? 1 : 0, &tab);
-    if (rc) return rc;
-    float* tab_split = nullptr;
-    if (tap_major && ctx->math != DDSP_MATH_FP32 && (rc = ddsp_get_table(ctx, st, kind, M, 2, &tab_split))) return rc;
-
-    const bool presplit = tap_major && tab_split && rows >= 8192 && M % 8 == 0 && ctx->math != 4;
     ddsp_prof_begin(ctx, st, PF_FIR_ACT);
-    const bool wide = M % 8 == 0 && ctrl_ld % 4 == 0 && lda % 8 == 0 && ((uintptr_t)ctrl % 16) == 0;
-    if (wide && mode != DDSP_FIR_ALLPASS)
-        hipLaunchKernelGGL(fir_act_exp8_kernel, dim3((unsigned)ceil_div64(rows * (M / 8), 256)), dim3(256), 0, st,
-                           mode == DDSP_FIR_STATIC ? 1.0f / 128.0f : 1.0f, ctrl, ctrl_ld, M, lda, rows, act, presplit ? 1 : 0);
-    else if (wide)
-        hipLaunchKernelGGL(fir_act_allpass4_kernel, dim3((unsigned)ceil_div64(rows, 4)), dim3(256), 0, st, ctrl, ctrl_ld, M, lda, rows,
-                           act, presplit ? 1 : 0);
-    else
-        hipLaunchKernelGGL(fir_act_kernel, dim3((unsigned)ceil_div64(rows, 4)), dim3(256), 0, st, mode, ctrl, ctrl_ld, M,
-                           lda, rows, act, presplit ? 1 : 0);
-    ddsp_prof_end(ctx, st, 0.0, 4.0 * rows * (M + K));
+    fir_act_launch(st, p, ctrl_ld, rows);
+    ddsp_prof_end(ctx, st, 0.0, 4.0 * rows * (p.M + p.K));
     DDSP_LAUNCH_CHECK(ctx);
     ddsp_prof_begin(ctx, st, PF_FIR_DFT_GEMM);
-
-    auto run = [&](gemm::Args g, const auto& epi) {
-        g.math = tap_major ? (ctx->math == 4 ? DDSP_MATH_SPLIT_BF16 : ctx->math) : 0;
-        g.B_split = tab_split;
-        if (presplit) {
-            g.A_split = 1;
-            g.B = tab_split;
-        }
-        if (tap_major)
-            gemm::launch<true, true, gemm::A_PLAIN>(st, g, 1, epi);
-        else
-            gemm::launch<true, false, gemm::A_PLAIN>(st, g, 1, epi);
-    };
-    const int64_t ldb = tap_major ? K : ddsp_pad4(n);
-    if (mode == DDSP_FIR_ALLPASS) {
-        gemm::Args g = gemm::make(act, lda, tab, ldb, (int)rows, n, K);
-        run(g, gemm::EpiStore{ir, n, nullptr, 1, 0, 0});
-    } else {
-        gemm::Args g = gemm::make(act, lda, tab, ldb, (int)rows, n / 2 + 1, K);
-        if (mode == DDSP_FIR_DYNAMIC)
-            run(g, EpiDynWindow{ir, n, f0_frames, 1.5f * (float)sr, (tap_major && ctx->math != DDSP_MATH_FP32) ? 1 : 0});
-        else
-            run(g, EpiMirrorStore{ir, n});
-    }
-    ddsp_prof_end(ctx, st, 2.0 * rows * (double)n * K, 4.0 * rows * (K + n));
+    fir_dft_launch(ctx, st, p, f0_frames, rows, sr);
+    ddsp_prof_end(ctx, st, 2.0 * rows * (double)p.n * p.K, 4.0 * rows * (p.K + p.n));
     DDSP_LAUNCH_CHECK(ctx);
+    return DDSP_OK;
+}
+
+extern "C" int ddsp_fir3_from_ctrl(ddsp_ctx* ctx, void* stream, const float* ctrl, int64_t ctrl_ld, const ddsp_fir_desc* filt,
+                                   const float* f0_frames, int64_t rows, int sr) {
+    DDSP_REQUIRE(ctx, ctx && ctrl && filt, "ddsp_fir3_from_ctrl: null argument");
+    DDSP_REQUIRE(ctx, rows >= 0 && rows < (1 << 30), "ddsp_fir3_from_ctrl: bad shape");
+    for (int i = 0; i < 3; ++i) {
+        const ddsp_fir_desc& d = filt[i];
+        DDSP_REQUIRE(ctx, d.ir, "ddsp_fir3_from_ctrl: null argument");
+        DDSP_REQUIRE(ctx, d.mode >= 0 && d.mode <= 2, "ddsp_fir3_from_ctrl: unknown mode");
+        DDSP_REQUIRE(ctx, d.n_mag >= 3 && d.n_mag <= 1024 && d.col0 >= 0 && ctrl_ld >= (int64_t)d.col0 + d.n_mag,
+                     "ddsp_fir3_from_ctrl: bad shape");
+        DDSP_REQUIRE(ctx, d.mode != DDSP_FIR_DYNAMIC || f0_frames, "ddsp_fir3_from_ctrl: DYNAMIC needs f0_frames");
+    }
+    if (rows == 0) return DDSP_OK;
+    hipStream_t st = (hipStream_t)stream;
+    DDSP_ENTER_DEVICE(ctx);
+    FirPlan p[3];
+    bool wide = true;
+    size_t bytes = 4096;
+    for (int i = 0; i < 3; ++i) {
+        int rc = fir_plan(ctx, st, filt[i].mode, ctrl + filt[i].col0, ctrl_ld, filt[i].n_mag, rows, filt[i].ir, p[i]);
+        if (rc) return rc;
+        wide = wide && p[i].wide;
+        bytes += (size_t)rows * p[i].lda * sizeof(float) + 256;
+    }
+    if (!wide) {
+        for (int i = 0; i < 3; ++i) {
+            int rc = ddsp_fir_from_ctrl(ctx, stream, filt[i].mode, ctrl + filt[i].col0, ctrl_ld, filt[i].n_mag, f0_frames, rows, sr,
+                                        filt[i].ir);
+            if (rc) return rc;
+        }
+        return DDSP_OK;
+    }
+    int rc = ddsp_scratch_reserve_bytes(ctx, bytes);
+    if (rc) return rc;
+    ddsp_scratch_reset(ctx);
+    FirActSeg seg[3];
+    unsigned blocks = 0;
+    double act_bytes = 0.0;
+    for (int i = 0; i < 3; ++i) {
+        if ((rc = ddsp_scratch_get(ctx, (size_t)rows * p[i].lda * sizeof(float), (void**)&p[i].act))) return rc;
+        const int64_t nb = p[i].mode == DDSP_FIR_ALLPASS ? ceil_div64(rows, 4) : ceil_div64(rows * (p[i].M / 8), 256);
+        seg[i] = FirActSeg{p[i].ctrl, p[i].act, p[i].M, p[i].lda, p[i].mode, p[i].presplit ? 1 : 0, (unsigned)nb};
+        blocks += (unsigned)nb;
+        act_bytes += 4.0 * rows * (p[i].M + p[i].K);
+    }
+    ddsp_prof_begin(ctx, st, PF_FIR_ACT);
+    hipLaunchKernelGGL(fir_act3_kernel, dim3(blocks), dim3(256), 0, st, seg[0], seg[1], seg[2], ctrl_ld, rows);
+    ddsp_prof_end(ctx, st, 0.0, act_bytes);
+    DDSP_LAUNCH_CHECK(ctx);
+    for (int i = 0; i < 3; ++i) {
+        ddsp_prof_begin(ctx, st, PF_FIR_DFT_GEMM);
+        fir_dft_launch(ctx, st, p[i], f0_frames, rows, sr);
+        ddsp_prof_end(ctx, st, 2.0 * rows * (double)p[i].n * p[i].K, 4.0 * rows * (p[i].K + p[i].n));
+        DDSP_LAUNCH_CHECK(ctx);
+    }
     return DDSP_OK;
 }
 
diff --git a/ddsp-svc-official_amd/csrc/gemm_f32.h b/ddsp-svc-official_amd/csrc/gemm_f32.h
--- a/ddsp-svc-official_amd/csrc/gemm_f32.h
+++ b/ddsp-svc-official_amd/csrc/gemm_f32.h
@@ -296,7 +296,7 @@
 }
 
 
-template <int BM, int BN, class Epi, int NS = 3, int NW = 8, int A_MODE = A_PLAIN, int MATH = 0>
+template <int BM, int BN, class Epi, int NS = 3, int NW = 8, int A_MODE = A_PLAIN, int MATH = 0, bool KSPLIT = false>
 __global__ void __launch_bounds__(64 * NW, (NW == 4 ? 3 : BM * BN <= 128 * 128 ? 4 : 2)) kernel_dma(Args g, Epi epi, int tiles_m, int tiles_n, int total_tiles) {
     constexpr int WGM = NW / 2, WGN = 2;
     constexpr int TM = BM / (32 * WGM), TN = BN / (32 * WGN);
@@ -428,6 +428,10 @@
         for (int j = 0; j < TN; ++j)
 #pragma unroll
             for (int r = 0; r < 16; ++r) acc[i][j][r] = 0.f;
+    f32x16 acc_lo[KSPLIT ? TM : 1][KSPLIT ? TN : 1];
+    (void)acc_lo;
+    static_assert(!KSPLIT || (!epi_has_store4<Epi>::value && !epi_is_gated<Epi>::value && !epi_is_rowpair<Epi>::value &&
+                              !epi_wants_pair<Epi>::value), "the split-K form hands (lo, hi) to a scalar epilogue");
 
     int kt = 0, tile_i = 0;
     for (int step = 0; step < steps; ++step) {
@@ -518,6 +522,18 @@
                     for (int j = 0; j < TN; ++j)
                         acc[i][j] = __builtin_amdgcn_mfma_f32_32x32x2f32(av[i][s >> 2][s & 3], bv[j][s >> 2][s & 3],
                                                                          acc[i][j], 0, 0, 0);
+        }
+        if constexpr (KSPLIT) {
+            if (kt + 1 == nk / 2) {
+#pragma unroll
+                for (int i = 0; i < TM; ++i)
+#pragma unroll
+                    for (int j = 0; j < TN; ++j) {
+                        acc_lo[i][j] = acc[i][j];
+#pragma unroll
+                        for (int r = 0; r < 16; ++r) acc[i][j][r] = 0.f;
+                    }
+            }
         }
         if (++kt == nk) {
             const int tile = tile_of(tile_i);
@@ -587,7 +603,10 @@
 #pragma unroll
                     for (int r = 0; r < 16; ++r) {
                         const int m = m0 + wm + 32 * i + (r & 3) + 8 * (r >> 2) + 4 * lh;
-                        if constexpr (epi_is_rowpair<Epi>::value) {
+                        if constexpr (KSPLIT) {
+                            (void)cb;
+                            if (n_ok && m < g.M) epi(z, m, n, acc_lo[i][j][r], acc[i][j][r]);
+                        } else if constexpr (epi_is_rowpair<Epi>::value) {
                             if ((r & 1) == 0 && n_ok && m < g.M) epi.pair(z, m, n, acc[i][j][r], acc[i][j][r + 1], cb);
                         } else if constexpr (epi_wants_pair<Epi>::value) {
                             const float other = __shfl_xor(acc[i][j][r], 1, 64);
@@ -609,7 +628,7 @@
            g.sA_hi % 4 == 0 && g.sA_lo % 4 == 0 && g.sB_hi % 4 == 0 && g.sB_lo % 4 == 0;
 }
 
-template <int BM, int BN, class Epi, int NS = 3, int NW = 8, int A_MODE = A_PLAIN, int MATH = 0>
+template <int BM, int BN, class Epi, int NS = 3, int NW = 8, int A_MODE = A_PLAIN, int MATH = 0, bool KSPLIT = false>
 inline void launch_dma(hipStream_t st, const Args& g, int batch, const Epi& epi, int total_override = -1) {
     const int tiles_m = (g.M + BM - 1) / BM, tiles_n = (g.N + BN - 1) / BN;
     const int total = total_override >= 0 ? total_override : tiles_m * tiles_n * batch;
@@ -620,27 +639,27 @@
     constexpr int per_cu = by_lds < by_waves ? by_lds : by_waves;
     int grid = 256 * per_cu;
     if (grid > total) grid = total;
-    hipLaunchKernelGGL((kernel_dma<BM, BN, Epi, NS, NW, A_MODE, MATH>), dim3(grid), dim3(64 * NW), 0, st, g, epi, tiles_m, tiles_n, total);
+    hipLaunchKernelGGL((kernel_dma<BM, BN, Epi, NS, NW, A_MODE, MATH, KSPLIT>), dim3(grid), dim3(64 * NW), 0, st, g, epi, tiles_m, tiles_n, total);
 }
 
 inline int xcd_default(int math) { return math == 3 ? 1 : 0; }
 
-template <int BM, int BN, class Epi, int NS = 3, int NW = 8, int A_MODE = A_PLAIN>
+template <int BM, int BN, class Epi, int NS = 3, int NW = 8, int A_MODE = A_PLAIN, bool KSPLIT = false>
 inline void dma_go(hipStream_t st, const Args& g0, int batch, const Epi& epi, int total_override = -1) {
     Args g = g0;
     if (g.xcd < 0) g.xcd = (batch == 1 && total_override < 0) ? xcd_default(g.math) : 0;
     if (g.math == 3 && g.B_split && g.A_split) {
         Args h = g;
         h.B = g.B_split;
-        launch_dma<BM, BN, Epi, NS, NW, A_MODE, 8>(st, h, batch, epi, total_override);
+        launch_dma<BM, BN, Epi, NS, NW, A_MODE, 8, KSPLIT>(st, h, batch, epi, total_override);
     } else if (g.math == 3 && g.B_split) {
         Args h = g;
         h.B = g.B_split;
-        launch_dma<BM, BN, Epi, NS, NW, A_MODE, 7>(st, h, batch, epi, total_override);
+        launch_dma<BM, BN, Epi, NS, NW, A_MODE, 7, KSPLIT>(st, h, batch, epi, total_override);
     } else if (g.math == 3)
-        launch_dma<BM, BN, Epi, NS, NW, A_MODE, 3>(st, g, batch, epi, total_override);
+        launch_dma<BM, BN, Epi, NS, NW, A_MODE, 3, KSPLIT>(st, g, batch, epi, total_override);
     else
-        launch_dma<BM, BN, Epi, NS, NW, A_MODE, 0>(st, g, batch, epi, total_override);
+        launch_dma<BM, BN, Epi, NS, NW, A_MODE, 0, KSPLIT>(st, g, batch, epi, total_override);
 }
 
 template <int BM, int BN, bool A_KC, bool B_KC, int A_MODE, class Epi, int NW = 4>
@@ -711,8 +730,14 @@
             return;
         }
     }
+    if constexpr (A_KC && B_KC && A_MODE == A_PLAIN) {
+        if (((g.B_split && g.B_split == g.B) || g.A_split) && dma_ok(g)) {
+            dma_go<64, 64, Epi, 3, 4>(st, g, batch, epi);
+            return;
+        }
+    }
     if ((g.B_split && g.B_split == g.B) || g.A_split) {
-        ddsp_launch_refusal() = "pre-split GEMM operands reached the register-staged path (size predicates disagree)";
+        ddsp_launch_refusal() = "pre-split GEMM operands do not qualify for the LDS-DMA kernel, which alone reads them";
         return;
     }
     if (blocks(128, 64) >= 512)
diff --git a/ddsp-svc-official_amd/csrc/tables.h b/ddsp-svc-official_amd/csrc/tables.h
--- a/ddsp-svc-official_amd/csrc/tables.h
+++ b/ddsp-svc-official_amd/csrc/tables.h
@@ -7,6 +7,7 @@
     TAB_IRDFT_CPLX = 3,
     TAB_RDFT_FWD_W = 4,
     TAB_RDFT_INV_W = 5,
+    TAB_IRDFT_CPLX_HALF = 6,
 };
 
 static inline int ddsp_pad4(int n) { return (n + 3) & ~3; }
diff --git a/ddsp-svc-official_amd/csrc/tables.hip b/ddsp-svc-official_amd/csrc/tables.hip
--- a/ddsp-svc-official_amd/csrc/tables.hip
+++ b/ddsp-svc-official_amd/csrc/tables.hip
@@ -4,8 +4,8 @@
 
 constexpr double kTwoPi = 6.283185307179586476925286766559;
 
-__global__ void irdft_table_kernel(float* __restrict__ tab, int M, int n, int ld, int rows, int hann, int tap_major) {
-    const int64_t total = tap_major ? (int64_t)n * rows : (int64_t)rows * ld;
+__global__ void irdft_table_kernel(float* __restrict__ tab, int M, int n, int ld, int rows, int hann, int tap_major, int ntap) {
+    const int64_t total = tap_major ? (int64_t)ntap * rows : (int64_t)rows * ld;
     for (int64_t idx = (int64_t)blockIdx.x * blockDim.x + threadIdx.x; idx < total;
          idx += (int64_t)gridDim.x * blockDim.x) {
         const int row = tap_major ? (int)(idx % rows) : (int)(idx / ld);
@@ -129,6 +129,10 @@
         case TAB_IRDFT_CPLX:
             elems = n1 ? (size_t)2 * n0 * 2 * (n0 - 1) : (size_t)2 * n0 * ddsp_pad4(2 * (n0 - 1));
             break;
+        case TAB_IRDFT_CPLX_HALF:
+            if (!n1) return ddsp_fail(ctx, DDSP_ERR_ARG, "the half inverse-DFT table is tap-major only", "");
+            elems = (size_t)2 * n0 * n0;
+            break;
         case TAB_RDFT_FWD_W:
             elems = (size_t)n0 * ddsp_pad4(2 * (n0 / 2 + 1));
             break;
@@ -142,11 +146,11 @@
     hipError_t e = hipMalloc((void**)&dev, elems * sizeof(float));
     if (e != hipSuccess) return ddsp_fail(ctx, DDSP_ERR_OOM, "table hipMalloc", hipGetErrorString(e));
     const unsigned blocks = (unsigned)((elems + 255) / 256 > 2048 ? 2048 : (elems + 255) / 256);
-    if (kind == TAB_IRDFT_RE || kind == TAB_IRDFT_RE_HANN || kind == TAB_IRDFT_CPLX) {
+    if (kind == TAB_IRDFT_RE || kind == TAB_IRDFT_RE_HANN || kind == TAB_IRDFT_CPLX || kind == TAB_IRDFT_CPLX_HALF) {
         const int M = n0, n = 2 * (n0 - 1);
-        const int rows = kind == TAB_IRDFT_CPLX ? 2 * M : M;
+        const int rows = (kind == TAB_IRDFT_CPLX || kind == TAB_IRDFT_CPLX_HALF) ? 2 * M : M;
         hipLaunchKernelGGL(irdft_table_kernel, dim3(blocks), dim3(256), 0, st, dev, M, n, ddsp_pad4(n), rows,
-                           kind == TAB_IRDFT_RE_HANN ? 1 : 0, n1 ? 1 : 0);
+                           kind == TAB_IRDFT_RE_HANN ? 1 : 0, n1 ? 1 : 0, kind == TAB_IRDFT_CPLX_HALF ? n / 2 + 1 : n);
     } else {
         hipLaunchKernelGGL(rdft_w_table_kernel, dim3(blocks), dim3(256), 0, st, dev, n0,
                            ddsp_pad4(2 * (n0 / 2 + 1)), kind == TAB_RDFT_INV_W ? 1 : 0);
diff --git a/ddsp-svc-official_amd/ddsp/vocoder.py b/ddsp-svc-official_amd/ddsp/vocoder.py
--- a/ddsp-svc-official_amd/ddsp/vocoder.py
+++ b/ddsp-svc-official_amd/ddsp/vocoder.py
@@ -435,16 +435,15 @@
         c2 = ctrl.reshape(rows, -1)
         crop = (lambda *xs: ctx.ragged_crop_(n_dev, Fr, hop, *xs)) if n_dev is not None else (lambda *xs: None)
         crop(comb)
-        ir = ctx.fir_from_ctrl(FIR_ALLPASS, c2, 0, na, rows, sr)
-        h, _ = ctx.ltv_fir(comb, ir, B, Fr, hop, math=ctx.fir_math)
+        ir_ap, ir_h, ir_n = ctx.fir3_from_ctrl(c2, [(FIR_ALLPASS, 0, na), (FIR_DYNAMIC, na, nh), (FIR_STATIC, na + nh, nn_)],
+                                               rows, sr, f0_frames)
+        h, _ = ctx.ltv_fir(comb, ir_ap, B, Fr, hop, math=ctx.fir_math)
         crop(h)
-        ir = ctx.fir_from_ctrl(FIR_DYNAMIC, c2, na, nh, rows, sr, f0_frames)
-        harmonic, _ = ctx.ltv_fir(h, ir, B, Fr, hop, math=ctx.fir_math)
+        harmonic, _ = ctx.ltv_fir(h, ir_h, B, Fr, hop, math=ctx.fir_math)
         crop(harmonic)
-        ir = ctx.fir_from_ctrl(FIR_STATIC, c2, na + nh, nn_, rows, sr)
         nz, exc, seed = self._noise_args(noise, noise_seed) if n_dev is None else \
             self._ragged_noise(ctx, n_dev, B, Fr, noise, noise_seed)
-        noise_out, signal = ctx.ltv_fir(nz, ir, B, Fr, hop, excitation=exc, noise_seed=seed, add_in=harmonic,
+        noise_out, signal = ctx.ltv_fir(nz, ir_n, B, Fr, hop, excitation=exc, noise_seed=seed, add_in=harmonic,
                                         math=ctx.fir_math)
         crop(noise_out, signal)
         return signal, harmonic, noise_out
diff --git a/ddsp-svc-official_amd/hipddsp/__init__.py b/ddsp-svc-official_amd/hipddsp/__init__.py
--- a/ddsp-svc-official_amd/hipddsp/__init__.py
+++ b/ddsp-svc-official_amd/hipddsp/__init__.py
@@ -106,6 +106,10 @@
                 ("flops_total", _c.c_double), ("bytes_total", _c.c_double)]
 
 
+class FirDesc(_c.Structure):
+    _fields_ = [("mode", _int), ("col0", _int), ("n_mag", _int), ("ir", _vp)]
+
+
 CONV_X_SPLIT, CONV_ACT_SPLIT = 1, 2
 
 
@@ -134,6 +138,7 @@
     "ddsp_upsample": (_int, [_vp, _vp, _vp, _i64, _i64, _i64, _int, _vp]),
     "ddsp_phase_scan": (_int, [_vp, _vp, _vp, _vp, _i64, _i64, _int, _int, _int, _int, _vp, _vp, _vp, _vp, _vp]),
     "ddsp_fir_from_ctrl": (_int, [_vp, _vp, _int, _vp, _i64, _int, _vp, _i64, _int, _vp]),
+    "ddsp_fir3_from_ctrl": (_int, [_vp, _vp, _vp, _i64, _c.POINTER(FirDesc), _vp, _i64, _int]),
     "ddsp_ltv_fir_bwd": (_int, [_vp, _vp, _vp, _int, _u64, _vp, _vp, _i64, _i64, _int, _int, _vp, _vp]),
     "ddsp_fir_from_ctrl_bwd": (_int, [_vp, _vp, _int, _vp, _i64, _int, _vp, _i64, _int, _vp, _vp, _i64]),
     "ddsp_sins_bank": (_int, [_vp, _vp, _vp, _i64, _int, _vp, _vp, _i64, _i64, _int, _int, _vp]),
@@ -550,6 +555,16 @@
         self.call("ddsp_fir_from_ctrl", int(mode), base, ld, int(n_mag), _ptr(f0), rows, int(sr), _ptr(ir))
         return ir
 
+    def fir3_from_ctrl(self, ctrl2d, filters, rows, sr, f0_frames=None):
+        if len(filters) != 3:
+            raise ValueError("fir3_from_ctrl takes exactly three filters")
+        irs = [torch.empty(rows, 2 * (n_mag - 1), device=ctrl2d.device, dtype=torch.float32) for _, _, n_mag in filters]
+        desc = (FirDesc * 3)(*[FirDesc(int(mode), int(col0), int(n_mag), _ptr(ir))
+                               for (mode, col0, n_mag), ir in zip(filters, irs)])
+        f0 = None if f0_frames is None else f0_frames.reshape(-1).contiguous().float()
+        self.call("ddsp_fir3_from_ctrl", _ptr(ctrl2d), ctrl2d.shape[-1], desc, _ptr(f0), rows, int(sr))
+        return irs
+
     def ltv_fir(self, audio, ir, B, Fr, hop, excitation=EXC_AUDIO, noise_seed=0, add_in=None, want_out=True,
                 math=FIR_FP32):
         n = ir.shape[-1]
diff --git a/include/ddsp_amd.h b/include/ddsp_amd.h
--- a/include/ddsp_amd.h
+++ b/include/ddsp_amd.h
@@ -40,6 +40,14 @@
 #define DDSP_FIR_STATIC 2
 int ddsp_fir_from_ctrl(ddsp_ctx* ctx, void* stream, int mode, const float* ctrl, int64_t ctrl_ld, int n_mag,
                        const float* f0_frames, int64_t rows, int sr, float* ir);
+typedef struct ddsp_fir_desc {
+    int mode;
+    int col0;
+    int n_mag;
+    float* ir;
+} ddsp_fir_desc;
+int ddsp_fir3_from_ctrl(ddsp_ctx* ctx, void* stream, const float* ctrl, int64_t ctrl_ld, const ddsp_fir_desc* filt,
+                        const float* f0_frames, int64_t rows, int sr);
 
 #define DDSP_FIR_FP32 0
 #define DDSP_FIR_SPLIT_BF16 3
```
